# hidasib/GRU4Rec

Measured on NVIDIA H100. Metric: mini-batches/sec, higher is better.
Workload: dtype f32

## Files before the change

### gru4rec_b200/_lib.py

```python
import ctypes as C
import os
import numpy as np

_HERE = os.path.dirname(os.path.abspath(__file__))
LIB_PATH = os.path.join(_HERE, 'libg4r.so')
G4R_MAX_LAYERS = 8
G4R_TOPK_MAX = 1024
SCHED_POSITIONS = 2

G4R_OK, G4R_ERR_INVALID, G4R_ERR_INDEX, G4R_ERR_CUDA, G4R_ERR_NAN, G4R_ERR_STATE = 0, -1, -2, -3, -4, -5
LOSS = {'cross-entropy': 0, 'bpr-max': 1, 'top1-max': 2, 'bpr': 3, 'top1': 4, 'xe_logit': 5}
ACT = {'linear': 0, 'relu': 1, 'tanh': 2, 'leaky': 3, 'elu': 4, 'selu': 5, 'softmax': 6, 'softmax_logit': 7}
ADAPT = {None: 0, 'adagrad': 1, 'rmsprop': 2, 'adadelta': 3, 'adam': 4}


class G4RConfig(C.Structure):
    _fields_ = [
        ('n_items', C.c_int32), ('n_layers', C.c_int32), ('layers', C.c_int32 * G4R_MAX_LAYERS), ('batch_size', C.c_int32),
        ('embedding', C.c_int32), ('constrained_embedding', C.c_int32), ('loss', C.c_int32),
        ('final_act', C.c_int32), ('final_act_p1', C.c_float), ('final_act_p2', C.c_float),
        ('hidden_act', C.c_int32), ('hidden_act_p1', C.c_float), ('hidden_act_p2', C.c_float),
        ('dropout_p_hidden', C.c_float), ('dropout_p_embed', C.c_float),
        ('learning_rate', C.c_float), ('momentum', C.c_float), ('lmbd', C.c_float),
        ('n_sample', C.c_int32), ('sample_alpha', C.c_float),
        ('smoothing', C.c_float), ('bpreg', C.c_float), ('logq', C.c_float),
        ('adapt', C.c_int32), ('sample_store', C.c_int32), ('dropout_seed', C.c_uint32), ('mrg_seed', C.c_uint32),
        ('max_resident_steps', C.c_int32), ('device', C.c_int32), ('world_size', C.c_int32), ('rank', C.c_int32),
        ('eval_batch_size', C.c_int32), ('step_mode', C.c_int32), ('mg_replicated', C.c_int32), ('eval_tc', C.c_int32),
        ('adapt_p1', C.c_float), ('adapt_p1c', C.c_float), ('adapt_p2', C.c_float), ('adapt_p2c', C.c_float), ('grad_cap', C.c_float),
    ]


EXPORTS = [
    'g4r_version', 'g4r_workspace_bytes', 'g4r_create', 'g4r_destroy', 'g4r_last_error', 'g4r_stream',
    'g4r_tensor_shape', 'g4r_set_tensor', 'g4r_get_tensor', 'g4r_reset_hidden',
    'g4r_set_sampling_cdf', 'g4r_set_logq_support', 'g4r_generate_samples', 'g4r_generate_samples_from_uniform',
    'g4r_set_sample_store', 'g4r_get_sample_store', 'g4r_sample_store_rows', 'g4r_set_sample_pointer', 'g4r_get_sample_pointer',
    'g4r_mrg_uniform', 'g4r_searchsorted', 'g4r_gather_rows',
    'g4r_schedule_build', 'g4r_schedule_build_history', 'g4r_schedule_free', 'g4r_schedule_steps', 'g4r_schedule_events', 'g4r_schedule_export', 'g4r_schedule_positions',
    'g4r_train_step', 'g4r_train_steps', 'g4r_upload_steps', 'g4r_run_uploaded', 'g4r_kernel_launches',
    'g4r_profile_uploaded', 'g4r_phase_name', 'g4r_phase_count', 'g4r_persistent_stamps', 'g4r_fast_windows', 'g4r_uses_tensor_cores', 'g4r_mg_unique_id', 'g4r_mg_init',
    'g4r_mg_sharded', 'g4r_mg_ipc_handle', 'g4r_mg_ipc_open', 'g4r_mg_owner', 'g4r_mg_local_row', 'g4r_mg_shard_rows', 'g4r_mg_segment_bytes',
    'g4r_eval_schedule', 'g4r_eval_events', 'g4r_eval_counts', 'g4r_set_eval_items', 'g4r_set_eval_exclude_seen', 'g4r_predict', 'g4r_reset_eval_hidden',
    'g4r_predict_topk', 'g4r_predict_topk_filtered',
    'g4r_sessions_open', 'g4r_sessions_count', 'g4r_sessions_feed', 'g4r_sessions_topk', 'g4r_sessions_end',
    'g4r_sessions_export', 'g4r_sessions_import',
]

_lib = None


def load():
    global _lib
    if _lib is not None:
        return _lib
    if not os.path.exists(LIB_PATH):
        raise RuntimeError('libg4r.so not found at %s: build it with gru4rec_b200/csrc/build.sh '
                           '(there is no CPU fallback)' % LIB_PATH)
    lib = C.CDLL(LIB_PATH)
    vp, i32, i64, f32p = C.c_void_p, C.c_int32, C.c_int64, C.POINTER(C.c_float)
    lib.g4r_version.restype = C.c_int
    lib.g4r_workspace_bytes.argtypes = [C.POINTER(G4RConfig), C.POINTER(C.c_size_t)]
    lib.g4r_create.argtypes = [C.POINTER(G4RConfig), vp, C.c_size_t, C.POINTER(vp)]
    lib.g4r_destroy.argtypes = [vp]
    lib.g4r_last_error.argtypes = [vp]; lib.g4r_last_error.restype = C.c_char_p
    lib.g4r_stream.argtypes = [vp]; lib.g4r_stream.restype = vp
    lib.g4r_tensor_shape.argtypes = [vp, C.c_char_p, C.POINTER(i64), C.POINTER(i64)]
    lib.g4r_set_tensor.argtypes = [vp, C.c_char_p, vp, i64, i64]
    lib.g4r_get_tensor.argtypes = [vp, C.c_char_p, vp, i64, i64]
    lib.g4r_reset_hidden.argtypes = [vp]
    lib.g4r_set_sampling_cdf.argtypes = [vp, vp, i64]
    lib.g4r_set_logq_support.argtypes = [vp, vp, i64]
    lib.g4r_generate_samples.argtypes = [vp]
    lib.g4r_generate_samples_from_uniform.argtypes = [vp, vp, i64]
    lib.g4r_set_sample_store.argtypes = [vp, vp, i64]
    lib.g4r_get_sample_store.argtypes = [vp, vp, i64]
    lib.g4r_sample_store_rows.argtypes = [vp]
    lib.g4r_set_sample_pointer.argtypes = [vp, i64]
    lib.g4r_get_sample_pointer.argtypes = [vp]; lib.g4r_get_sample_pointer.restype = i64
    lib.g4r_mrg_uniform.argtypes = [vp, vp, i64]
    lib.g4r_searchsorted.argtypes = [vp, vp, i64, vp, i64, vp]
    lib.g4r_gather_rows.argtypes = [vp, vp, i64, i64, vp, i64, vp]
    lib.g4r_schedule_build.argtypes = [vp, i64, vp, i64, vp, i32, i32, i32, C.POINTER(vp)]
    lib.g4r_schedule_build_history.argtypes = [vp, i64, vp, i64, vp, vp, i32, i32, C.POINTER(vp)]
    lib.g4r_schedule_free.argtypes = [vp]
    lib.g4r_schedule_steps.argtypes = [vp]; lib.g4r_schedule_steps.restype = i64
    lib.g4r_schedule_events.argtypes = [vp]; lib.g4r_schedule_events.restype = i64
    lib.g4r_schedule_export.argtypes = [vp, vp, vp, vp, vp, vp]
    lib.g4r_schedule_positions.argtypes = [vp, vp]
    lib.g4r_train_step.argtypes = [vp, vp, vp, i32, vp, C.POINTER(C.c_float)]
    lib.g4r_train_steps.argtypes = [vp, vp, i64, i64, vp, C.POINTER(i64)]
    lib.g4r_upload_steps.argtypes = [vp, vp, i64, i64]
    lib.g4r_run_uploaded.argtypes = [vp, vp, C.POINTER(C.c_float)]
    lib.g4r_kernel_launches.argtypes = [vp]; lib.g4r_kernel_launches.restype = i64
    lib.g4r_profile_uploaded.argtypes = [vp, vp, vp, i32]
    lib.g4r_phase_name.argtypes = [i32]; lib.g4r_phase_name.restype = C.c_char_p
    lib.g4r_phase_count.restype = C.c_int
    lib.g4r_persistent_stamps.argtypes = [vp, i32, vp, i64]
    lib.g4r_fast_windows.argtypes = [vp, C.POINTER(i64)]; lib.g4r_fast_windows.restype = i64
    lib.g4r_uses_tensor_cores.argtypes = [vp]
    lib.g4r_mg_unique_id.argtypes = [vp]
    lib.g4r_mg_init.argtypes = [vp, vp]
    lib.g4r_mg_sharded.argtypes = [vp]
    lib.g4r_mg_ipc_handle.argtypes = [vp, vp]
    lib.g4r_mg_ipc_open.argtypes = [vp, vp, i32]
    lib.g4r_mg_owner.argtypes = [i64, i32]
    lib.g4r_mg_local_row.argtypes = [i64, i32]; lib.g4r_mg_local_row.restype = i64
    lib.g4r_mg_shard_rows.argtypes = [i64, i32, i32]; lib.g4r_mg_shard_rows.restype = i64
    lib.g4r_mg_segment_bytes.argtypes = [C.POINTER(G4RConfig), C.POINTER(C.c_size_t), C.POINTER(C.c_size_t), C.POINTER(C.c_size_t), C.POINTER(C.c_size_t)]
    lib.g4r_eval_schedule.argtypes = [vp, vp, vp, i32, i32, vp, vp, C.POINTER(i64)]
    lib.g4r_eval_events.argtypes = [vp, vp, vp, i32, i32, i32, vp, vp, C.POINTER(i64), vp, vp, vp]
    lib.g4r_eval_counts.argtypes = [vp, vp, i64]
    lib.g4r_set_eval_items.argtypes = [vp, vp, i64]
    lib.g4r_set_eval_exclude_seen.argtypes = [vp, i32]
    lib.g4r_predict.argtypes = [vp, vp, i32, vp, vp]
    lib.g4r_reset_eval_hidden.argtypes = [vp]
    lib.g4r_predict_topk.argtypes = [vp, vp, i32, vp, i32, vp, vp]
    lib.g4r_predict_topk_filtered.argtypes = [vp, vp, i32, vp, i32, vp, i64, vp, vp, vp, vp]
    lib.g4r_sessions_open.argtypes = [vp, i64]
    lib.g4r_sessions_count.argtypes = [vp, C.POINTER(i64)]; lib.g4r_sessions_count.restype = i64
    lib.g4r_sessions_feed.argtypes = [vp, vp, vp, i64]
    lib.g4r_sessions_topk.argtypes = [vp, vp, vp, i64, i32, vp, i64, vp, vp, i32, vp, vp]
    lib.g4r_sessions_end.argtypes = [vp, vp, i64]
    lib.g4r_sessions_export.argtypes = [vp, vp, vp, vp, vp]
    lib.g4r_sessions_import.argtypes = [vp, vp, vp, vp, vp, i64]
    _lib = lib
    return lib


class NaNError(ArithmeticError):
    def __init__(self, msg, step):
        ArithmeticError.__init__(self, msg)
        self.step = step


def _ptr(a):
    return a.ctypes.data_as(C.c_void_p) if a is not None else None


def parse_act(name):
    if name in ('linear', 'relu', 'tanh', 'softmax', 'softmax_logit'):
        return ACT[name], 0.0, 0.0
    if name.startswith('leaky-'):
        return ACT['leaky'], float(name.split('-')[1]), 0.0
    if name.startswith('elu-'):
        return ACT['elu'], float(name.split('-')[1]), 0.0
    if name.startswith('selu-'):
        p = [float(x) for x in name.split('-')[1:]]
        return ACT['selu'], p[0], p[1]
    raise NotImplementedError


SEEN_BUDGET = 256 << 20


def seen_budget():
    env = os.environ.get('G4R_SEEN_BUDGET')
    return SEEN_BUDGET if env is None else min(SEEN_BUDGET, max(0, int(env)))


def check_topk(k, n_items):
    if not isinstance(k, (int, np.integer)) or isinstance(k, bool) or not 1 <= k <= min(n_items, G4R_TOPK_MAX):
        raise ValueError('k must be an integer in 1 .. min(n_items, %d) = %d, got %r' % (G4R_TOPK_MAX, min(n_items, G4R_TOPK_MAX), k))
    return int(k)


def set_adapt_params(cfg, adapt, adapt_params, grad_cap):
    ap = [float(x) for x in (adapt_params or [])]
    if adapt in ('rmsprop', 'adadelta') and len(ap) < 1 or adapt == 'adam' and len(ap) < 2:
        raise IndexError('list index out of range')
    cfg.adapt_p1 = ap[0] if len(ap) > 0 else 0.0
    cfg.adapt_p1c = (1.0 - ap[0]) if len(ap) > 0 else 0.0
    cfg.adapt_p2 = ap[1] if len(ap) > 1 else 0.0
    cfg.adapt_p2c = (1.0 - ap[1]) if len(ap) > 1 else 0.0
    cfg.grad_cap = float(grad_cap or 0.0)


def make_config(n_items, mk, sample_store=0, eval_lanes=0, max_resident_steps=0, step_mode=0, world_size=1, rank=0, replicated=False, eval_tc=None):
    cfg = G4RConfig()
    layers = mk.get('layers', [100])
    cfg.n_items = n_items
    cfg.n_layers = len(layers)
# ... 224 lines not shown
        self._check(self.lib.g4r_train_step(self.h, _ptr(X), _ptr(Y), len(X), _ptr(Rp), C.byref(cost)))
        return np.float32(cost.value)

    def train_steps(self, sched, first=0, n=None):
        n = sched.n_steps - first if n is None else n
        if self.cfg.world_size > 1:
            import torch
            import torch.distributed as dist
            if dist.is_available() and dist.is_initialized():
                dev = 'cuda' if dist.get_backend() == 'nccl' else 'cpu'
                t = torch.tensor([n, -n], dtype=torch.int64, device=dev)
                dist.all_reduce(t, op=dist.ReduceOp.MIN)
                if int(t[0]) != n or int(-t[1]) != n:
                    raise ValueError('train_steps: every rank must run the same number of steps (got %d, range %d..%d)' % (n, int(t[0]), int(-t[1])))
        costs = np.empty(n, dtype=np.float32)
        nan_step = C.c_int64(-1)
        rc = self.lib.g4r_train_steps(self.h, sched.h, first, n, _ptr(costs), C.byref(nan_step))
        self._check(rc, nan_step.value)
        return costs

    def upload_steps(self, sched, first, n):
        self._check(self.lib.g4r_upload_steps(self.h, sched.h, first, n))

    def run_uploaded(self, n, want_cost=True):
        costs = np.empty(n, dtype=np.float32) if want_cost else None
        ms = C.c_float()
        self._check(self.lib.g4r_run_uploaded(self.h, _ptr(costs), C.byref(ms)))
        return costs, ms.value

    def profile_uploaded(self):
        n = self.lib.g4r_phase_count()
        ms = np.zeros(n, dtype=np.float32); cnt = np.zeros(n, dtype=np.int32)
        self._check(self.lib.g4r_profile_uploaded(self.h, _ptr(ms), _ptr(cnt), n))
        return {self.lib.g4r_phase_name(i).decode(): (float(ms[i]), int(cnt[i])) for i in range(n) if cnt[i] > 0}

    def persistent_stamps(self, enable=True, n_steps=0):
        out = np.zeros((n_steps, 16), dtype=np.uint64) if n_steps > 0 else None
        self._check(self.lib.g4r_persistent_stamps(self.h, 1 if enable else 0, _ptr(out), n_steps))
        return out

    def init_multi_gpu(self, dist):
        import torch
        buf = (C.c_char * 128)()
        if dist.get_rank() == 0:
            rc = self.lib.g4r_mg_unique_id(buf)
            if rc != 0:
                raise RuntimeError('ncclGetUniqueId failed')
        t = torch.tensor(list(bytes(buf)), dtype=torch.uint8, device='cuda' if dist.get_backend() == 'nccl' else 'cpu')
        dist.broadcast(t, 0)
        raw = bytes(t.cpu().tolist())
        idbuf = (C.c_char * 128).from_buffer_copy(raw)
        self._check(self.lib.g4r_mg_init(self.h, idbuf))
        self._dist = dist
        if self.sharded():
            mh = (C.c_char * 64)()
            self._check(self.lib.g4r_mg_ipc_handle(self.h, mh))
            dev = 'cuda' if dist.get_backend() == 'nccl' else 'cpu'
            mine = torch.tensor(list(bytes(mh)), dtype=torch.uint8, device=dev)
            allh = [torch.empty_like(mine) for _ in range(dist.get_world_size())]
            dist.all_gather(allh, mine)
            raw = b''.join(bytes(t.cpu().tolist()) for t in allh)
            buf2 = (C.c_char * len(raw)).from_buffer_copy(raw)
            self._check(self.lib.g4r_mg_ipc_open(self.h, buf2, dist.get_world_size()))
            dist.barrier()

    def sharded(self):
        return bool(self.lib.g4r_mg_sharded(self.h))

    def _quiesce(self):
        d = getattr(self, '_dist', None)
        if d is not None and self.sharded():
            import torch
            torch.cuda.synchronize()
            d.barrier()

    def uses_tensor_cores(self):
        return bool(self.lib.g4r_uses_tensor_cores(self.h))

    def fast_windows(self):
        fb = C.c_int64()
        n = self.lib.g4r_fast_windows(self.h, C.byref(fb))
        return n, fb.value

    def kernel_launches(self):
        return self.lib.g4r_kernel_launches(self.h)

    def stream(self):
        return self.lib.g4r_stream(self.h)

    def eval_schedule(self, sched, cut_off, mode=0):
        cut = np.ascontiguousarray(cut_off, dtype=np.int32)
        rec = np.zeros(len(cut), dtype=np.float64); mrr = np.zeros(len(cut), dtype=np.float64)
        n = C.c_int64()
        self._check(self.lib.g4r_eval_schedule(self.h, sched.h, _ptr(cut), len(cut), mode, _ptr(rec), _ptr(mrr), C.byref(n)))
        return rec, mrr, n.value

    def eval_events(self, sched, cut_off, mode=0, k=0):
        cut = np.ascontiguousarray(cut_off, dtype=np.int32)
        rec = np.zeros(len(cut), dtype=np.float64); mrr = np.zeros(len(cut), dtype=np.float64)
        n = C.c_int64()
        counts = np.empty((sched.n_events, 2), dtype=np.int32)
        items = scores = None
        if k:
            items = np.empty((sched.n_events, k), dtype=np.int32); scores = np.empty((sched.n_events, k), dtype=np.float32)
        self._check(self.lib.g4r_eval_events(self.h, sched.h, _ptr(cut), len(cut), mode, int(k), _ptr(rec), _ptr(mrr), C.byref(n),
                                             _ptr(counts), _ptr(items), _ptr(scores)))
        return rec, mrr, n.value, counts, items, scores

    def eval_counts(self, n_lanes):
        out = np.zeros((n_lanes, 2), dtype=np.int32)
        self._check(self.lib.g4r_eval_counts(self.h, _ptr(out), n_lanes))
        return out

    def set_eval_items(self, items=None):
        if items is None or len(items) == 0:
            self._check(self.lib.g4r_set_eval_items(self.h, None, 0))
            return
        it = np.ascontiguousarray(items, dtype=np.int64)
        self._check(self.lib.g4r_set_eval_items(self.h, _ptr(it), it.size))

    def set_eval_exclude_seen(self, on):
        self._check(self.lib.g4r_set_eval_exclude_seen(self.h, 1 if on else 0))

    def predict(self, X, reset_mask=None):
        X = np.ascontiguousarray(X, dtype=np.int32)
        rm = None if reset_mask is None else np.ascontiguousarray(reset_mask, dtype=np.uint8)
        out = np.empty((len(X), self.cfg.n_items), dtype=np.float32)
        self._check(self.lib.g4r_predict(self.h, _ptr(X), len(X), _ptr(rm), _ptr(out)))
        return out

    def predict_topk(self, X, k, reset_mask=None, items=None, exclude=None):
        X = np.ascontiguousarray(X, dtype=np.int32)
        rm = None if reset_mask is None else np.ascontiguousarray(reset_mask, dtype=np.uint8)
        if items is None and exclude is None:
            k = check_topk(k, self.cfg.n_items)
            out_i = np.empty((len(X), k), dtype=np.int32)
            out_s = np.empty((len(X), k), dtype=np.float32)
            self._check(self.lib.g4r_predict_topk(self.h, _ptr(X), len(X), _ptr(rm), k, _ptr(out_i), _ptr(out_s)))
            return out_i, out_s
        k, cand, off, ex = self._topk_filters(len(X), k, items, exclude)
        out_i = np.empty((len(X), k), dtype=np.int32)
        out_s = np.empty((len(X), k), dtype=np.float32)
        self._check(self.lib.g4r_predict_topk_filtered(self.h, _ptr(X), len(X), _ptr(rm), k, _ptr(cand), 0 if cand is None else cand.size,
                                                       _ptr(off), _ptr(ex), _ptr(out_i), _ptr(out_s)))
        return out_i, out_s

    def _topk_filters(self, n, k, items, exclude):
        cand = None
        n_distinct = self.cfg.n_items
        if items is not None:
            cand = np.asarray(items, dtype=np.int64).reshape(-1)
            if cand.size and (cand.min() < 0 or cand.max() >= self.cfg.n_items):
                raise IndexError('candidate item index out of range')
            cand = np.ascontiguousarray(cand, dtype=np.int32)
            n_distinct = int(np.count_nonzero(np.bincount(cand, minlength=self.cfg.n_items)))
        k = check_topk(k, n_distinct)
        off = ex = None
        if exclude is not None:
            if len(exclude) != n:
                raise ValueError('exclude must hold one entry per lane (%d), got %d' % (n, len(exclude)))
            parts = [np.asarray(e if e is not None else [], dtype=np.int64).reshape(-1) for e in exclude]
            off = np.zeros(n + 1, dtype=np.int64)
            off[1:] = np.cumsum([len(p) for p in parts])
            ex = np.concatenate(parts) if parts else np.zeros(0, np.int64)
            if ex.size and (ex.min() < 0 or ex.max() >= self.cfg.n_items):
                raise IndexError('excluded item index out of range')
# ... 60 lines not shown
```

### gru4rec_b200/csrc/g4r_fast.cuh

```cuda
#pragma once

constexpr int FK_THREADS = 512;
constexpr int FK_NW = FK_THREADS / 32;
constexpr int FK_G = 48;
constexpr int FK_CT = 32;
constexpr int FK_Q = FK_CT / FK_NW;
constexpr int FK_B = 32;
static_assert(FK_THREADS / 16 == FK_B, "statistics mapping: 16 threads per lane");
constexpr int FK_LDS = 132;


__device__ __forceinline__ void red_release_add(unsigned int* p, unsigned int v) {
  asm volatile("red.release.gpu.global.add.u32 [%0], %1;" :: "l"(p), "r"(v) : "memory");
}
__device__ __forceinline__ unsigned int atom_acqrel_add(unsigned int* p, unsigned int v) {
  unsigned int old;
  asm volatile("atom.acq_rel.gpu.global.add.u32 %0, [%1], %2;" : "=r"(old) : "l"(p), "r"(v) : "memory");
  return old;
}
__device__ __forceinline__ void wait_ge(const unsigned int* p, unsigned int target) {
  while (ld_acquire_u32(p) < target) { }
}
__device__ __forceinline__ uint32_t smem_u32(const void* p) { return (uint32_t)__cvta_generic_to_shared(p); }
__device__ __forceinline__ void mbar_init(uint64_t* bar, unsigned int count) {
  asm volatile("mbarrier.init.shared::cta.b64 [%0], %1;" :: "r"(smem_u32(bar)), "r"(count) : "memory");
}
__device__ __forceinline__ void mbar_expect_tx(uint64_t* bar, unsigned int bytes) {
  asm volatile("mbarrier.arrive.expect_tx.shared::cta.b64 _, [%0], %1;" :: "r"(smem_u32(bar)), "r"(bytes) : "memory");
}
__device__ __forceinline__ void mbar_wait(uint64_t* bar, unsigned int parity) {
  asm volatile(
      "{\n\t.reg .pred p;\n\t"
      "WAIT_LOOP:\n\t"
      "mbarrier.try_wait.parity.shared::cta.b64 p, [%0], %1;\n\t"
      "@p bra.uni WAIT_DONE;\n\t"
      "bra.uni WAIT_LOOP;\n\t"
      "WAIT_DONE:\n\t}\n" :: "r"(smem_u32(bar)), "r"(parity) : "memory");
}
__device__ __forceinline__ void tma_row(void* sdst, const void* gsrc, unsigned int bytes, uint64_t* bar) {
  asm volatile("cp.async.bulk.shared::cluster.global.mbarrier::complete_tx::bytes [%0], [%1], %2, [%3];"
               :: "r"(smem_u32(sdst)), "l"(gsrc), "r"(bytes), "r"(smem_u32(bar)) : "memory");
}

struct FastSmem {
  alignas(128) float sY[FK_B * FK_LDS];
  float sS[FK_CT * FK_LDS];
  float sAcc[FK_CT * FK_LDS];
  float sVel[FK_CT * FK_LDS];
  float sTW[FK_B * FK_LDS];
  float sD[FK_CT * FK_LDS];
  float sG[FK_CT * FK_B];
  float sO[FK_CT * FK_B];
  float sRS[FK_B * 8];
  float sPart[FK_NW * FK_B * 8];
  float sT[FK_B];
  float sBias[FK_CT], sByP[FK_CT], sByA[FK_CT], sByV[FK_CT], sDby[FK_CT], sTB[FK_B];
  int sIt[2][FK_CT], sPos[2][FK_CT], sTc[2][FK_B], sYit[2][FK_B], sCb[2][2];
  int sFlag[4];
  alignas(8) unsigned long long mbar;
  alignas(16) float gA[FK_B * 388];
  alignas(16) float gW[8 * FK_LDS + FK_NW * FK_B * 5 + 16 * FK_B];
  int gIdx[3 * FK_B];
};

template <class SM>
__device__ __forceinline__ void fk_load_idx(const ModelDev& md, SM& sm, int s, int n_steps, int chunk, int buf) {
  const int tid = threadIdx.x;
  if (s >= n_steps) return;
  const int M = md.wM[s];
  const int* cbeg = md.pCbeg + (size_t)s * (md.NCH + 1);
  const bool hc = chunk < md.NCH;
  const int cb = hc ? cbeg[chunk] : 0, ce = hc ? cbeg[chunk + 1] : 0;
  if (tid < FK_CT) {
    int it = 0, pos = 0;
    if (cb + tid < ce) { it = md.pItem[(size_t)s * md.NP + cb + tid]; pos = md.pPos[(size_t)s * md.NP + cb + tid]; }
    sm.sIt[buf][tid] = it; sm.sPos[buf][tid] = pos;
  }
  if (tid >= 32 && tid < 32 + FK_B) {
    const int b = tid - 32;
    sm.sTc[buf][b] = b < M ? md.pTcol[(size_t)s * md.B + b] : -1;
    sm.sYit[buf][b] = b < M ? md.wY[(size_t)s * md.B + b] : 0;
  }
  if (tid == 64) { sm.sCb[buf][0] = cb; sm.sCb[buf][1] = ce; }
}

template <class SM>
__device__ __forceinline__ void fk_prefetch_rows(const ModelDev& md, SM& sm, int s, int n_steps, int buf, bool pw) {
  if (s >= n_steps) return;
  const int tid = threadIdx.x;
  const int M = md.wM[s];
  const int cb = sm.sCb[buf][0], ce = sm.sCb[buf][1];
  const int nj = ce - cb;
  const bool ada = md.adapt == G4R_ADAPT_ADAGRAD, mom = md.mom > 0.f;
  const unsigned int rowb = (unsigned int)md.ldL * 4u;
  uint64_t* bar = reinterpret_cast<uint64_t*>(&sm.mbar);
  const int ntab = 1 + (ada ? 1 : 0) + (mom ? 1 : 0);
  const int ncopy = nj * ntab + (pw ? M : 0);
  if (tid == 0) {
    const unsigned int total = rowb * (unsigned int)ncopy;
    if (total > 0) mbar_expect_tx(bar, total);
    else asm volatile("mbarrier.arrive.shared::cta.b64 _, [%0];" :: "r"(smem_u32(bar)) : "memory");
  }
  if ((tid & 31) == 0) {
    asm volatile("fence.proxy.async.global;" ::: "memory");
    for (int i = tid >> 5; i < ncopy; i += FK_NW) {
      if (i < nj * ntab) {
        const int j = i / ntab, t = i % ntab;
        const size_t off = (size_t)sm.sIt[buf][j] * md.ldL;
        if (t == 0) tma_row(sm.sS + j * FK_LDS, md.Wy + off, rowb, bar);
        else if (t == 1 && ada) tma_row(sm.sAcc + j * FK_LDS, md.Wy_acc + off, rowb, bar);
        else tma_row(sm.sVel + j * FK_LDS, md.Wy_vel + off, rowb, bar);
      } else {
        const int b = i - nj * ntab;
        tma_row(sm.sTW + b * FK_LDS, md.Wy + (size_t)sm.sYit[buf][b] * md.ldL, rowb, bar);
      }
    }
  }
  if (false) {
  } else if (tid >= 64 && tid < 64 + FK_CT) {
    const int j = tid - 64;
    if (j < nj) {
      const int it = sm.sIt[buf][j];
      float bz = md.By[it];
      sm.sByP[j] = bz;
      if (md.logq > 0.f) bz -= (sm.sPos[buf][j] < M) ? md.logP0t[it] : md.logP0s[it];
      sm.sBias[j] = bz;
      sm.sByA[j] = ada ? md.By_acc[it] : 0.f;
      sm.sByV[j] = mom ? md.By_vel[it] : 0.f;
    }
  } else if (tid >= 96 && tid < 96 + FK_B) {
    const int b = tid - 96;
    if (pw && b < M) {
      const int it = sm.sYit[buf][b];
      float bz = md.By[it];
      if (md.logq > 0.f) bz -= md.logP0t[it];
      sm.sTB[b] = bz;
    }
  }
}

__device__ __forceinline__ void fk_group_barrier(FastSync* fs, unsigned int& gepoch, unsigned int G = FK_G) {
  __syncthreads();
  gepoch += 1;
  if (threadIdx.x == 0) { red_release_add(&fs->grp, 1u); wait_ge(&fs->grp, gepoch * G); }
  __syncthreads();
}

template <class SM>
__device__ __forceinline__ void fk_stage_lanes(const ModelDev& md, SM& sm, int s, int M) {
  if (threadIdx.x < FK_B) {
    const int b = threadIdx.x;
    sm.gIdx[b] = b < M ? md.wSlot[(size_t)s * md.B + b] : -1;
    sm.gIdx[FK_B + b] = b < M ? md.wX[(size_t)s * md.B + b] : 0;
    sm.gIdx[2 * FK_B + b] = b < M ? md.wF[(size_t)s * md.B + b] : 0;
  }
  __syncthreads();
}
template <int W>
__device__ __forceinline__ void fk_slab_dot(float (&acc)[W], const float* sAop, int lda, const float* sWt, int K) {
  const int b = threadIdx.x & 31, ks = threadIdx.x >> 5;
  const int kq = (K + 3) / 4;
  const int per = (kq + FK_NW - 1) / FK_NW;
  const int q0 = ks * per, q1 = min(kq, q0 + per);
#pragma unroll
  for (int j = 0; j < W; j++) acc[j] = 0.f;
  for (int q = q0; q < q1; q++) {
    const float4 a = ld4(sAop + b * lda + q * 4);
#pragma unroll
    for (int j = 0; j < W; j++) {
      const float4 w = ld4(sWt + j * FK_LDS + q * 4);
      acc[j] = fmaf(a.x, w.x, acc[j]); acc[j] = fmaf(a.y, w.y, acc[j]); acc[j] = fmaf(a.z, w.z, acc[j]); acc[j] = fmaf(a.w, w.w, acc[j]);
    }
  }
}
template <int W>
__device__ __forceinline__ float fk_slab_reduce(const float (&acc)[W], float* red, int jsel) {
  const int b = threadIdx.x & 31, ks = threadIdx.x >> 5;
#pragma unroll
  for (int j = 0; j < W; j++) red[(ks * FK_B + b) * W + j] = acc[j];
  __syncthreads();
  float v = 0.f;
  if (jsel < W) {
#pragma unroll
    for (int k = 0; k < FK_NW; k++) v += red[(k * FK_B + b) * W + jsel];
  }
  return v;
}
constexpr int FK_W1 = 5;
constexpr int FK_W2 = 3;

__device__ void fk_f1(const ModelDev& md, FastSmem& sm, int s, int cta, const unsigned int* wait_ctr, unsigned int wait_target, const float* inrows = nullptr) {
  const LayerDev& ly = md.layer[0];
  const int M = md.wM[s], L = ly.L, ldL = ly.ldL, tid = threadIdx.x;
  const int c0 = cta * FK_W1;
  if (c0 >= 2 * L) return;
  const int W = min(FK_W1, 2 * L - c0);
  fk_stage_lanes(md, sm, s, M);
  if (tid == 0) sm.sFlag[3] = (!wait_ctr || ld_acquire_u32(wait_ctr) >= wait_target) ? 1 : 0;
  const int kw = ldL / 4;
  stage_rows4(sm.gA, FK_LDS, FK_B, kw, [&](int rr) -> const float* { const int sl = sm.gIdx[rr]; return sl >= 0 ? ly.H + (size_t)sl * ldL : nullptr; });
  for (int i = tid; i < FK_W1 * FK_LDS; i += FK_THREADS) {
    const int j = i / FK_LDS, k = i % FK_LDS;
    sm.gW[i] = (j < W && k < L) ? ly.Wrz[(size_t)k * ly.ld2 + c0 + j] : 0.f;
  }
  const int b = tid & 31, jsel = tid >> 5;
  __syncthreads();
  const bool early = sm.sFlag[3] != 0;
  float pre = 0.f;
  if (early && jsel < W && b < M) pre = (inrows ? inrows[(size_t)b * ly.ld3 + L + c0 + jsel] : ly.Wx[(size_t)sm.gIdx[FK_B + b] * ly.ld3 + L + c0 + jsel]) + ly.Bh[L + c0 + jsel];
  float acc[FK_W1];
  fk_slab_dot<FK_W1>(acc, sm.gA, FK_LDS, sm.gW, L);
  const float v = fk_slab_reduce<FK_W1>(acc, sm.gW + 8 * FK_LDS, jsel);
  if (!early) {
    if (tid == 0) wait_ge(wait_ctr, wait_target);
    __syncthreads();
    if (jsel < W && b < M) pre = (inrows ? inrows[(size_t)b * ly.ld3 + L + c0 + jsel] : ly.Wx[(size_t)sm.gIdx[FK_B + b] * ly.ld3 + L + c0 + jsel]) + ly.Bh[L + c0 + jsel];
  }
  if (jsel < W && b < M) {
    const int c = c0 + jsel;
    const float g = sigmoidf_(v + pre);
    if (c < L) ly.r[(size_t)b * ldL + c] = g; else ly.z[(size_t)b * ldL + (c - L)] = g;
  }
  if (cta == 0) {
    for (int i = tid; i < FK_B * kw; i += FK_THREADS) {
      const int rr = i / kw, c4 = i % kw;
      if (rr < M) st4(ly.Hold + (size_t)rr * ldL + c4 * 4, ld4(sm.gA + rr * FK_LDS + c4 * 4));
    }
// ... 18 lines not shown
        if (rr < M) { hv[u] = ld4(ly.Hold + (size_t)rr * ldL + c4 * 4); rv[u] = ld4(ly.r + (size_t)rr * ldL + c4 * 4); }
      }
    }
#pragma unroll
    for (int u = 0; u < 2; u++) {
      const int i = i0 + u * FK_THREADS + tid;
      if (i < FK_B * kw) st4(sm.gA + (i / kw) * FK_LDS + (i % kw) * 4, make_float4(hv[u].x * rv[u].x, hv[u].y * rv[u].y, hv[u].z * rv[u].z, hv[u].w * rv[u].w));
    }
  }
  for (int i = tid; i < FK_W2 * FK_LDS; i += FK_THREADS) {
    const int j = i / FK_LDS, k = i % FK_LDS;
    sm.gW[i] = (j < W && k < L) ? ly.Wh[(size_t)k * ldL + c0 + j] : 0.f;
  }
  const int b = tid & 31, jsel = tid >> 5;
  float pre = 0.f, z = 0.f, ho = 0.f;
  if (jsel < W && b < M) {
    const int c = c0 + jsel;
    pre = (inrows ? inrows[(size_t)b * ly.ld3 + c] : ly.Wx[(size_t)sm.gIdx[FK_B + b] * ly.ld3 + c]) + ly.Bh[c];
    z = ly.z[(size_t)b * ldL + c];
    ho = ly.Hold[(size_t)b * ldL + c];
  }
  __syncthreads();
  float acc[FK_W2];
  fk_slab_dot<FK_W2>(acc, sm.gA, FK_LDS, sm.gW, L);
  const float v0 = fk_slab_reduce<FK_W2>(acc, sm.gW + 8 * FK_LDS, jsel);
  if (jsel < W && b < M) {
    const int c = c0 + jsel;
    const float v = v0 + pre;
    const float ht = act_fwd(md.hact, v);
    float h = (1.0f - z) * ho + z * ht;
    if (md.p_drop_h > 0.f) h *= drop_scale(md.drop_seed, md.wG[s], 0u, (uint32_t)(b * L + c), 1.0f - md.p_drop_h);
    ly.ah[(size_t)b * ldL + c] = v;
    ly.ht[(size_t)b * ldL + c] = ht;
    ly.y[(size_t)b * ldL + c] = h;
    ly.H[(size_t)sm.gIdx[b] * ldL + c] = (sm.gIdx[2 * FK_B + b] & 1) ? 0.f : h;
  }
}
__device__ void fk_b2(const ModelDev& md, FastSmem& sm, int s, int cta) {
  const LayerDev& ly = md.layer[0];
  const int M = md.wM[s], L = ly.L, ldL = ly.ldL, tid = threadIdx.x;
  const int c0 = cta * FK_W2;
  if (c0 >= L) return;
  const int W = min(FK_W2, L - c0);
  const int kw = ldL / 4;
  __syncthreads();
  stage_rows4(sm.gA, FK_LDS, FK_B, kw, [&](int rr) -> const float* { return rr < M ? ly.dvec + (size_t)rr * ly.ld3 : nullptr; });
  stage_rows4(sm.gW, FK_LDS, W, kw, [&](int rr) -> const float* { return ly.Wh + (size_t)(c0 + rr) * ldL; });
  const int b = tid & 31, jsel = tid >> 5;
  float ho = 0.f, r = 0.f;
  if (jsel < W && b < M) { ho = ly.Hold[(size_t)b * ldL + c0 + jsel]; r = ly.r[(size_t)b * ldL + c0 + jsel]; }
  __syncthreads();
  float acc[FK_W2];
  fk_slab_dot<FK_W2>(acc, sm.gA, FK_LDS, sm.gW, L);
  const float v = fk_slab_reduce<FK_W2>(acc, sm.gW + 8 * FK_LDS, jsel);
  if (jsel < W && b < M) ly.dvec[(size_t)b * ly.ld3 + L + c0 + jsel] = v * ho * r * (1.f - r);
}
template <class SM>
__device__ void fk_sparse_in(const ModelDev& md, SM& sm, int s, int b) {
  const LayerDev& ly = md.layer[0];
  const int M = md.wM[s];
  if (b >= M) return;
  const uint8_t xf = md.wXflag[(size_t)s * md.B + b];
  if (!(xf & 1)) return;
  const int ld3 = ly.ld3, tid = threadIdx.x;
  const int item = md.wX[(size_t)s * md.B + b];
  const int* xnext = md.wXnext + (size_t)s * md.B;
  if (tid == 0) { int n = 0; for (int bb = b; bb >= 0 && n < FK_B; bb = xnext[bb]) sm.gIdx[n++] = bb; sm.gIdx[FK_B] = n; }
  __syncthreads();
  const int nmem = sm.gIdx[FK_B];
  const bool ada = md.adapt == G4R_ADAPT_ADAGRAD, mom = md.mom > 0.f;
  float* prow = ly.Wx + (size_t)item * ld3;
  for (int c4 = tid; c4 < ld3 / 4; c4 += FK_THREADS) {
    const float4 p0 = ld4(prow + c4 * 4), z = make_float4(0.f, 0.f, 0.f, 0.f);
    RowChain<float4> u;
    u.begin(p0, p0, ada ? ld4(ly.Wx_acc + (size_t)item * ld3 + c4 * 4) : z, mom ? ld4(ly.Wx_vel + (size_t)item * ld3 + c4 * 4) : z);
    for (int k = 0; k < nmem; k++) u.add(md, ld4(ly.dvec + (size_t)sm.gIdx[k] * ld3 + c4 * 4), ada, mom);
    st4(prow + c4 * 4, u.ps);
    if (ada) st4(ly.Wx_acc + (size_t)item * ld3 + c4 * 4, u.al);
    if (mom) st4(ly.Wx_vel + (size_t)item * ld3 + c4 * 4, u.vl);
  }
}

template <class SM>
__device__ void fk_sparse_in_one(const ModelDev& md, SM& sm, int s, int b, const unsigned int* ctr, unsigned int target) {
  const LayerDev& ly = md.layer[0];
  const int M = md.wM[s], ld3 = ly.ld3, tid = threadIdx.x;
  const bool act = b < M && (md.wXflag[(size_t)s * md.B + b] & 1);
  const int item = act ? md.wX[(size_t)s * md.B + b] : 0;
  const bool ada = md.adapt == G4R_ADAPT_ADAGRAD, mom = md.mom > 0.f;
  if (act && tid == 0) {
    const int* xnext = md.wXnext + (size_t)s * md.B;
    int n = 0; for (int bb = b; bb >= 0 && n < FK_B; bb = xnext[bb]) sm.gIdx[n++] = bb; sm.gIdx[FK_B] = n;
  }
  float* prow = ly.Wx + (size_t)item * ld3;
  const int c4 = tid;
  const bool mine = act && c4 < ld3 / 4;
  float4 p0 = make_float4(0.f, 0.f, 0.f, 0.f), a0 = p0, v0 = p0;
  if (mine) {
    p0 = ld4(prow + c4 * 4);
    if (ada) a0 = ld4(ly.Wx_acc + (size_t)item * ld3 + c4 * 4);
    if (mom) v0 = ld4(ly.Wx_vel + (size_t)item * ld3 + c4 * 4);
  }
  if (tid == 0) wait_ge(ctr, target);
  __syncthreads();
  if (mine) {
    const int nmem = sm.gIdx[FK_B];
    RowChain<float4> u;
    u.begin(p0, p0, a0, v0);
    for (int k = 0; k < nmem; k++) u.add(md, ld4(ly.dvec + (size_t)sm.gIdx[k] * ld3 + c4 * 4), ada, mom);
    st4(prow + c4 * 4, u.ps);
    if (ada) st4(ly.Wx_acc + (size_t)item * ld3 + c4 * 4, u.al);
    if (mom) st4(ly.Wx_vel + (size_t)item * ld3 + c4 * 4, u.vl);
  }
}

template <bool CL, class SM>
__device__ void fk_b1(const ModelDev& md, SM& sm, int s, int cta, int ncta) {
  const LayerDev& ly = md.layer[0];
  const int M = md.wM[s], L = ly.L, ldL = ly.ldL;
  const int tid = threadIdx.x, lane = tid & 31, warp = tid >> 5;
  const int E = M * ldL;
  const int per = ((E + ncta - 1) / ncta + 31) / 32 * 32;
  const int e0 = cta * per;
  float* red = sm.sPart;
  const size_t cs = (size_t)md.B * ldL;
  float pht = 0.f, pho = 0.f, pz = 0.f, pah = 0.f;
  if (!CL && tid < per && e0 + tid < E && (e0 + tid) % ldL < L) {
    const size_t o = (size_t)((e0 + tid) / ldL) * ldL + (e0 + tid) % ldL;
    pht = ly.ht[o]; pho = ly.Hold[o]; pz = ly.z[o]; pah = ly.ah[o];
  }
  for (int eb = 0; eb < per; eb += 32) {
    const int e = e0 + eb + lane;
    float d = 0.f;
    if (e < E) {
      float v[10];
#pragma unroll
      for (int u = 0; u < 10; u++) { const int ch = warp + FK_NW * u; v[u] = ch < md.NCH ? md.part[(size_t)ch * cs + e] : 0.f; }
      d = (((v[0] + v[1]) + (v[2] + v[3])) + ((v[4] + v[5]) + (v[6] + v[7]))) + (v[8] + v[9]);
    }
    red[warp * per + eb + lane] = d;
  }
  __syncthreads();
  for (int i = tid; i < per; i += FK_THREADS) {
    const int e = e0 + i;
    if (e >= E) continue;
    const int b = e / ldL, c = e % ldL;
    if (c >= L) continue;
    float dy = 0.f;
#pragma unroll
    for (int w = 0; w < FK_NW; w++) dy += red[w * per + i];
    const size_t o = (size_t)b * ldL + c;
    if (CL) { ly.dy[o] = dy; continue; }
    const float ht = pht, ho = pho, z = pz, ah = pah;
    float dh = dy;
    if (md.p_drop_h > 0.f) dh *= drop_scale(md.drop_seed, md.wG[s], 0u, (uint32_t)(b * L + c), 1.0f - md.p_drop_h);
    const float dz = dh * (ht - ho);
    const float dah = dh * z * act_der(md.hact, ah, ht);
    ly.dvec[(size_t)b * ly.ld3 + c] = dah;
    ly.dvec[(size_t)b * ly.ld3 + 2 * L + c] = dz * z * (1.f - z);
  }
}

constexpr int FR_U = 4;

struct FastSmemR {
  alignas(128) float sY[FK_B * FK_LDS];
  float sS[FK_CT * FK_LDS];
  float sAcc[FK_CT * FK_LDS];
  float sVel[FK_CT * FK_LDS];
  float sTW[FK_B * FK_LDS];
  float sD[FK_CT * FK_LDS];
  float sG[FK_CT * FK_B];
  float sO[FK_CT * FK_B];
  float sRS[FK_B * 8];
  float sPart[FK_NW * FK_B * 8];
  float sT[FK_B];
  float sBias[FK_CT], sByP[FK_CT], sByA[FK_CT], sByV[FK_CT], sDby[FK_CT], sTB[FK_B];
  int sIt[2][FK_CT], sPos[2][FK_CT], sTc[2][FK_B], sYit[2][FK_B], sCb[2][2];
  int sFlag[4];
  alignas(8) unsigned long long mbar;
  int gIdx[3 * FK_B];
  alignas(16) float gH[2][FK_B * FK_LDS];
  float gHr[FK_B * FK_LDS];
  float rC[3][3 * FR_U * FK_LDS];
  float rR[3][FR_U * FK_LDS];
  float rB[3][3 * FR_U];
  float gR[FK_B * FR_U], gZ[FK_B * FR_U], gDr[FK_B * FR_U], gDz[FK_B * FR_U];
};
static_assert(sizeof(FastSmemR) <= 232448, "FastSmemR exceeds the 227 KB shared memory of one CTA");
static_assert(FK_NW * FK_B * 8 >= FK_NW * FK_B * 2 * FR_U, "sPart too small for the F1 reduction");

__device__ void fr_load_resident(const ModelDev& md, FastSmemR& sm, int k0) {
  const LayerDev& ly = md.layer[0];
  const int L = ly.L, tid = threadIdx.x;
  for (int i = tid; i < 3 * FR_U * FK_LDS; i += FK_THREADS) {
    const int q = i / FK_LDS, k = i % FK_LDS, t = q / FR_U, c = k0 + q % FR_U;
    float p = 0.f, a = 0.f, v = 0.f;
    if (c < L && k < L) {
      const size_t o = t == 0 ? (size_t)k * ly.ldL + c : (size_t)k * ly.ld2 + (t == 2 ? L : 0) + c;
      const float* P = t == 0 ? ly.Wh : ly.Wrz;
      const float* A = t == 0 ? ly.Wh_acc : ly.Wrz_acc;
      const float* V = t == 0 ? ly.Wh_vel : ly.Wrz_vel;
      p = P[o]; if (A) a = A[o]; if (V) v = V[o];
    }
    sm.rC[0][i] = p; sm.rC[1][i] = a; sm.rC[2][i] = v;
  }
  for (int i = tid; i < FR_U * FK_LDS; i += FK_THREADS) {
    const int k = k0 + i / FK_LDS, c = i % FK_LDS;
    float p = 0.f, a = 0.f, v = 0.f;
    if (k < L && c < L) {
      const size_t o = (size_t)k * ly.ldL + c;
      p = ly.Wh[o]; if (ly.Wh_acc) a = ly.Wh_acc[o]; if (ly.Wh_vel) v = ly.Wh_vel[o];
    }
    sm.rR[0][i] = p; sm.rR[1][i] = a; sm.rR[2][i] = v;
  }
  if (tid < 3 * FR_U) {
    const int c = k0 + tid % FR_U;
    float p = 0.f, a = 0.f, v = 0.f;
    if (c < L) { const int o = (tid / FR_U) * L + c; p = ly.Bh[o]; if (ly.Bh_acc) a = ly.Bh_acc[o]; if (ly.Bh_vel) v = ly.Bh_vel[o]; }
    sm.rB[0][tid] = p; sm.rB[1][tid] = a; sm.rB[2][tid] = v;
  }
  __syncthreads();
}
__device__ void fr_store_resident(const ModelDev& md, FastSmemR& sm, int k0) {
  const LayerDev& ly = md.layer[0];
  const int L = ly.L, tid = threadIdx.x;
  __syncthreads();
  for (int i = tid; i < 3 * FR_U * FK_LDS; i += FK_THREADS) {
    const int q = i / FK_LDS, k = i % FK_LDS, t = q / FR_U, c = k0 + q % FR_U;
    if (c < L && k < L) {
      const size_t o = t == 0 ? (size_t)k * ly.ldL + c : (size_t)k * ly.ld2 + (t == 2 ? L : 0) + c;
      float* P = t == 0 ? ly.Wh : ly.Wrz;
      float* A = t == 0 ? ly.Wh_acc : ly.Wrz_acc;
      float* V = t == 0 ? ly.Wh_vel : ly.Wrz_vel;
      P[o] = sm.rC[0][i]; if (A) A[o] = sm.rC[1][i]; if (V) V[o] = sm.rC[2][i];
    }
  }
  if (tid < 3 * FR_U) {
    const int c = k0 + tid % FR_U;
    if (c < L) { const int o = (tid / FR_U) * L + c; ly.Bh[o] = sm.rB[0][tid]; if (ly.Bh_acc) ly.Bh_acc[o] = sm.rB[1][tid]; if (ly.Bh_vel) ly.Bh_vel[o] = sm.rB[2][tid]; }
  }
}

__device__ void fr_f1(const ModelDev& md, FastSmemR& sm, int s, int k0, const float* sH, const unsigned int* wait_ctr, unsigned int wait_target) {
  const LayerDev& ly = md.layer[0];
  const int M = md.wM[s], L = ly.L, ldL = ly.ldL, tid = threadIdx.x;
  if (tid == 0) sm.sFlag[3] = (!wait_ctr || ld_acquire_u32(wait_ctr) >= wait_target) ? 1 : 0;
  __syncthreads();
  const bool early = sm.sFlag[3] != 0;
  const int b = tid & 31, jsel = tid >> 5, j = jsel % FR_U, c = k0 + j;
  const bool isr = jsel < FR_U;
  const bool on = jsel < 2 * FR_U && b < M && c < L;
  const int col = (isr ? L : 2 * L) + c;
  const float bias = sm.rB[0][(isr ? 1 : 2) * FR_U + j];
  float pre = 0.f;
  if (early && on) pre = ly.Wx[(size_t)sm.gIdx[FK_B + b] * ly.ld3 + col] + bias;
  float acc[2 * FR_U];
  fk_slab_dot<2 * FR_U>(acc, sH, FK_LDS, sm.rC[0] + FR_U * FK_LDS, L);
  const float v = fk_slab_reduce<2 * FR_U>(acc, sm.sPart, jsel);
  if (!early) {
    if (tid == 0) wait_ge(wait_ctr, wait_target);
    __syncthreads();
    if (on) pre = ly.Wx[(size_t)sm.gIdx[FK_B + b] * ly.ld3 + col] + bias;
  }
  if (jsel < 2 * FR_U) {
    const float g = on ? sigmoidf_(v + pre) : 0.f;
    if (isr) {
      sm.gR[b * FR_U + j] = g;
      if (on) {
        const float ho = sH[b * FK_LDS + c];
        ly.r[(size_t)b * ldL + c] = g;
        ly.Hold[(size_t)b * ldL + c] = ho;
        ly.Hr[(size_t)b * ldL + c] = ho * g;
      }
    } else {
      sm.gZ[b * FR_U + j] = g;
      if (on) ly.z[(size_t)b * ldL + c] = g;
    }
  }
}
__device__ void fr_f2(const ModelDev& md, FastSmemR& sm, int s, int k0, const float* sHo) {
  const LayerDev& ly = md.layer[0];
  const int M = md.wM[s], L = ly.L, ldL = ly.ldL, tid = threadIdx.x;
  const int b = tid & 31, jsel = tid >> 5, c = k0 + jsel;
  const bool on = jsel < FR_U && b < M && c < L;
  float pre = 0.f;
  if (on) pre = ly.Wx[(size_t)sm.gIdx[FK_B + b] * ly.ld3 + c] + sm.rB[0][jsel];
  stage_rows4(sm.gHr, FK_LDS, FK_B, ldL / 4, [&](int rr) -> const float* { return rr < M ? ly.Hr + (size_t)rr * ldL : nullptr; });
  __syncthreads();
  float acc[FR_U];
  fk_slab_dot<FR_U>(acc, sm.gHr, FK_LDS, sm.rC[0], L);
  const float v0 = fk_slab_reduce<FR_U>(acc, sm.sPart, jsel);
  if (on) {
    const float v = v0 + pre;
    const float ht = act_fwd(md.hact, v);
    const float z = sm.gZ[b * FR_U + jsel], ho = sHo[b * FK_LDS + c];
    float h = (1.0f - z) * ho + z * ht;
    if (md.p_drop_h > 0.f) h *= drop_scale(md.drop_seed, md.wG[s], 0u, (uint32_t)(b * L + c), 1.0f - md.p_drop_h);
    ly.ah[(size_t)b * ldL + c] = v;
    ly.ht[(size_t)b * ldL + c] = ht;
    ly.y[(size_t)b * ldL + c] = h;
    ly.H[(size_t)sm.gIdx[b] * ldL + c] = (sm.gIdx[2 * FK_B + b] & 1) ? 0.f : h;
  }
}
__device__ void fr_b2(const ModelDev& md, FastSmemR& sm, int s, int k0, const float* sHo) {
  const LayerDev& ly = md.layer[0];
  const int M = md.wM[s], L = ly.L, ld3 = ly.ld3, tid = threadIdx.x;
  float dz = 0.f;
  if (tid < FK_B * FR_U && tid / FR_U < M && k0 + tid % FR_U < L) dz = ly.dvec[(size_t)(tid / FR_U) * ld3 + 2 * L + k0 + tid % FR_U];
  stage_rows4(sm.sD, FK_LDS, FK_B, ly.ldL / 4, [&](int rr) -> const float* { return rr < M ? ly.dvec + (size_t)rr * ld3 : nullptr; });
  if (tid < FK_B * FR_U) sm.gDz[tid] = dz;
  __syncthreads();
  const int b = tid & 31, jsel = tid >> 5, c = k0 + jsel;
  float acc[FR_U];
  fk_slab_dot<FR_U>(acc, sm.sD, FK_LDS, sm.rR[0], L);
  const float v = fk_slab_reduce<FR_U>(acc, sm.sPart, jsel);
  if (jsel < FR_U) {
    float dar = 0.f;
    if (b < M && c < L) {
      const float ho = sHo[b * FK_LDS + c], r = sm.gR[b * FR_U + jsel];
      dar = v * ho * r * (1.f - r);
      ly.dvec[(size_t)b * ld3 + L + c] = dar;
    }
    sm.gDr[b * FR_U + jsel] = dar;
  }
}
__device__ void fr_dense(const ModelDev& md, FastSmemR& sm, int s, int k0, const float* sHo) {
  const LayerDev& ly = md.layer[0];
  const int M = md.wM[s], L = ly.L, kw = ly.ldL / 4;
  const bool ada = md.adapt == G4R_ADAPT_ADAGRAD, mom = md.mom > 0.f;
  const int ncol = 3 * FR_U * kw, nrow = FR_U * kw;
  for (int t = threadIdx.x; t < ncol + nrow + 3 * FR_U; t += FK_THREADS) {
    if (t < ncol + nrow) {
      const bool colt = t < ncol;
      const int u = colt ? t : t - ncol, q = u % kw, jm = u / kw, j = jm % FR_U;
      const float* vec; const float* sc; int ss, o;
      if (colt) {
        const int m = jm / FR_U;
        vec = (m == 0 ? sm.gHr : sHo) + q * 4;
        if (m == 0) { sc = sm.sD + k0 + j; ss = FK_LDS; } else { sc = (m == 1 ? sm.gDr : sm.gDz) + j; ss = FR_U; }
        o = jm * FK_LDS + q * 4;
      } else {
        vec = sm.sD + q * 4; sc = sm.gHr + k0 + j; ss = FK_LDS;
        o = j * FK_LDS + q * 4;
      }
      float4 g = make_float4(0.f, 0.f, 0.f, 0.f);
#pragma unroll 4
      for (int b = 0; b < M; b++) {
        const float4 a = ld4(vec + b * FK_LDS);
        const float d = sc[b * ss];
        g.x = fmaf(a.x, d, g.x); g.y = fmaf(a.y, d, g.y); g.z = fmaf(a.z, d, g.z); g.w = fmaf(a.w, d, g.w);
      }
      if (k0 + j < L) {
        float* P = colt ? sm.rC[0] : sm.rR[0];
        float* A = colt ? sm.rC[1] : sm.rR[1];
        float* V = colt ? sm.rC[2] : sm.rR[2];
        if (q * 4 + 0 < L) dense_elem(md, ada, mom, g.x, P + o + 0, A + o + 0, V + o + 0);
        if (q * 4 + 1 < L) dense_elem(md, ada, mom, g.y, P + o + 1, A + o + 1, V + o + 1);
        if (q * 4 + 2 < L) dense_elem(md, ada, mom, g.z, P + o + 2, A + o + 2, V + o + 2);
        if (q * 4 + 3 < L) dense_elem(md, ada, mom, g.w, P + o + 3, A + o + 3, V + o + 3);
      }
    } else {
      const int i = t - ncol - nrow, m = i / FR_U, j = i % FR_U;
      if (k0 + j < L) {
        float g = 0.f;
        for (int b = 0; b < M; b++) g = g + (m == 0 ? sm.sD[b * FK_LDS + k0 + j] : (m == 1 ? sm.gDr : sm.gDz)[b * FR_U + j]);
        dense_elem(md, ada, mom, g, sm.rB[0] + i, sm.rB[1] + i, sm.rB[2] + i);
      }
    }
  }
}
template <class SM>
__device__ __forceinline__ void fk_part(SM& sm, float* part, int M, int nj, int ldL) {
  const int kw = ldL / 4;
  for (int t = threadIdx.x; t < M * kw; t += FK_THREADS) {
    const int bb = t / kw, q4 = t % kw;
    float4 a = make_float4(0.f, 0.f, 0.f, 0.f);
    for (int jj = 0; jj < nj; jj++) {
      const float g = sm.sG[jj * FK_B + bb];
      const float4 w = ld4(sm.sS + jj * FK_LDS + q4 * 4);
      a.x = fmaf(g, w.x, a.x); a.y = fmaf(g, w.y, a.y); a.z = fmaf(g, w.z, a.z); a.w = fmaf(g, w.w, a.w);
    }
    st4(part + (size_t)bb * ldL + q4 * 4, a);
  }
}
template <class SM>
__device__ __forceinline__ void fk_dsy(SM& sm, int M, int nj, int kw) {
  for (int t = threadIdx.x; t < nj * kw; t += FK_THREADS) {
    const int jj = t / kw, q4 = t % kw;
    float4 d = make_float4(0.f, 0.f, 0.f, 0.f);
    for (int bb = 0; bb < M; bb++) {
      const float4 y = ld4(sm.sY + bb * FK_LDS + q4 * 4);
      const float g = sm.sG[jj * FK_B + bb];
      d.x = fmaf(g, y.x, d.x); d.y = fmaf(g, y.y, d.y); d.z = fmaf(g, y.z, d.z); d.w = fmaf(g, y.w, d.w);
    }
    st4(sm.sD + jj * FK_LDS + q4 * 4, d);
  }
}
template <class SM>
__device__ __forceinline__ void fk_update_rows(const ModelDev& md, SM& sm, int buf, int nj, int kw) {
  const int lane = threadIdx.x & 31, warp = threadIdx.x >> 5, ldL = md.ldL;
  const bool ada = md.adapt == G4R_ADAPT_ADAGRAD, mom = md.mom > 0.f;
  for (int j = warp; j < nj; j += FK_NW) {
    const int item = sm.sIt[buf][j];
    if (j > 0 && sm.sIt[buf][j - 1] == item) continue;
    int je = j + 1;
    while (je < nj && sm.sIt[buf][je] == item) je++;
    if (lane < kw) {
      const float4 p0 = ld4(sm.sS + j * FK_LDS + lane * 4), z = make_float4(0.f, 0.f, 0.f, 0.f);
      RowChain<float4> u;
      u.begin(p0, p0, ada ? ld4(sm.sAcc + j * FK_LDS + lane * 4) : z, mom ? ld4(sm.sVel + j * FK_LDS + lane * 4) : z);
      for (int k = j; k < je; k++) u.add(md, ld4(sm.sD + k * FK_LDS + lane * 4), ada, mom);
      const size_t off = (size_t)item * ldL + lane * 4;
      st4(md.Wy + off, u.ps);
      if (ada) st4(md.Wy_acc + off, u.al);
      if (mom) st4(md.Wy_vel + off, u.vl);
    }
    if (lane == 0) {
      RowChain<float> u;
      u.begin(sm.sByP[j], sm.sByP[j], sm.sByA[j], sm.sByV[j]);
      for (int k = j; k < je; k++) u.add(md, sm.sDby[k], ada, mom);
      md.By[item] = u.ps;
      if (ada) md.By_acc[item] = u.al;
      if (mom) md.By_vel[item] = u.vl;
    }
  }
}
template <class SM>
__device__ __forceinline__ void fk_dby(SM& sm, int M, int nj) {
  const int lane = threadIdx.x & 31, warp = threadIdx.x >> 5;
  for (int jj = warp; jj < nj; jj += FK_NW) {
    float a = (lane < M) ? sm.sG[jj * FK_B + lane] : 0.f;
    a = warp_sum(a);
    if (lane == 0) sm.sDby[jj] = a;
  }
}
#include "g4r_fastc.cuh"

template <bool CL>
__global__ void __launch_bounds__(FK_THREADS, 1) k_fast_t(int slot, int n_steps, FastSync* fs, unsigned long long* tstamp) {
  using SM = typename std::conditional<CL, FastSmemC, FastSmemR>::type;
  extern __shared__ __align__(128) unsigned char fk_raw[];
  SM& sm = *reinterpret_cast<SM*>(fk_raw);
  const ModelDev& md = MD;
  const LayerDev& ly = md.layer[0];
  const int cta = blockIdx.x, ncta = gridDim.x;
  const int tid = threadIdx.x, lane = tid & 31, warp = tid >> 5;
  const int G = CL ? (int)cl_size() : md.ldL / 4;
  const bool gru = cta < G;
  const bool col = CL || !gru;
  const int chunk = CL ? cta : cta - G;
  const int ncol = CL ? ncta : ncta - G;
  const bool has_chunk = col && chunk < md.NCH;
  const bool pw = loss_pairwise(md.loss);
  const int ldL = md.ldL, B = md.B;
  const int kw = ldL / 4;
  uint64_t* bar = reinterpret_cast<uint64_t*>(&sm.mbar);
  unsigned int bar_epoch = 0, gepoch = 0, stats_target = 0;
  const int in_ctas = min(B, ncta - G);
#ifdef G4R_CF_FINE
#define FK_FTS(s_) ((tstamp && cta == 0 && (s_) < 500 && n_steps >= 1000) ? tstamp + (size_t)((s_) + 500) * 16 : nullptr)
#define FK_STAMP_OK(s_) ((s_) < 500)
#else
#define FK_FTS(s_) ((unsigned long long*)nullptr)
#define FK_STAMP_OK(s_) true
#endif
#define FK_STAMP(k) do { if (tstamp && cta == ((CL || ((k) >= 4 && (k) <= 8)) ? 0 : G) && tid == 0 && FK_STAMP_OK(s)) { unsigned long long t_; asm volatile("mov.u64 %0, %%globaltimer;" : "=l"(t_)); tstamp[(size_t)s * 16 + (k)] = t_; } } while (0)
  if (tid == 0) { mbar_init(bar, 1); asm volatile("fence.mbarrier_init.release.cluster;" ::: "memory"); }
  if (col) fk_load_idx(md, sm, 0, n_steps, chunk, 0);
  __syncthreads();
  if (col) fk_prefetch_rows(md, sm, 0, n_steps, 0, pw);
  ClusterCtx cc = {0, 1, 0, 0};
  if constexpr (CL) {
    if (gru) {
      cc = cf_init(md, sm);
      cf_load_resident(md, sm, cc);
      if (n_steps > 0) {
        fk_stage_lanes(md, sm, 0, md.wM[0]);
        cf_f1(md, sm, cc, 0, false, nullptr, 0u, nullptr);
        cf_f2(md, sm, cc, 0, nullptr);
        __syncthreads();
        if (tid == 0) red_release_add(&fs->h_ready, 1u);
      }
    }
  } else {
    if (gru) {
      fr_load_resident(md, sm, 4 * cta);
      if (n_steps > 0) {
        fk_stage_lanes(md, sm, 0, md.wM[0]);
        stage_rows4(sm.gH[0], FK_LDS, FK_B, kw, [&](int rr) -> const float* { const int sl = sm.gIdx[rr]; return sl >= 0 ? ly.H + (size_t)sl * ldL : nullptr; });
        fr_f1(md, sm, 0, 4 * cta, sm.gH[0], nullptr, 0u);
        fk_group_barrier(fs, gepoch, G);
        fr_f2(md, sm, 0, 4 * cta, sm.gH[0]);
        __syncthreads();
        if (tid == 0) red_release_add(&fs->h_ready, 1u);
      }
    }
  }
  for (int s = 0; s < n_steps; s++) {
    const int buf = s & 1;
    const int M = md.wM[s];
    const int sti = md.wSti[s];
    const int N = M + (sti >= 0 ? md.S : 0);
    FK_STAMP(0);
    if (col) fk_load_idx(md, sm, s + 1, n_steps, chunk, buf ^ 1);
    const bool gru_next = !CL && gru && s + 1 < n_steps;
    if (gru_next && tid < FK_B) {
      const int M1 = md.wM[s + 1];
      sm.gIdx[tid] = tid < M1 ? md.wSlot[(size_t)(s + 1) * B + tid] : -1;
      sm.gIdx[FK_B + tid] = tid < M1 ? md.wX[(size_t)(s + 1) * B + tid] : 0;
      sm.gIdx[2 * FK_B + tid] = tid < M1 ? md.wF[(size_t)(s + 1) * B + tid] : 0;
    }
    if (tid == 0) wait_ge(&fs->h_ready, (unsigned int)(s + 1) * (unsigned int)G);
    __syncthreads();
    if constexpr (!CL) {
      if (!col) {
        const bool nxt = s + 1 < n_steps;
        const int k0 = 4 * cta;
        const float* sHo = sm.gH[s & 1];
        float* hnext = sm.gH[(s + 1) & 1];
        if (nxt) stage_rows4(hnext, FK_LDS, FK_B, kw, [&](int rr) -> const float* { const int sl = sm.gIdx[rr]; return sl >= 0 ? ly.H + (size_t)sl * ldL : nullptr; });
        __syncthreads();
        if (tid == 0) wait_ge(&fs->b1_done, (unsigned int)(s + 1) * (unsigned int)ncol);
        __syncthreads();
        FK_STAMP(4);
        fr_b2(md, sm, s, k0, sHo);
        __syncthreads();
        if (tid == 0) red_release_add(&fs->dvec_done, 1u);
        FK_STAMP(5);
        fr_dense(md, sm, s, k0, sHo);
        FK_STAMP(6);
        if (nxt) {
          fr_f1(md, sm, s + 1, k0, hnext, &fs->in_done, (unsigned int)(s + 1) * (unsigned int)in_ctas);
          fk_group_barrier(fs, gepoch, G);
          FK_STAMP(7);
          fr_f2(md, sm, s + 1, k0, hnext);
          __syncthreads();
          if (tid == 0) red_release_add(&fs->h_ready, 1u);
        }
        FK_STAMP(8);
        continue;
      }
    }
    stage_rows4(sm.sY, FK_LDS, FK_B, kw, [&](int rr) -> const float* { return rr < M ? ly.y + (size_t)rr * ldL : nullptr; });
    mbar_wait(bar, (unsigned int)(s & 1));
    __syncthreads();
    FK_STAMP(1);
    const int cb = sm.sCb[buf][0], ce = sm.sCb[buf][1];
    const int nj = ce - cb;
    if (pw) {
      for (int b = warp; b < FK_B; b += FK_NW) {
        if (b < M) {
          float a = 0.f;
          if (lane < kw) {
            const float4 y = ld4(sm.sY + b * FK_LDS + lane * 4), w = ld4(sm.sTW + b * FK_LDS + lane * 4);
            a = fmaf(w.x, y.x, a); a = fmaf(w.y, y.y, a); a = fmaf(w.z, y.z, a); a = fmaf(w.w, y.w, a);
          }
          a = warp_sum(a);
          if (lane == 0) sm.sT[b] = act_fwd(md.fact, a + sm.sTB[b]);
        }
      }
    }
    {
      float accq[FK_Q];
#pragma unroll
      for (int q = 0; q < FK_Q; q++) accq[q] = 0.f;
      const float* yr = sm.sY + lane * FK_LDS;
      for (int c4 = 0; c4 < kw; c4++) {
        const float4 y = ld4(yr + c4 * 4);
#pragma unroll
        for (int q = 0; q < FK_Q; q++) {
          if (warp + FK_NW * q < nj) {
            const float4 w = ld4(sm.sS + (warp + FK_NW * q) * FK_LDS + c4 * 4);
            accq[q] = fmaf(y.x, w.x, accq[q]); accq[q] = fmaf(y.y, w.y, accq[q]); accq[q] = fmaf(y.z, w.z, accq[q]); accq[q] = fmaf(y.w, w.w, accq[q]);
          }
        }
      }
      FK_STAMP(9);
#pragma unroll
      for (int q = 0; q < FK_Q; q++) {
        const int jj = warp + q * FK_NW;
        if (jj < nj && lane < M) sm.sO[jj * FK_B + lane] = accq[q] + sm.sBias[jj];
      }
      __syncthreads();
      {
        const int b = tid >> 4, sub = tid & 15;
        const bool okb = b < M;
        const int tc = okb ? sm.sTc[buf][b] : -1;
        const float t = (pw && okb) ? sm.sT[b] : 0.f;
        float yv[2]; bool use[2], ist[2];
        float mloc = -INFINITY;
        const bool smx = loss_softmaxneg(md.loss), xe = (md.loss == G4R_LOSS_XE || md.loss == G4R_LOSS_XE_LOGIT);
#pragma unroll
        for (int q = 0; q < 2; q++) {
          const int jj = sub + 16 * q;
          use[q] = okb && jj < nj;
          ist[q] = use[q] && (tc == cb + jj);
          const float o = use[q] ? sm.sO[jj * FK_B + b] : 0.f;
          yv[q] = xe ? o : act_fwd(md.fact, o);
          if (use[q] && (xe || (smx && !ist[q]))) mloc = fmaxf(mloc, yv[q]);
        }
#pragma unroll
        for (int o = 1; o < 16; o <<= 1) mloc = fmaxf(mloc, __shfl_xor_sync(0xffffffffu, mloc, o));
        float Z = 0.f, A = 0.f, Q = 0.f, D = 0.f, T = 0.f, has = 0.f;
#pragma unroll
        for (int q = 0; q < 2; q++) {
          if (!use[q]) continue;
          const float y = yv[q];
          if (ist[q]) has = 1.f;
          if (xe) { Z += expf(y - mloc); if (ist[q]) T = y; }
          else if (md.loss == G4R_LOSS_BPR_MAX) { if (!ist[q]) { const float e = expf(y - mloc), sg = sigmoidf_(t - y); Z += e; A += sg * e; Q += y * y * e; D += sg * (1.f - sg) * e; } }
          else if (md.loss == G4R_LOSS_TOP1_MAX) { if (!ist[q]) { const float e = expf(y - mloc), a1 = sigmoidf_(y - t), b1 = sigmoidf_(y * y); Z += e; A += (a1 + b1) * e; D += a1 * (1.f - a1) * e; } }
          else if (md.loss == G4R_LOSS_BPR) { const float sg = sigmoidf_(t - y); A += -logf(sg); if (!ist[q]) D += 1.f - sg; }
          else { const float a1 = sigmoidf_(y - t), b1 = sigmoidf_(y * y); A += a1 + b1; if (!ist[q]) D += a1 * (1.f - a1); }
        }
#pragma unroll
        for (int o = 1; o < 16; o <<= 1) {
          Z += __shfl_xor_sync(0xffffffffu, Z, o); A += __shfl_xor_sync(0xffffffffu, A, o); Q += __shfl_xor_sync(0xffffffffu, Q, o);
          D += __shfl_xor_sync(0xffffffffu, D, o); T += __shfl_xor_sync(0xffffffffu, T, o); has += __shfl_xor_sync(0xffffffffu, has, o);
        }
        if (has_chunk && okb && sub == 0) {
          float* st = md.stat + ((size_t)chunk * md.B + b) * G4R_NSTAT;
          st4(st, make_float4(mloc, Z, A, Q));
          st4(st + 4, make_float4(D, T, has > 0.f ? 1.f : 0.f, pw ? t : 0.f));
        }
      }
    }
    __syncthreads();
    FK_STAMP(10);
    bar_epoch += 1;
    if (tid == 0) { red_release_add(&fs->bar, 1u); wait_ge(&fs->bar, bar_epoch * (unsigned int)ncol); }
    __syncthreads();
    if (chunk < M) {
      const int b = chunk;
      const bool maxed = !(md.loss == G4R_LOSS_BPR || md.loss == G4R_LOSS_TOP1);
      float mc = -INFINITY, Z = 0.f, A = 0.f, Q = 0.f, D = 0.f, T = 0.f, has = 0.f, tt = 0.f;
      if (tid < md.NCH) {
        const float* st = md.stat + ((size_t)tid * md.B + b) * G4R_NSTAT;
        const float4 u = ld4(st), v = ld4(st + 4);
        mc = u.x; Z = u.y; A = u.z; Q = u.w; D = v.x; T = v.y; has = v.z;
        if (tid == 0) tt = v.w;
      }
      float mg = mc;
#pragma unroll
      for (int o = 1; o < 32; o <<= 1) mg = fmaxf(mg, __shfl_xor_sync(0xffffffffu, mg, o));
      if (lane == 0) sm.sPart[warp] = mg;
      __syncthreads();
      mg = sm.sPart[0];
      for (int w = 1; w < FK_NW; w++) mg = fmaxf(mg, sm.sPart[w]);
      if (loss_softmaxneg(md.loss)) mg = fmaxf(mg, 0.f);
      if (maxed) {
        const float sc = (mc == -INFINITY) ? 0.f : expf(mc - mg);
        Z *= sc; A *= sc; Q *= sc; D *= sc;
      }
#pragma unroll
      for (int o = 1; o < 32; o <<= 1) {
        Z += __shfl_xor_sync(0xffffffffu, Z, o); A += __shfl_xor_sync(0xffffffffu, A, o); Q += __shfl_xor_sync(0xffffffffu, Q, o);
        D += __shfl_xor_sync(0xffffffffu, D, o); T += __shfl_xor_sync(0xffffffffu, T, o); has += __shfl_xor_sync(0xffffffffu, has, o);
      }
      __syncthreads();
      if (lane == 0) { float* w = sm.sPart + 32 + warp * 8; w[0] = Z; w[1] = A; w[2] = Q; w[3] = D; w[4] = T; w[5] = has; w[6] = tt; }
      __syncthreads();
      if (tid == 0) {
        tt = sm.sPart[32 + 6];
        for (int w = 1; w < FK_NW; w++) { const float* q = sm.sPart + 32 + w * 8; Z += q[0]; A += q[1]; Q += q[2]; D += q[3]; T += q[4]; }
        const float m = mg;
        float* rs = md.RS + (size_t)b * G4R_NSTAT;
        float loss = 0.f, r0 = m, r1 = Z, r2 = 0.f, r3 = 0.f, r4 = 0.f, r5 = tt;
        if (md.loss == G4R_LOSS_XE) { const float pt = __fdiv_rn(expf(T - m), Z); loss = -logf(pt + G4R_EPS_LOG); r2 = pt; r5 = T; }
        else if (md.loss == G4R_LOSS_XE_LOGIT) { loss = logf(Z) - (T - m); r5 = T; }
        else if (md.loss == G4R_LOSS_BPR_MAX) { r2 = __fdiv_rn(A, Z); r3 = __fdiv_rn(Q, Z); r4 = __fdiv_rn(D, Z); loss = -logf(r2 + G4R_EPS_LOG) + md.bpreg * r3; }
        else if (md.loss == G4R_LOSS_TOP1_MAX) { r2 = __fdiv_rn(A, Z); r4 = __fdiv_rn(D, Z); loss = r2; }
        else if (md.loss == G4R_LOSS_BPR) { loss = A; r4 = D; }
        else { const float c = sigmoidf_(tt * tt); loss = (float)M * (__fdiv_rn(A, (float)N) - __fdiv_rn(c, (float)(M + md.S_cfg))); r4 = D; }
        st4(rs, make_float4(r0, r1, r2, r3));
        st4(rs + 4, make_float4(r4, r5, loss, 0.f));
        red_release_add(&fs->stats, 1u);
      }
    }
    stats_target += (unsigned int)M;
    if (tid == 0) wait_ge(&fs->stats, stats_target);
    __syncthreads();
    FK_STAMP(2);
    if (tid < M * 2) st4(sm.sRS + tid * 4, ld4(md.RS + tid * 4));
    __syncthreads();
    if (chunk == 0 && tid == 0) {
      float c = 0.f;
      for (int b = 0; b < M; b++) c += sm.sRS[b * 8 + 6];
      c = __fdiv_rn(c, (float)md.B);
      md.cost[s] = c;
      if (c != c) atomicExch(md.nanflag, 1);
    }
    FK_STAMP(11);
    for (int i = tid; i < FK_CT * FK_B; i += FK_THREADS) {
      const int jj = i / FK_B, b = i % FK_B;
      sm.sG[i] = (jj < nj && b < M) ? loss_grad_elem(md, sm.sRS + (size_t)b * 8, sm.sO[i], sm.sTc[buf][b] == cb + jj, M, N) : 0.f;
    }
    __syncthreads();
    fk_dby(sm, M, nj);
    FK_STAMP(12);
    float* part = md.part + (size_t)(has_chunk ? chunk : 0) * md.B * ldL;
    if constexpr (CL) {
      if (has_chunk) { fk_dsy(sm, M, nj, kw); fk_part(sm, part, M, nj, ldL); }
      __syncthreads();
      FK_STAMP(13);
      fk_update_rows(md, sm, buf, nj, kw);
      if (has_chunk && nj == 0) for (int i = tid; i < M * ldL; i += FK_THREADS) part[i] = 0.f;
      __syncthreads();
      FK_STAMP(14);
      bar_epoch += 1;
      if (tid == 0) { red_release_add(&fs->bar, 1u); wait_ge(&fs->bar, bar_epoch * (unsigned int)ncta); }
      __syncthreads();
      FK_STAMP(3);
      fk_b1<CL>(md, sm, s, cta, ncta);
      __syncthreads();
      if (tid == 0) red_release_add(&fs->b1_done, 1u);
      FK_STAMP(15);
      fk_prefetch_rows(md, sm, s + 1, n_steps, buf ^ 1, pw);
      FK_STAMP(4);
      if (gru) {
        if (s + 1 < n_steps) fk_stage_lanes(md, sm, s + 1, md.wM[s + 1]);
        cf_backward(md, sm, cc, fs, s, ncta, s + 1 < n_steps, (tstamp && cta == 0 && FK_STAMP_OK(s)) ? tstamp + (size_t)s * 16 : nullptr, FK_FTS(s));
        FK_STAMP(6);
        if (s + 1 < n_steps) {
          cf_f1(md, sm, cc, s + 1, true, &fs->in_done, (unsigned int)(s + 1) * (unsigned int)in_ctas, FK_FTS(s));
          FK_STAMP(7);
          cf_f2(md, sm, cc, s + 1, FK_FTS(s));
          __syncthreads();
          if (tid == 0) red_release_add(&fs->h_ready, 1u);
        } else {
          cl_wait();
        }
        FK_STAMP(8);
      }
      if (!gru && cta < G + in_ctas) {
        const unsigned int tgt = (unsigned int)(s + 1) * (unsigned int)G;
        if (in_ctas == B && ly.ld3 / 4 <= FK_THREADS) fk_sparse_in_one(md, sm, s, cta - G, &fs->grp, tgt);
        else {
          if (tid == 0) wait_ge(&fs->grp, tgt);
          __syncthreads();
          for (int b = cta - G; b < B; b += in_ctas) { fk_sparse_in(md, sm, s, b); __syncthreads(); }
        }
        __syncthreads();
        if (tid == 0) red_release_add(&fs->in_done, 1u);
      }
    } else {
      if (has_chunk) fk_part(sm, part, M, nj, ldL);
      if (has_chunk && nj == 0) for (int i = tid; i < M * ldL; i += FK_THREADS) part[i] = 0.f;
      __syncthreads();
      FK_STAMP(13);
      bar_epoch += 1;
      if (tid == 0) { red_release_add(&fs->bar, 1u); wait_ge(&fs->bar, bar_epoch * (unsigned int)ncol); }
      __syncthreads();
      FK_STAMP(3);
      fk_b1<CL>(md, sm, s, chunk, ncol);
      __syncthreads();
      if (tid == 0) red_release_add(&fs->b1_done, 1u);
      FK_STAMP(15);
      fk_dsy(sm, M, nj, kw);
      __syncthreads();
      if (chunk < in_ctas) {
        const unsigned int tgt = (unsigned int)(s + 1) * (unsigned int)G;
        if (in_ctas == B && ly.ld3 / 4 <= FK_THREADS) fk_sparse_in_one(md, sm, s, chunk, &fs->dvec_done, tgt);
        else {
          if (tid == 0) wait_ge(&fs->dvec_done, tgt);
          __syncthreads();
          for (int b = chunk; b < B; b += in_ctas) { fk_sparse_in(md, sm, s, b); __syncthreads(); }
        }
        __syncthreads();
        if (tid == 0) red_release_add(&fs->in_done, 1u);
      }
      fk_update_rows(md, sm, buf, nj, kw);
      __syncthreads();
      FK_STAMP(14);
      if (tid == 0) red_release_add(&fs->rows_done, 1u);
      if (s + 1 < n_steps) {
        if (tid == 0) wait_ge(&fs->rows_done, (unsigned int)(s + 1) * (unsigned int)ncol);
        __syncthreads();
        fk_prefetch_rows(md, sm, s + 1, n_steps, buf ^ 1, pw);
      }
    }
  }
  if constexpr (CL) { if (gru) cf_store_resident(md, sm, cc); }
  else { if (gru) fr_store_resident(md, sm, 4 * cta); }
#undef FK_STAMP
}
```

### gru4rec_b200/csrc/g4r_kernels.cuh

```cuda
#pragma once
#include <cuda_runtime.h>
#include <stdint.h>
#include "../../include/g4r.h"

#define G4R_EPS_LOG 1e-24f
#define G4R_NSTAT 8

struct ActSpec { int kind; float p1, p2; };
constexpr int MG_CAP = 256;
struct MgDev {
  int R, rank;
  int *gItem, *gPos, *gM, *gX;
  int *mEnt, *mItem, *mCbeg;
  int *mTot;
  int *xEnt, *xItem, *xTot;
  float *DSYall, *DBYall, *INall;
  float* gradFlat; size_t gradCount;
};

struct MgTensor { float *p, *acc, *vel; size_t goff; int count; };
struct TsBuf {
  unsigned char *A1, *A2, *A3, *A4, *A5, *A6, *A7, *A8;
  unsigned char *W1, *W2, *W3, *W4, *B3, *B4, *B5, *B8a, *B8b;
  float *P, *P1, *Pa, *Pb;
  float *O, *bias;
  int ldO;
  int Mpad, Lk2, Lk1, Lk3, Nk, Bk;
  int Lp;
};
struct TsShape { int NT, m_tiles, n_tiles, ksplit, ldP; size_t p_floats; };
static inline TsShape ts_shape(int rows, int cols, int chunks, int n_sm, int cluster_cap) {
  TsShape t;
  t.NT = cols > 128 ? 256 : 128;
  t.m_tiles = (rows + 127) / 128; t.n_tiles = (cols + t.NT - 1) / t.NT;
  const int tiles = t.m_tiles * t.n_tiles;
  int ks = (n_sm - 8) / tiles;
  if (ks > chunks) ks = chunks;
  if (ks < 1) ks = 1;
  if (cluster_cap > 0) {
    int p2 = 1;
    while (p2 * 2 <= ks && p2 * 2 <= cluster_cap) p2 *= 2;
    t.ksplit = p2;
  } else {
    const int cps = (chunks + ks - 1) / ks;
    t.ksplit = (chunks + cps - 1) / cps;
  }
  t.ldP = t.n_tiles * t.NT;
  t.p_floats = (size_t)t.ksplit * t.m_tiles * 128 * t.ldP;
  return t;
}

constexpr int MGS_MAXR = 8;
constexpr int MGS_FLAG_STRIDE = 32;
constexpr int MGS_GRU_CTAS = 48;
enum { MGF_ROWS = 0, MGF_APPLIED = MGS_MAXR, MGF_IN = 2 * MGS_MAXR, MGF_INAPPLIED = 3 * MGS_MAXR, MGF_DENSE = 4 * MGS_MAXR,
       MGF_COUNT = 4 * MGS_MAXR + MGS_MAXR * MGS_GRU_CTAS };
struct ShardDev {
  int R, rank, rows_local, ldW;
  int NA, DSL;
  float* W[MGS_MAXR];
  float* Wx[MGS_MAXR];
  float* inbox[MGS_MAXR];
  float* inboxIn[MGS_MAXR];
  float* denseIn[MGS_MAXR];
  float* mgInLL[MGS_MAXR];
  unsigned int* flags[MGS_MAXR];
  float *W_acc, *W_vel, *Wx_acc, *Wx_vel;
  float* mgIn;
  const int *aEnt, *aItem, *aCbeg;
  const int *xEnt, *xItem, *xTot;
  const int *gX, *gM;
  int* abort;
};
struct FastSync {
  unsigned int bar;      unsigned int p0[31];
  unsigned int stats;    unsigned int p1[31];
  unsigned int h_ready;  unsigned int p2[31];
  unsigned int b1_done;  unsigned int p3[31];
  unsigned int grp;      unsigned int p4[31];
  unsigned int in_done;  unsigned int p5[31];
  unsigned int dvec_done; unsigned int p6[31];
  unsigned int rows_done; unsigned int p7[31];
};
struct GridBar { unsigned int count; unsigned int gen; unsigned int pad[30]; };

struct LayerDev {
  int L, ldL, ld2, ld3;
  int in_dim, ld_in;
  float *Wx, *Wx_acc, *Wx_vel;
  float *Wh, *Wh_acc, *Wh_vel;
  float *Wrz, *Wrz_acc, *Wrz_vel;
  float *Bh, *Bh_acc, *Bh_vel;
  float *Wx_g, *Wh_g, *Wrz_g, *Bh_g;
  float *H;
  float *Hold, *r, *z, *ah, *ht, *y;
  float *dvec;
  float *dy;
  float *Hr;
  const float* in;
};

struct ModelDev {
  int n_items, n_layers, B, Bld, S, mode;
  int L, ldL;
  int in0_dim, ld_in0;
  int NP;
  int NCH;
  int loss; ActSpec fact, hact;
  float p_drop_h, p_drop_e, lr, mom, lmbd, bpreg, logq, alpha;
  int adapt; int nn_top1;
  float ap1, ap1c, ap2, ap2c;
  float grad_cap, smoothing;
  const float* gscale;
  float* gnorm2;
  float* stat2;
  int S_cfg;
  int export_only;
  uint32_t drop_seed;
  LayerDev layer[G4R_MAX_LAYERS];
  float *Wy, *Wy_acc, *Wy_vel; float *By, *By_acc, *By_vel;
  float *E, *E_acc, *E_vel;
  float *Sx, *in0, *dSx;
  float *snapAcc, *snapVel;
  const float *logP0t, *logP0s;
  float *O;
  float *DSY; float *DBY;
  float *part;
  float *stat;
  float *RS;
  float *cost;
  int   *nanflag;
  int CAP;
  const int *wX, *wY, *wSlot, *wM, *wSti, *wXnext; const uint8_t *wF, *wXflag; const uint32_t* wG;
  int *pItem, *pPos, *pTcol, *pCbeg;
  int* pKey;
  int shardR;
  const int* ST;
};

__device__ __forceinline__ float sigmoidf_(float x) { return 1.0f / (1.0f + expf(-x)); }

__device__ __forceinline__ float act_fwd(const ActSpec a, float x) {
  switch (a.kind) {
    case G4R_ACT_LINEAR: return x;
    case G4R_ACT_RELU: return fmaxf(x, 0.f);
    case G4R_ACT_TANH: return tanhf(x);
    case G4R_ACT_LEAKY: return x >= 0.f ? x : a.p1 * x;
    case G4R_ACT_ELU: return x >= 0.f ? x : a.p1 * (expf(x) - 1.0f);
    case G4R_ACT_SELU: return a.p1 * (x >= 0.f ? x : a.p2 * (expf(x) - 1.0f));
    default: return x;
  }
}
__device__ __forceinline__ float act_der(const ActSpec a, float x, float y) {
  switch (a.kind) {
    case G4R_ACT_LINEAR: return 1.f;
    case G4R_ACT_RELU: return x > 0.f ? 1.f : 0.f;
    case G4R_ACT_TANH: return 1.f - y * y;
    case G4R_ACT_LEAKY: return x >= 0.f ? 1.f : a.p1;
    case G4R_ACT_ELU: return x >= 0.f ? 1.f : a.p1 * expf(x);
    case G4R_ACT_SELU: return a.p1 * (x >= 0.f ? 1.f : a.p2 * expf(x));
    default: return 1.f;
  }
}

__host__ __device__ __forceinline__ uint32_t mix32(uint32_t x) {
  x ^= x >> 16; x *= 0x7feb352dU; x ^= x >> 15; x *= 0x846ca68bU; x ^= x >> 16; return x;
}
__device__ __forceinline__ float drop_scale(uint32_t seed, uint32_t gstep, uint32_t stream, uint32_t idx, float retain) {
  uint32_t k = mix32(seed ^ (0x9E3779B9U * (stream + 1U)));
  k = mix32(k + gstep);
  uint32_t r = mix32(k + idx);
  float u = (float)(r >> 8) * (1.0f / 16777216.0f);
  return u < retain ? __fdiv_rn(1.0f, retain) : 0.f;
}
#define G4R_STREAM_EMBED 100u

__device__ __forceinline__ float warp_sum(float v) {
#pragma unroll
  for (int o = 16; o > 0; o >>= 1) v += __shfl_xor_sync(0xffffffffu, v, o);
  return v;
}
// ... 1060 lines not shown
```

### gru4rec_b200/csrc/g4r_lib.cu

```cuda
#include <cuda_runtime.h>
#include <algorithm>
#include <cmath>
#include <cstdio>
#include <cstring>
#include <map>
#include <mutex>
#include <string>
#include <vector>
#include "g4r_kernels.cuh"
#include "g4r_misc.cuh"

#define G4R_VERSION 100

static thread_local std::string g_create_error;
struct g4r_handle;
static void eval_release(g4r_handle* h);
static void sessions_release(g4r_handle* h);
static void mg_release(g4r_handle* h);
static void shard_release(g4r_handle* h);
static bool shard_eligible(const g4r_config& c, int n_sm);
static int shard_create(g4r_handle* h);
static bool tc_eligible(const g4r_config& c);
struct TensorInfo;
static int shard_set_tensor(g4r_handle* h, const TensorInfo& t, const float* host);
static int shard_get_tensor(g4r_handle* h, const TensorInfo& t, float* host);
static int mgs_run_window(g4r_handle* h, int64_t n);
static int mgs_plan_window(g4r_handle* h, int64_t n);

struct TensorInfo { float* ptr; int64_t rows, cols, ld; bool sharded = false; size_t seg_off = 0; };

struct g4r_schedule {
  int B = 0, mode = 0;
  int64_t n_steps = 0, n_events = 0;
  std::vector<int32_t> X, Y, slots, M;
  std::vector<uint8_t> F;
  std::vector<int64_t> P;
  bool has_pos = false;
  int64_t max_len = 1;
  bool hist = false;
};

struct g4r_handle {
  g4r_config cfg;
  ModelDev md;
  std::string err;
  cudaStream_t stream = nullptr;
  cudaEvent_t ev0 = nullptr, ev1 = nullptr;
  char* ws = nullptr; size_t ws_bytes = 0; bool own_ws = false;
  size_t ws_off = 0;
  std::map<std::string, TensorInfo> tensors;
  int Bmax = 0, n_sm = 132;
  int CAP = 0;
  int *hX = nullptr, *hY = nullptr, *hSlot = nullptr, *hM = nullptr, *hSti = nullptr; uint8_t* hF = nullptr; uint32_t* hG = nullptr;
  float* hCost = nullptr;
  int *dX = nullptr, *dY = nullptr, *dSlot = nullptr, *dM = nullptr, *dSti = nullptr, *dXnext = nullptr; uint8_t *dF = nullptr, *dXflag = nullptr; uint32_t* dG = nullptr;
  int* dStepBase = nullptr;
  float *dP = nullptr, *dLogP0t = nullptr, *dLogP0s = nullptr, *dU = nullptr;
  int* dST = nullptr; int gen_len = 0; int64_t sample_ptr = 0; bool have_store = false; bool have_cdf = false;
  int32_t* dMrgState = nullptr; int n_streams = 0; bool mrg_init = false; int64_t mrg_rstate[6];
  float* He[G4R_MAX_LAYERS] = {};
  int* dRankCnt = nullptr; float* dTgt = nullptr;
  uint32_t global_step = 0;
  int win_steps = 0;
  int64_t launches = 0;
  int npow2 = 0;
  int slot = -1;
  cudaGraphExec_t graphU = nullptr, graph1 = nullptr; int graph_unroll = 16;
  bool use_graph = true;
  GridBar* dGridBar = nullptr; unsigned long long* dStamp = nullptr; int pk_blocks = 0; size_t pk_smem = 0;
  bool mg_alloc = false; MgDev mgdev; std::vector<MgTensor> mg_tensors;
  void* eval_ctx = nullptr;
  void* sessions = nullptr;
  uint64_t wy_version = 0;
  void* mg_host = nullptr;
  void* shard = nullptr;
  char* shard_ws = nullptr;
  size_t shard_ws_bytes = 0;
  FastSync* dFastSync = nullptr; bool fast_ok = false; bool fastc_ok = false; int fastc_grid = 0; int* hFlags = nullptr; int64_t fast_windows = 0, slow_windows = 0;
  bool prof = false; bool stamp_on = false;
  bool two_pass = false;
  bool phase_only = false;
  float* dGscale = nullptr;
  bool tc_ok = false; void* ts_buf = nullptr; unsigned long long* ts_dbg = nullptr; cudaStream_t side = nullptr, side2 = nullptr; cudaEvent_t ts_ev[12] = {};
  std::vector<cudaEvent_t> prof_ev; std::vector<int> prof_phase;
};

enum { PH_GATHER = 0, PH_F1, PH_F2, PH_SCORE, PH_STATS, PH_LOSSGRAD, PH_B1, PH_B2, PH_B3, PH_DENSE, PH_SPARSE_IN, PH_STATS2, PH_GRADCAP, PH_COUNT };
static const char* kPhaseNames[PH_COUNT] = {"gather_in", "gru_rz", "gru_h", "score", "stats", "lossgrad_update", "gru_bwd_elem", "gru_bwd_dHr", "gru_bwd_din", "dense_update", "sparse_in_update",
                                            "smoothing_stats", "grad_cap_norm_apply"};

#define LAUNCH_ON(strm, ph, ...) do { \
    cudaEvent_t e0_ = nullptr, e1_ = nullptr; \
    if (h->prof) { cudaEventCreate(&e0_); cudaEventCreate(&e1_); cudaEventRecord(e0_, (strm)); } \
    __VA_ARGS__; \
    h->launches++; \
    if (h->prof) { cudaEventRecord(e1_, (strm)); h->prof_ev.push_back(e0_); h->prof_ev.push_back(e1_); h->prof_phase.push_back(ph); } \
  } while (0)
#define LAUNCH(ph, ...) LAUNCH_ON(h->stream, ph, __VA_ARGS__)

#define CK(call) do { cudaError_t e_ = (call); if (e_ != cudaSuccess) { h->err = std::string(#call) + ": " + cudaGetErrorString(e_); return G4R_ERR_CUDA; } } while (0)
#define FAIL(code, msg) do { h->err = (msg); return (code); } while (0)

static inline int round4(int x) { return (x + 3) & ~3; }
static inline size_t align_up(size_t x, size_t a) { return (x + a - 1) / a * a; }

struct Carver {
  char* base; size_t off; bool dry;
  template <class T> T* take(size_t n) {
    off = align_up(off, 256);
    T* p = dry ? nullptr : reinterpret_cast<T*>(base + off);
    off += n * sizeof(T);
    return p;
  }
};

static int validate_config(const g4r_config& c, std::string& err) {
  if (c.n_items <= 0 || c.n_layers <= 0 || c.n_layers > G4R_MAX_LAYERS || c.batch_size <= 0) { err = "invalid sizes"; return G4R_ERR_INVALID; }
  for (int i = 0; i < c.n_layers; i++) if (c.layers[i] <= 0) { err = "invalid layer width"; return G4R_ERR_INVALID; }
  if (c.adapt < G4R_ADAPT_NONE || c.adapt > G4R_ADAPT_ADAM) { err = "adapt: unknown optimizer"; return G4R_ERR_INVALID; }
  if (c.adapt > G4R_ADAPT_ADAGRAD && c.constrained_embedding) {
    err = "adapt = rmsprop / adadelta / adam with constrained_embedding is not implemented on the device path"; return G4R_ERR_INVALID;
  }
  if (c.grad_cap < 0.f) { err = "grad_cap < 0"; return G4R_ERR_INVALID; }
  if ((c.adapt > G4R_ADAPT_ADAGRAD || c.grad_cap > 0.f || c.smoothing != 0.f) && c.world_size > 1) {
    err = "adapt other than adagrad, grad_cap and smoothing are single-GPU options"; return G4R_ERR_INVALID;
  }
  if (c.hidden_act < G4R_ACT_LINEAR || c.hidden_act > G4R_ACT_SELU) { err = "hidden_act unsupported"; return G4R_ERR_INVALID; }
  const bool elem = c.final_act >= G4R_ACT_LINEAR && c.final_act <= G4R_ACT_SELU;
  bool ok = false;
  if (c.loss == G4R_LOSS_XE && c.final_act == G4R_ACT_SOFTMAX) ok = true;
  if (c.loss == G4R_LOSS_XE_LOGIT && c.final_act == G4R_ACT_SOFTMAX_LOGIT) ok = true;
  if ((c.loss == G4R_LOSS_BPR_MAX || c.loss == G4R_LOSS_TOP1_MAX || c.loss == G4R_LOSS_BPR || c.loss == G4R_LOSS_TOP1) && elem) ok = true;
  if (!ok) { err = "loss / final_act combination not implemented on the device path"; return G4R_ERR_INVALID; }
  if (c.smoothing < 0.f) { err = "smoothing < 0"; return G4R_ERR_INVALID; }
  if (c.constrained_embedding && c.embedding) {  }
  if (c.n_sample < 0) { err = "n_sample < 0"; return G4R_ERR_INVALID; }
  return G4R_OK;
}

static int model_mode(const g4r_config& c) { return c.constrained_embedding ? 2 : (c.embedding > 0 ? 1 : 0); }

static int next_pow2(int x) { int p = 1; while (p < x) p <<= 1; return p; }

static void layout(const g4r_config& c, Carver& cv, g4r_handle* h, int n_sm) {
  const bool shard = shard_eligible(c, n_sm);
  const int mode = model_mode(c);
  const int nl = c.n_layers;
  const int B = c.batch_size;
  const int Be = c.eval_batch_size > 0 ? c.eval_batch_size : B;
  const int Bmax = std::max(B, Be);
  const int Llast = c.layers[nl - 1], ldL = round4(Llast);
  const bool mom = c.momentum > 0.f;
  const bool ada = c.adapt != G4R_ADAPT_NONE;
  const int nacc = opt_states(c.adapt);
  const int gen_len = (c.n_sample > 0 && c.sample_store > 0) ? c.sample_store / c.n_sample : 0;
  const bool store = gen_len > 1;
  const int S = store ? c.n_sample : 0;
  const int NP = round4(B + S);
  const int NCH = std::max(1, std::min(shard ? n_sm - MGS_GRU_CTAS : n_sm, (NP + 3) / 4));
  const int R = c.world_size > 1 ? c.world_size : 1;
  const int CAP = std::max(c.max_resident_steps > 0 ? c.max_resident_steps : 2048, R > 1 ? MG_CAP : 1);
  ModelDev md; memset(&md, 0, sizeof(md));
  md.n_items = c.n_items; md.n_layers = nl; md.B = B; md.Bld = round4(Bmax); md.S = S; md.mode = mode; md.L = Llast; md.ldL = ldL;
  md.NP = NP; md.NCH = NCH; md.CAP = CAP; md.S_cfg = c.n_sample; md.shardR = shard ? R : 0;
  md.loss = c.loss; md.fact = {c.final_act, c.final_act_p1, c.final_act_p2}; md.hact = {c.hidden_act, c.hidden_act_p1, c.hidden_act_p2};
  md.p_drop_h = c.dropout_p_hidden; md.p_drop_e = c.dropout_p_embed; md.lr = c.learning_rate; md.mom = c.momentum; md.lmbd = c.lmbd;
  md.bpreg = c.bpreg; md.logq = c.logq; md.alpha = c.sample_alpha; md.adapt = c.adapt;
  md.ap1 = c.adapt_p1; md.ap1c = c.adapt_p1c; md.ap2 = c.adapt_p2; md.ap2c = c.adapt_p2c; md.grad_cap = c.grad_cap;
  md.smoothing = (c.loss == G4R_LOSS_XE || c.loss == G4R_LOSS_XE_LOGIT) ? c.smoothing : 0.f;
  md.drop_seed = c.dropout_seed + (c.world_size > 1 ? (uint32_t)c.rank * 0x9E3779B1u : 0u);
  md.in0_dim = mode == 2 ? Llast : (mode == 1 ? c.embedding : 0);
  md.ld_in0 = round4(md.in0_dim);
  auto reg = [&](const std::string& name, float* p, int64_t rows, int64_t cols, int64_t ld) { if (!cv.dry) h->tensors[name] = TensorInfo{p, rows, cols, ld}; };
  auto table3 = [&](const std::string& name, int64_t rows, int64_t cols, float** p, float** a, float** v, int64_t ld_override = 0) {
    const int64_t ld = ld_override > 0 ? ld_override : round4((int)cols);
    *p = cv.take<float>((size_t)rows * ld); reg(name, *p, rows, cols, ld);
    *a = ada ? cv.take<float>((size_t)rows * ld * nacc) : nullptr; if (ada) reg(name + ".acc", *a, rows, cols, ld);
    if (nacc > 1) reg(name + (c.adapt == G4R_ADAPT_ADAM ? ".meang" : ".upd"), *a + (size_t)rows * ld, rows, cols, ld);
    if (nacc > 2) reg(name + ".countt", *a + 2 * (size_t)rows * ld, rows, cols, ld);
    *v = mom ? cv.take<float>((size_t)rows * ld) : nullptr; if (mom) reg(name + ".vel", *v, rows, cols, ld);
  };
  if (!shard) {
    table3("Wy", c.n_items, Llast, &md.Wy, &md.Wy_acc, &md.Wy_vel);
    table3("By", c.n_items, 1, &md.By, &md.By_acc, &md.By_vel, 1);
  }
  if (mode == 1) table3("E", c.n_items, c.embedding, &md.E, &md.E_acc, &md.E_vel);
  for (int i = 0; i < nl; i++) {
    LayerDev& ly = md.layer[i];
    const int L = c.layers[i];
    ly.L = L; ly.ldL = round4(L); ly.ld2 = round4(2 * L); ly.ld3 = round4(3 * L);
    int in_rows;
    if (i == 0) { in_rows = mode == 0 ? c.n_items : md.in0_dim; ly.in_dim = mode == 0 ? 0 : md.in0_dim; ly.ld_in = md.ld_in0; }
    else { in_rows = c.layers[i - 1]; ly.in_dim = c.layers[i - 1]; ly.ld_in = round4(c.layers[i - 1]); }
    const std::string si = std::to_string(i);
    if (!(shard && i == 0)) table3("Wx" + si, in_rows, 3 * L, &ly.Wx, &ly.Wx_acc, &ly.Wx_vel);
    table3("Wh" + si, L, L, &ly.Wh, &ly.Wh_acc, &ly.Wh_vel);
    table3("Wrz" + si, L, 2 * L, &ly.Wrz, &ly.Wrz_acc, &ly.Wrz_vel);
    table3("Bh" + si, 1, 3 * L, &ly.Bh, &ly.Bh_acc, &ly.Bh_vel);
    ly.H = cv.take<float>((size_t)B * ly.ldL); reg("H" + si, ly.H, B, L, ly.ldL);
    float* he = cv.take<float>((size_t)Be * ly.ldL); if (!cv.dry) h->He[i] = he;
    reg("He" + si, he, Be, L, ly.ldL);
    ly.Hold = cv.take<float>((size_t)Bmax * ly.ldL); ly.r = cv.take<float>((size_t)Bmax * ly.ldL); ly.z = cv.take<float>((size_t)Bmax * ly.ldL);
    ly.ah = cv.take<float>((size_t)Bmax * ly.ldL); ly.ht = cv.take<float>((size_t)Bmax * ly.ldL); ly.y = cv.take<float>((size_t)Bmax * ly.ldL);
    ly.dvec = cv.take<float>((size_t)Bmax * ly.ld3); ly.dy = cv.take<float>((size_t)Bmax * ly.ldL); ly.Hr = cv.take<float>((size_t)Bmax * ly.ldL);
    reg("y" + si, ly.y, Bmax, L, ly.ldL); reg("dvec" + si, ly.dvec, Bmax, 3 * L, ly.ld3);
  }
  if (mode != 0) {
    md.Sx = cv.take<float>((size_t)Bmax * md.ld_in0); md.in0 = cv.take<float>((size_t)Bmax * md.ld_in0); md.dSx = cv.take<float>((size_t)Bmax * md.ld_in0);
    if (mode == 2) { md.snapAcc = cv.take<float>((size_t)Bmax * md.ld_in0); md.snapVel = cv.take<float>((size_t)Bmax * md.ld_in0); }
    reg("dSx", md.dSx, Bmax, md.in0_dim, md.ld_in0);
  }
  for (int i = 0; i < nl; i++) md.layer[i].in = (i == 0) ? md.in0 : md.layer[i - 1].y;
  md.O = cv.take<float>((size_t)NP * md.Bld);
  md.DSY = cv.take<float>((size_t)NP * ldL); md.DBY = cv.take<float>((size_t)NP);
  md.part = cv.take<float>((size_t)NCH * B * ldL);
  md.stat = cv.take<float>((size_t)NCH * B * G4R_NSTAT);
  md.RS = cv.take<float>((size_t)Bmax * G4R_NSTAT);
  md.stat2 = md.smoothing > 0.f ? cv.take<float>((size_t)NCH * B * 2) : nullptr;
  float* gsc = c.grad_cap > 0.f ? cv.take<float>(8) : nullptr;
  md.gscale = gsc;
  md.cost = cv.take<float>((size_t)CAP);
  md.nanflag = cv.take<int>(4);
  reg("O", md.O, NP, Bmax, md.Bld); reg("DSY", md.DSY, NP, Llast, ldL);
  int* dX = cv.take<int>((size_t)CAP * B); int* dY = cv.take<int>((size_t)CAP * B); int* dSlot = cv.take<int>((size_t)CAP * B);
  int* dXnext = cv.take<int>((size_t)CAP * B);
  uint8_t* dF = cv.take<uint8_t>((size_t)CAP * B); uint8_t* dXflag = cv.take<uint8_t>((size_t)CAP * B);
  int* dM = cv.take<int>(CAP); int* dSti = cv.take<int>(CAP); uint32_t* dG = cv.take<uint32_t>(CAP);
  md.pItem = cv.take<int>((size_t)CAP * NP); md.pPos = cv.take<int>((size_t)CAP * NP);
  md.pTcol = cv.take<int>((size_t)CAP * B); md.pCbeg = cv.take<int>((size_t)CAP * (NCH + 1));
  md.pKey = shard ? cv.take<int>((size_t)CAP * NP) : nullptr;
  int* dStepBase = cv.take<int>(4);
  GridBar* dGridBar = cv.take<GridBar>(1);
  FastSync* dFastSync = cv.take<FastSync>(1);
  unsigned long long* dStamp = cv.take<unsigned long long>((size_t)CAP * 16);
  float* dP = cv.take<float>(c.n_items); float* dL0t = cv.take<float>(c.n_items); float* dL0s = cv.take<float>(c.n_items);
  int* dST = store ? cv.take<int>((size_t)gen_len * c.n_sample) : nullptr;
  float* dU = store ? cv.take<float>((size_t)gen_len * c.n_sample) : nullptr;
  int32_t* dMrg = cv.take<int32_t>((size_t)15360 * 6);
  MgDev mgd; memset(&mgd, 0, sizeof(mgd));
  std::vector<MgTensor> mgt;
  const bool twins = R > 1 || c.grad_cap > 0.f;
  if (twins) {
    size_t cnt = 0;
    for (int i = 0; i < nl; i++) {
      const LayerDev& ly = md.layer[i];
      if (ly.in_dim > 0) cnt += (size_t)ly.in_dim * ly.ld3;
      cnt += (size_t)ly.L * ly.ldL + (size_t)ly.L * ly.ld2 + ly.ld3;
    }
    float* gf = cv.take<float>(cnt);
    size_t off = 0;
    for (int i = 0; i < nl; i++) {
      LayerDev& ly = md.layer[i];
      if (ly.in_dim > 0) { ly.Wx_g = gf ? gf + off : nullptr; mgt.push_back(MgTensor{ly.Wx, ly.Wx_acc, ly.Wx_vel, off, ly.in_dim * ly.ld3}); off += (size_t)ly.in_dim * ly.ld3; }
      ly.Wh_g = gf ? gf + off : nullptr; mgt.push_back(MgTensor{ly.Wh, ly.Wh_acc, ly.Wh_vel, off, ly.L * ly.ldL}); off += (size_t)ly.L * ly.ldL;
      ly.Wrz_g = gf ? gf + off : nullptr; mgt.push_back(MgTensor{ly.Wrz, ly.Wrz_acc, ly.Wrz_vel, off, ly.L * ly.ld2}); off += (size_t)ly.L * ly.ld2;
      ly.Bh_g = gf ? gf + off : nullptr; mgt.push_back(MgTensor{ly.Bh, ly.Bh_acc, ly.Bh_vel, off, ly.ld3}); off += ly.ld3;
    }
    mgd.R = R; mgd.rank = c.rank; mgd.gradFlat = gf; mgd.gradCount = cnt;
  }
  if (R > 1) {
    mgd.gItem = cv.take<int>((size_t)R * MG_CAP * NP); mgd.gPos = nullptr;
    mgd.gM = cv.take<int>((size_t)R * MG_CAP); mgd.gX = cv.take<int>((size_t)R * MG_CAP * B);
    mgd.mEnt = cv.take<int>((size_t)MG_CAP * R * NP); mgd.mItem = cv.take<int>((size_t)MG_CAP * R * NP);
    mgd.mCbeg = cv.take<int>((size_t)MG_CAP * (n_sm + 1)); mgd.mTot = cv.take<int>(MG_CAP);
    mgd.xEnt = cv.take<int>((size_t)MG_CAP * R * B); mgd.xItem = cv.take<int>((size_t)MG_CAP * R * B); mgd.xTot = cv.take<int>(MG_CAP);
    if (!shard) {
      const int in_ld = mode == 0 ? md.layer[0].ld3 : md.ld_in0;
      mgd.DSYall = cv.take<float>((size_t)R * NP * ldL); mgd.DBYall = cv.take<float>((size_t)R * NP); mgd.INall = cv.take<float>((size_t)R * B * in_ld);
    }
  }
  char* shard_ws = nullptr; size_t shard_ws_bytes = 0;
  if (shard) {
    shard_ws_bytes = (size_t)2 * MG_CAP * R * sizeof(int) + 4096 + (size_t)B * md.layer[0].ld3 * sizeof(float) + 1024;
    shard_ws = cv.take<char>(shard_ws_bytes);
  }
  TsBuf tsb; memset(&tsb, 0, sizeof(tsb));
  const bool tc = tc_eligible(c);
  if (tc) {
    auto r32 = [](int x) { return (x + 31) / 32 * 32; };
    auto r128 = [](int x) { return (x + 127) / 128 * 128; };
    const int L = Llast;
    tsb.Mpad = r128(B); tsb.Lk1 = r32(L); tsb.Lk2 = r32(2 * L); tsb.Lk3 = r32(3 * L); tsb.Nk = r128(NP); tsb.Bk = r32(B);
    tsb.ldO = tsb.Nk;
    auto op = [&](int rows, int K) { return cv.take<unsigned char>((size_t)((rows + 255) / 256 * 256) * K * 8); };
    tsb.Lp = (L + 255) / 256 * 256;
    tsb.A1 = op(B, tsb.Lk2); tsb.A2 = op(B, tsb.Lk2); tsb.A3 = op(B, tsb.Lk1); tsb.A4 = op(NP, tsb.Bk); tsb.A5 = op(B, tsb.Nk);
    tsb.A6 = op(B, tsb.Lk1); tsb.A7 = op(B, tsb.Lk3); tsb.A8 = op(3 * L, tsb.Bk);
    tsb.W1 = op(2 * L, tsb.Lk2); tsb.W2 = op(L, tsb.Lk2); tsb.W3 = op(L, tsb.Lk1); tsb.W4 = op(L, tsb.Lk3);
    tsb.B3 = op(NP, tsb.Lk1); tsb.B4 = op(L, tsb.Bk); tsb.B5 = op(L, tsb.Nk); tsb.B8a = op(2 * tsb.Lp, tsb.Bk); tsb.B8b = op(L, tsb.Bk);
    size_t pf = 0;
    for (const TsShape& t : {ts_shape(B, 2 * L, tsb.Lk2 / 32, n_sm, 16), ts_shape(B, L, tsb.Lk2 / 32, n_sm, 16), ts_shape(B, NP, tsb.Lk1 / 32, n_sm, 16),
                             ts_shape(B, L, tsb.Nk / 32, n_sm, 16), ts_shape(B, L, tsb.Lk1 / 32, n_sm, 16), ts_shape(B, L, tsb.Lk3 / 32, n_sm, 16)}) pf = std::max(pf, t.p_floats);
    tsb.P = cv.take<float>(pf);
    tsb.P1 = cv.take<float>(ts_shape(tsb.Nk, L, tsb.Bk / 32, n_sm, 16).p_floats);
    tsb.Pa = cv.take<float>(ts_shape(3 * L, 2 * tsb.Lp, tsb.Bk / 32, n_sm, 0).p_floats);
    tsb.Pb = cv.take<float>(ts_shape(3 * L, L, tsb.Bk / 32, n_sm, 0).p_floats);
    tsb.O = cv.take<float>((size_t)tsb.Mpad * tsb.ldO); tsb.bias = cv.take<float>(tsb.Nk);
  }
  int* dRank = cv.take<int>((size_t)Be * 4); float* dTgt = cv.take<float>((size_t)Be * 3);
  if (!cv.dry) {
    md.wX = dX; md.wY = dY; md.wSlot = dSlot; md.wM = dM; md.wSti = dSti; md.wXnext = dXnext; md.wF = dF; md.wXflag = dXflag; md.wG = dG;
    md.ST = dST; md.logP0t = dL0t; md.logP0s = dL0s;
    h->md = md; h->Bmax = Bmax; h->CAP = CAP; h->mg_alloc = R > 1; h->mgdev = mgd; h->mg_tensors = mgt; h->gen_len = store ? gen_len : 0;
    h->dX = dX; h->dY = dY; h->dSlot = dSlot; h->dM = dM; h->dSti = dSti; h->dXnext = dXnext; h->dF = dF; h->dXflag = dXflag; h->dG = dG;
    h->dGridBar = dGridBar; h->dStamp = dStamp; h->dFastSync = dFastSync;
    h->dStepBase = dStepBase; h->dP = dP; h->dLogP0t = dL0t; h->dLogP0s = dL0s; h->dST = dST; h->dU = dU; h->dMrgState = dMrg;
    h->dRankCnt = dRank; h->dTgt = dTgt;
    h->npow2 = next_pow2(B + S);
    h->shard_ws = shard_ws; h->shard_ws_bytes = shard_ws_bytes;
    h->tc_ok = tc;
    if (tc) { if (!h->ts_buf) h->ts_buf = new TsBuf(); *static_cast<TsBuf*>(h->ts_buf) = tsb; }
    h->dGscale = gsc; h->two_pass = c.grad_cap > 0.f; h->phase_only = c.grad_cap > 0.f || md.smoothing > 0.f;
  }
}

#define G4R_MAX_SLOTS 24
__constant__ ModelDev c_models[G4R_MAX_SLOTS];
static bool g_slot_used[G4R_MAX_SLOTS] = {};
static std::mutex g_slot_mutex;
static int slot_alloc() { std::lock_guard<std::mutex> lk(g_slot_mutex); for (int i = 0; i < G4R_MAX_SLOTS; i++) if (!g_slot_used[i]) { g_slot_used[i] = true; return i; } return -1; }
static void slot_free(int i) { std::lock_guard<std::mutex> lk(g_slot_mutex); if (i >= 0 && i < G4R_MAX_SLOTS) g_slot_used[i] = false; }
static cudaError_t slot_upload(int slot, const ModelDev& md, cudaStream_t st) {
  return cudaMemcpyToSymbolAsync(c_models, &md, sizeof(ModelDev), (size_t)slot * sizeof(ModelDev), cudaMemcpyHostToDevice, st);
}
#define MD (c_models[slot])
#define STEP_IDX (base ? (*base + off) : off)
__global__ void __launch_bounds__(256) k_gather_in(int slot, const int* base, int off, int train) { phase_gather_in(MD, STEP_IDX, train != 0, blockIdx.x, gridDim.x); }
__global__ void __launch_bounds__(GEMM_THREADS) k_f1(int slot, const int* base, int off, int li, float* Hsrc) {
  __shared__ float sA[GK * (GB + 1)], sB[GK * (GB + 1)];
  phase_f1(MD, li, STEP_IDX, Hsrc, blockIdx.x, sA, sB);
}
__global__ void __launch_bounds__(GEMM_THREADS) k_f2(int slot, const int* base, int off, int li, float* Hsrc, int train) {
  __shared__ float sA[GK * (GB + 1)], sB[GK * (GB + 1)];
  phase_f2(MD, li, STEP_IDX, Hsrc, train != 0, blockIdx.x, sA, sB);
}
__global__ void __launch_bounds__(SC_THREADS) k_score(int slot, const int* base, int off) {
  extern __shared__ __align__(16) float smem[];
  phase_score(MD, STEP_IDX, blockIdx.x, smem);
}
__global__ void __launch_bounds__(256) k_stats(int slot, const int* base, int off) {
  extern __shared__ __align__(16) float smem[];
  phase_stats(MD, STEP_IDX, blockIdx.x, gridDim.x, smem);
}
__global__ void __launch_bounds__(SC_THREADS) k_lossgrad(int slot, const int* base, int off) {
  extern __shared__ __align__(16) float smem[];
  phase_lossgrad(MD, STEP_IDX, blockIdx.x, smem);
}
__global__ void __launch_bounds__(256) k_b1(int slot, const int* base, int off, int li, int nch) { phase_b1(MD, li, STEP_IDX, blockIdx.x, gridDim.x, nch); }
__global__ void __launch_bounds__(GEMM_THREADS) k_b2(int slot, const int* base, int off, int li) {
  __shared__ float sA[GK * (GB + 1)], sB[GK * (GB + 1)];
  phase_b2(MD, li, STEP_IDX, blockIdx.x, sA, sB);
}
__global__ void __launch_bounds__(GEMM_THREADS) k_b3(int slot, const int* base, int off, int li) {
  __shared__ float sA[GK * (GB + 1)], sB[GK * (GB + 1)];
  phase_b3(MD, li, STEP_IDX, blockIdx.x, sA, sB);
}
__global__ void __launch_bounds__(GEMM_THREADS) k_dense(int slot, const int* base, int off, int li) {
  __shared__ float sA[GK * (GB + 1)], sB[GK * (GB + 1)];
  phase_dense(MD, li, STEP_IDX, blockIdx.x, sA, sB);
}
__global__ void __launch_bounds__(128) k_sparse_in(int slot, const int* base, int off, int apply_pass) { phase_sparse_in(MD, STEP_IDX, blockIdx.x, apply_pass != 0); }
__global__ void __launch_bounds__(256) k_stats2a(int slot, const int* base, int off) { phase_stats2a(MD, STEP_IDX, blockIdx.x); }
__global__ void __launch_bounds__(256) k_stats2b(int slot, const int* base, int off) {
  __shared__ float smem[64];
  phase_stats2b(MD, STEP_IDX, blockIdx.x, gridDim.x, smem);
}
__global__ void __launch_bounds__(1024) k_gradnorm(int slot, const int* base, int off, const float* dense_flat, size_t dense_count, float* gscale) {
  __shared__ float smem[32];
  phase_gradnorm(MD, STEP_IDX, dense_flat, dense_count, gscale, smem);
}
__global__ void __launch_bounds__(SC_THREADS) k_apply_rows(int slot, const int* base, int off) { phase_apply_rows(MD, STEP_IDX, blockIdx.x); }
__global__ void __launch_bounds__(256) k_apply_dense(int slot, float* p, float* acc, float* vel, const float* g, int n) {
  const int i = blockIdx.x * blockDim.x + threadIdx.x;
  if (i < n) dense_update(MD, p + i, acc ? acc + i : nullptr, vel ? vel + i : nullptr, g[i], (size_t)n);
}
__global__ void k_advance(int* base, int n) { if (threadIdx.x == 0 && blockIdx.x == 0) *base += n; }

#include "g4r_persistent.cuh"
#include "g4r_fast.cuh"

static bool fast_shape(const g4r_config& c, int n_sm) {
  const int L = c.layers[0], ldL = round4(L);
  const bool smoothing = (c.loss == G4R_LOSS_XE || c.loss == G4R_LOSS_XE_LOGIT) && c.smoothing > 0.f;
  return c.step_mode == 2 && c.adapt <= G4R_ADAPT_ADAGRAD && !(c.grad_cap > 0.f) && !smoothing && model_mode(c) == 0 && c.n_layers == 1 &&
         ldL <= 128 && c.batch_size <= FK_B && 2 * L <= FK_W1 * FK_G && L <= FK_W2 * FK_G && n_sm >= FK_G + 1 &&
         n_sm - ldL / 4 >= c.batch_size && !tc_eligible(c) && !shard_eligible(c, n_sm);
}

// ... 713 lines not shown
extern "C" int g4r_schedule_positions(const g4r_schedule* s, int64_t* pos) {
  if (!s || !pos) return G4R_ERR_INVALID;
  if (!s->has_pos) { g_create_error = "g4r_schedule_positions: the schedule was not built with mode 1 | G4R_SCHED_POSITIONS"; return G4R_ERR_STATE; }
  memcpy(pos, s->P.data(), s->P.size() * sizeof(int64_t));
  return G4R_OK;
}

static int64_t stage_window(g4r_handle* h, const g4r_schedule* s, int64_t first, int64_t n) {
  const int B = h->md.B;
  n = std::min<int64_t>(n, h->CAP);
  const bool store = h->gen_len > 0;
  if (store && h->sample_ptr >= h->gen_len) return 0;
  if (store) n = std::min<int64_t>(n, h->gen_len - h->sample_ptr);
  memcpy(h->hX, s->X.data() + first * B, (size_t)n * B * sizeof(int));
  memcpy(h->hY, s->Y.data() + first * B, (size_t)n * B * sizeof(int));
  memcpy(h->hSlot, s->slots.data() + first * B, (size_t)n * B * sizeof(int));
  memcpy(h->hF, s->F.data() + first * B, (size_t)n * B);
  memcpy(h->hM, s->M.data() + first, (size_t)n * sizeof(int));
  for (int64_t i = 0; i < n; i++) {
    h->hSti[i] = store ? (int)(h->sample_ptr + i) : -1;
    h->hG[i] = h->global_step + (uint32_t)i;
  }
  return n;
}

static int validate_window(g4r_handle* h, int64_t n) {
  const int B = h->md.B, I = h->md.n_items;
  for (int64_t i = 0; i < n; i++) {
    const int M = h->hM[i];
    if (M <= 0 || M > B) FAIL(G4R_ERR_INVALID, "batch size out of range");
    for (int b = 0; b < M; b++) {
      const int x = h->hX[i * B + b], y = h->hY[i * B + b], sl = h->hSlot[i * B + b];
      if (x < 0 || x >= I || y < 0 || y >= I) FAIL(G4R_ERR_INDEX, "Index out of bounds");
      if (sl < 0 || sl >= B) FAIL(G4R_ERR_INDEX, "lane slot out of bounds");
    }
  }
  return G4R_OK;
}

static int upload_window(g4r_handle* h, int64_t n) {
  const int B = h->md.B;
  int rc = validate_window(h, n);
  if (rc) return rc;
  if (h->gen_len > 0 && !h->have_store) FAIL(G4R_ERR_STATE, "sample store not generated");
  cudaStream_t st = h->stream;
  CK(cudaMemcpyAsync(h->dX, h->hX, (size_t)n * B * sizeof(int), cudaMemcpyHostToDevice, st));
  CK(cudaMemcpyAsync(h->dY, h->hY, (size_t)n * B * sizeof(int), cudaMemcpyHostToDevice, st));
  CK(cudaMemcpyAsync(h->dSlot, h->hSlot, (size_t)n * B * sizeof(int), cudaMemcpyHostToDevice, st));
  CK(cudaMemcpyAsync(h->dF, h->hF, (size_t)n * B, cudaMemcpyHostToDevice, st));
  CK(cudaMemcpyAsync(h->dM, h->hM, (size_t)n * sizeof(int), cudaMemcpyHostToDevice, st));
  CK(cudaMemcpyAsync(h->dSti, h->hSti, (size_t)n * sizeof(int), cudaMemcpyHostToDevice, st));
  CK(cudaMemcpyAsync(h->dG, h->hG, (size_t)n * sizeof(uint32_t), cudaMemcpyHostToDevice, st));
  CK(cudaMemsetAsync(h->md.nanflag + 2, 0, sizeof(int), st));
  k_plan<<<(unsigned)n, 256, (size_t)h->npow2 * 8 + 1024, st>>>(h->md, h->dXnext, h->dXflag, h->npow2);
  h->launches++;
  CK(cudaGetLastError());
  h->win_steps = (int)n;
  if (h->shard) return mgs_plan_window(h, n);
  return G4R_OK;
}

static int build_graph(g4r_handle* h, int unroll, cudaGraphExec_t* out) {
  cudaGraph_t g = nullptr;
  CK(cudaStreamBeginCapture(h->stream, cudaStreamCaptureModeThreadLocal));
  const int64_t l0 = h->launches;
  for (int i = 0; i < unroll; i++) enqueue_train_step(h, h->dStepBase, i);
  k_advance<<<1, 32, 0, h->stream>>>(h->dStepBase, unroll);
  h->launches = l0;
  CK(cudaStreamEndCapture(h->stream, &g));
  CK(cudaGraphInstantiate(out, g, 0));
  cudaGraphDestroy(g);
  return G4R_OK;
}
static int64_t launches_per_step(const g4r_handle* h) {
  const ModelDev& md = h->md;
  if (h->tc_ok) return 25;
  int64_t n = (md.mode != 0 ? 1 : 0) + 4;
  for (int li = 0; li < md.n_layers; li++) n += 2 + 2 + (md.layer[li].in_dim > 0 ? 1 : 0) + 1;
  if (md.smoothing > 0.f) n += 2;
  if (h->two_pass) n += 3 + (int64_t)h->mg_tensors.size();
  return n;
}

static int run_window(g4r_handle* h, int64_t n) {
  bool fast = false, fastc = false;
  if ((h->cfg.step_mode == 3 && h->fastc_ok) || (h->cfg.step_mode == 2 && h->fast_ok)) {
    if (!h->prof) {
      CK(cudaMemcpyAsync(h->hFlags, h->md.nanflag, 4 * sizeof(int), cudaMemcpyDeviceToHost, h->stream));
      CK(cudaStreamSynchronize(h->stream));
      const bool fits = h->hFlags[2] <= FK_CT;
      fastc = fits && h->cfg.step_mode == 3;
      fast = fits && h->cfg.step_mode == 2;
    }
  }
  if (fastc) {
    int slot = h->slot, nst = (int)n; FastSync* fsp = h->dFastSync; unsigned long long* ts = h->stamp_on ? h->dStamp : nullptr;
    void* args[] = {&slot, &nst, &fsp, &ts};
    CK(cudaMemsetAsync(h->dFastSync, 0, sizeof(FastSync), h->stream));
    CK(fastc_launch(h->fastc_grid, h->stream, args));
    h->launches += 1; h->fast_windows++;
  } else if (fast) {
    int slot = h->slot, nst = (int)n; FastSync* fsp = h->dFastSync; unsigned long long* ts = h->stamp_on ? h->dStamp : nullptr;
    void* args[] = {&slot, &nst, &fsp, &ts};
    CK(cudaMemsetAsync(h->dFastSync, 0, sizeof(FastSync), h->stream));
    CK(cudaLaunchCooperativeKernel((void*)k_fast_t<false>, dim3(h->pk_blocks), dim3(FK_THREADS), args, sizeof(FastSmemR), h->stream));
    h->launches += 1; h->fast_windows++;
  } else if (h->cfg.step_mode >= 1 && !h->prof && h->pk_blocks > 0 && !h->phase_only && !h->tc_ok) {
    if (h->cfg.step_mode >= 2) h->slow_windows++;
    int slot = h->slot, nst = (int)n; GridBar* gb = h->dGridBar; unsigned long long* ts = h->stamp_on ? h->dStamp : nullptr;
    void* args[] = {&slot, &nst, &gb, &ts};
    CK(cudaMemsetAsync(h->dGridBar, 0, sizeof(GridBar), h->stream));
    CK(cudaLaunchCooperativeKernel((void*)k_persistent, dim3(h->pk_blocks), dim3(PK_THREADS), args, h->pk_smem, h->stream));
    h->launches += 1;
  } else if (h->prof || !h->use_graph) {
    for (int64_t i = 0; i < n; i++) enqueue_train_step(h, nullptr, (int)i);
  } else {
    if (!h->graphU) { int rc = build_graph(h, h->graph_unroll, &h->graphU); if (rc) return rc; rc = build_graph(h, 1, &h->graph1); if (rc) return rc; }
    CK(cudaMemsetAsync(h->dStepBase, 0, sizeof(int), h->stream));
    int64_t i = 0;
    for (; i + h->graph_unroll <= n; i += h->graph_unroll) CK(cudaGraphLaunch(h->graphU, h->stream));
    for (; i < n; i++) CK(cudaGraphLaunch(h->graph1, h->stream));
    h->launches += n * launches_per_step(h) + (n / h->graph_unroll) + (n % h->graph_unroll);
  }
  CK(cudaGetLastError());
  if (h->gen_len > 0) h->sample_ptr += n;
  h->global_step += (uint32_t)n;
  return G4R_OK;
}

#include "g4r_multi.cuh"
#include "g4r_shard.cuh"
static bool mg_is_ready(g4r_handle* h) { return h->mg_host && static_cast<MgHost*>(h->mg_host)->ready; }

extern "C" int g4r_upload_steps(g4r_handle* h, const g4r_schedule* s, int64_t first, int64_t n) {
  if (!h || !s) return G4R_ERR_INVALID;
  if (h->shard && n > MG_CAP) FAIL(G4R_ERR_INVALID, "row-sharded handle: at most MG_CAP steps per uploaded window");
  if (s->B != h->md.B) FAIL(G4R_ERR_INVALID, "schedule batch size != model batch size");
  if (first < 0 || n <= 0 || first + n > s->n_steps) FAIL(G4R_ERR_INVALID, "step range out of schedule");
  if (n > h->CAP) FAIL(G4R_ERR_INVALID, "n exceeds the resident window capacity");
  cudaSetDevice(h->cfg.device);
  if (h->gen_len > 0 && h->sample_ptr + n > h->gen_len) FAIL(G4R_ERR_STATE, "window would wrap the sample store; regenerate or shorten");
  const int64_t got = stage_window(h, s, first, n);
  if (got != n) FAIL(G4R_ERR_STATE, "could not stage the window");
  return upload_window(h, n);
}

extern "C" int g4r_run_uploaded(g4r_handle* h, float* cost_out, float* device_ms) {
  if (!h) return G4R_ERR_INVALID;
  if (h->win_steps <= 0) FAIL(G4R_ERR_STATE, "no uploaded window");
  cudaSetDevice(h->cfg.device);
  h->wy_version++;
  const int n = h->win_steps;
  if (h->cfg.world_size > 1 && !mg_is_ready(h)) FAIL(G4R_ERR_STATE, "multi-GPU handle: call g4r_mg_init first");
  if (h->cfg.world_size > 1 && !h->shard) FAIL(G4R_ERR_STATE, "g4r_run_uploaded on a multi-GPU handle needs the row-sharded path");
  CK(cudaEventRecord(h->ev0, h->stream));
  int rc = h->shard ? mgs_run_window(h, n) : run_window(h, n);
  if (rc) return rc;
  CK(cudaEventRecord(h->ev1, h->stream));
  if (cost_out) CK(cudaMemcpyAsync(h->hCost, h->md.cost, (size_t)n * sizeof(float), cudaMemcpyDeviceToHost, h->stream));
  if (h->shard) CK(cudaMemcpyAsync(h->hFlags, h->md.nanflag, 4 * sizeof(int), cudaMemcpyDeviceToHost, h->stream));
  CK(cudaStreamSynchronize(h->stream));
  if (h->shard && h->hFlags[3]) FAIL(G4R_ERR_STATE, "multi-GPU: a cross-GPU wait timed out (a peer rank stopped or never started its window)");
  if (cost_out) memcpy(cost_out, h->hCost, (size_t)n * sizeof(float));
  if (device_ms) CK(cudaEventElapsedTime(device_ms, h->ev0, h->ev1));
  return G4R_OK;
}

extern "C" int g4r_profile_uploaded(g4r_handle* h, float* phase_ms, int32_t* phase_launches, int32_t n_phases) {
  if (!h || !phase_ms || !phase_launches || n_phases < PH_COUNT) return G4R_ERR_INVALID;
  if (h->shard) FAIL(G4R_ERR_STATE, "per-phase profiling is a single-GPU measurement (row-sharded handle)");
  if (h->win_steps <= 0) FAIL(G4R_ERR_STATE, "no uploaded window");
  cudaSetDevice(h->cfg.device);
  h->wy_version++;
  h->prof = true; h->prof_ev.clear(); h->prof_phase.clear();
  int rc = run_window(h, h->win_steps);
  h->prof = false;
  if (rc) return rc;
  CK(cudaStreamSynchronize(h->stream));
  for (int i = 0; i < n_phases; i++) { phase_ms[i] = 0.f; phase_launches[i] = 0; }
  for (size_t k = 0; k < h->prof_phase.size(); k++) {
    float ms = 0.f;
    cudaEventElapsedTime(&ms, h->prof_ev[2 * k], h->prof_ev[2 * k + 1]);
    phase_ms[h->prof_phase[k]] += ms; phase_launches[h->prof_phase[k]]++;
    cudaEventDestroy(h->prof_ev[2 * k]); cudaEventDestroy(h->prof_ev[2 * k + 1]);
  }
  h->prof_ev.clear(); h->prof_phase.clear();
  return G4R_OK;
}
extern "C" int g4r_persistent_stamps(g4r_handle* h, int32_t enable, unsigned long long* out, int64_t n_steps) {
  if (!h) return G4R_ERR_INVALID;
  h->stamp_on = enable != 0;
  if (out && n_steps > 0) {
    if (n_steps > h->CAP) FAIL(G4R_ERR_INVALID, "n_steps exceeds window capacity");
    cudaSetDevice(h->cfg.device);
    CK(cudaMemcpyAsync(out, h->dStamp, (size_t)n_steps * 16 * sizeof(unsigned long long), cudaMemcpyDeviceToHost, h->stream));
    CK(cudaStreamSynchronize(h->stream));
  }
  return G4R_OK;
}
extern "C" int g4r_uses_tensor_cores(const g4r_handle* h) { return (h && h->tc_ok) ? 1 : 0; }
extern "C" int64_t g4r_fast_windows(const g4r_handle* h, int64_t* fallback_windows) {
  if (!h) return 0;
  if (fallback_windows) *fallback_windows = h->slow_windows;
  return h->fast_windows;
}
extern "C" const char* g4r_phase_name(int32_t i) { return (i >= 0 && i < PH_COUNT) ? kPhaseNames[i] : ""; }
extern "C" int g4r_phase_count(void) { return PH_COUNT; }

extern "C" int g4r_train_steps(g4r_handle* h, const g4r_schedule* s, int64_t first, int64_t n, float* cost_out, int64_t* nan_step) {
  if (!h || !s) return G4R_ERR_INVALID;
  if (s->B != h->md.B) FAIL(G4R_ERR_INVALID, "schedule batch size != model batch size");
  if (first < 0 || n < 0 || first + n > s->n_steps) FAIL(G4R_ERR_INVALID, "step range out of schedule");
  cudaSetDevice(h->cfg.device);
  h->wy_version++;
  if (nan_step) *nan_step = -1;
  int64_t done = 0;
  while (done < n) {
    if (h->gen_len > 0 && (!h->have_store || h->sample_ptr >= h->gen_len)) {
      int rc = g4r_generate_samples(h);
      if (rc) return rc;
    }
    const bool multi = h->cfg.world_size > 1;
    const int64_t w = stage_window(h, s, first + done, multi ? std::min<int64_t>(n - done, MG_CAP) : n - done);
    if (w <= 0) FAIL(G4R_ERR_STATE, "empty window");
    int rc = upload_window(h, w);
    if (rc) return rc;
    if (multi) {
      if (!mg_is_ready(h)) FAIL(G4R_ERR_STATE, "multi-GPU handle: call g4r_mg_init first");
      rc = h->shard ? mgs_run_window(h, w) : mg_run_window(h, w);
    } else rc = run_window(h, w);
    if (rc) return rc;
    CK(cudaMemcpyAsync(h->hCost, h->md.cost, (size_t)w * sizeof(float), cudaMemcpyDeviceToHost, h->stream));
    if (h->shard) CK(cudaMemcpyAsync(h->hFlags, h->md.nanflag, 4 * sizeof(int), cudaMemcpyDeviceToHost, h->stream));
    CK(cudaStreamSynchronize(h->stream));
    if (h->shard && h->hFlags[3]) FAIL(G4R_ERR_STATE, "multi-GPU: a cross-GPU wait timed out (a peer rank stopped or never started its window)");
    for (int64_t i = 0; i < w; i++) {
      if (cost_out) cost_out[done + i] = h->hCost[i];
      if (h->hCost[i] != h->hCost[i]) {
        if (nan_step) *nan_step = first + done + i;
        FAIL(G4R_ERR_NAN, "NaN error!");
      }
    }
    done += w;
  }
  return G4R_OK;
}

extern "C" int g4r_train_step(g4r_handle* h, const int32_t* X, const int32_t* Y, int32_t M, const int8_t* R, float* cost) {
  if (!h || !X || !Y) return G4R_ERR_INVALID;
  const int B = h->md.B;
  if (M <= 0 || M > B) FAIL(G4R_ERR_INVALID, "M out of range");
  if (h->shard) FAIL(G4R_ERR_STATE, "g4r_train_step: not available on a row-sharded multi-GPU handle (use g4r_train_steps)");
  cudaSetDevice(h->cfg.device);
  h->wy_version++;
  if (h->gen_len > 0 && (!h->have_store || h->sample_ptr >= h->gen_len)) {
    int rc = g4r_generate_samples(h);
    if (rc) return rc;
  }
  for (int b = 0; b < B; b++) {
    h->hX[b] = b < M ? X[b] : -1; h->hY[b] = b < M ? Y[b] : -1; h->hSlot[b] = b;
    h->hF[b] = (b < M && R && R[b]) ? 1 : 0;
  }
  h->hM[0] = M; h->hSti[0] = h->gen_len > 0 ? (int)h->sample_ptr : -1; h->hG[0] = h->global_step;
  int rc = upload_window(h, 1);
  if (rc) return rc;
  rc = run_window(h, 1);
  if (rc) return rc;
  CK(cudaMemcpyAsync(h->hCost, h->md.cost, sizeof(float), cudaMemcpyDeviceToHost, h->stream));
  CK(cudaStreamSynchronize(h->stream));
  if (cost) *cost = h->hCost[0];
  if (h->hCost[0] != h->hCost[0]) FAIL(G4R_ERR_NAN, "NaN error!");
  return G4R_OK;
}

#include "g4r_eval.cuh"
```

### gru4rec_b200/csrc/g4r_shard.cuh

```cuda
#pragma once

constexpr unsigned long long MGS_TIMEOUT_NS = 4000000000ull;

__device__ __forceinline__ unsigned int ld_acquire_sys_u32(const unsigned int* p) {
  unsigned int v;
  asm volatile("ld.acquire.sys.global.u32 %0, [%1];" : "=r"(v) : "l"(p) : "memory");
  return v;
}
__device__ __forceinline__ void st_release_sys_u32(unsigned int* p, unsigned int v) {
  asm volatile("st.release.sys.global.u32 [%0], %1;" :: "l"(p), "r"(v) : "memory");
}
__device__ __forceinline__ float4 ld_volatile4(const float* p) {
  float4 v;
  asm volatile("ld.volatile.global.v4.f32 {%0, %1, %2, %3}, [%4];" : "=f"(v.x), "=f"(v.y), "=f"(v.z), "=f"(v.w) : "l"(p) : "memory");
  return v;
}
__device__ __forceinline__ unsigned long long mgs_timer() {
  unsigned long long t;
  asm volatile("mov.u64 %0, %%globaltimer;" : "=l"(t));
  return t;
}
__device__ __forceinline__ void wait_sys_ge(const unsigned int* p, unsigned int target, int* abort) {
  if ((int)(ld_acquire_sys_u32(p) - target) >= 0) return;
  const unsigned long long t0 = mgs_timer();
  unsigned int spins = 0;
  while ((int)(ld_acquire_sys_u32(p) - target) < 0) {
    if ((++spins & 127u) == 0) {
      if (*(volatile int*)abort) return;
      if (mgs_timer() - t0 > MGS_TIMEOUT_NS) { atomicExch(abort, 1); return; }
    }
  }
}
__device__ __forceinline__ void mgs_wait_flags(const ShardDev& sh, int first, int skip, unsigned int target) {
  if (threadIdx.x < 32) {
    const int q = threadIdx.x;
    if (q < sh.R && q != skip) wait_sys_ge(sh.flags[sh.rank] + (size_t)(first + q) * MGS_FLAG_STRIDE, target, sh.abort);
    __syncwarp();
  }
}
__device__ __forceinline__ void ll_store4(float* dst_pairs, float4 v, unsigned int seq) {
  asm volatile("st.volatile.global.v4.u32 [%0], {%1, %2, %3, %4};" :: "l"(dst_pairs), "r"(__float_as_uint(v.x)), "r"(seq), "r"(__float_as_uint(v.y)), "r"(seq) : "memory");
  asm volatile("st.volatile.global.v4.u32 [%0], {%1, %2, %3, %4};" :: "l"(dst_pairs + 4), "r"(__float_as_uint(v.z)), "r"(seq), "r"(__float_as_uint(v.w)), "r"(seq) : "memory");
}
__device__ __forceinline__ float4 ll_load4(const float* src_pairs, unsigned int seq, int* abort) {
  uint4 a, b;
  unsigned int spins = 0; unsigned long long t0 = 0;
  while (true) {
    asm volatile("ld.volatile.global.v4.u32 {%0, %1, %2, %3}, [%4];" : "=r"(a.x), "=r"(a.y), "=r"(a.z), "=r"(a.w) : "l"(src_pairs) : "memory");
    asm volatile("ld.volatile.global.v4.u32 {%0, %1, %2, %3}, [%4];" : "=r"(b.x), "=r"(b.y), "=r"(b.z), "=r"(b.w) : "l"(src_pairs + 4) : "memory");
    if (a.y == seq && a.w == seq && b.y == seq && b.w == seq) break;
    if ((++spins & 127u) == 0) {
      if (*(volatile int*)abort) break;
      const unsigned long long t = mgs_timer();
      if (t0 == 0) t0 = t;
      if (t - t0 > MGS_TIMEOUT_NS) { atomicExch(abort, 1); break; }
    }
  }
  return make_float4(__uint_as_float(a.x), __uint_as_float(a.z), __uint_as_float(b.x), __uint_as_float(b.z));
}
__device__ __forceinline__ float ll_load1(const float* src_pair, unsigned int seq, int* abort) {
  uint2 a;
  unsigned int spins = 0; unsigned long long t0 = 0;
  while (true) {
    asm volatile("ld.volatile.global.v2.u32 {%0, %1}, [%2];" : "=r"(a.x), "=r"(a.y) : "l"(src_pair) : "memory");
    if (a.y == seq) break;
    if ((++spins & 127u) == 0) {
      if (*(volatile int*)abort) break;
      const unsigned long long t = mgs_timer();
      if (t0 == 0) t0 = t;
      if (t - t0 > MGS_TIMEOUT_NS) { atomicExch(abort, 1); break; }
    }
  }
  return __uint_as_float(a.x);
}
__device__ __forceinline__ void wait_ge_abortable(const unsigned int* p, unsigned int target, int* abort) {
  unsigned int spins = 0;
  while (ld_acquire_u32(p) < target) { if ((++spins & 1023u) == 0 && *(volatile int*)abort) return; }
}

struct FastSmemMG : FastSmem {
  ShardDev sh;
  int sOw[2][FK_CT], sLoc[2][FK_CT], sYow[2][FK_B], sYloc[2][FK_B];
};
struct FastSyncMG {
  unsigned int exp_done;   unsigned int p0[31];
  unsigned int apply_done; unsigned int p1[31];
  unsigned int h1;         unsigned int p2[31];
  unsigned int h2;         unsigned int p3[31];
};

__device__ __forceinline__ void fk_load_idx_mg(const ModelDev& md, FastSmemMG& sm, int s, int n_steps, int chunk, int buf) {
  const int tid = threadIdx.x;
  if (s >= n_steps) return;
  const int M = md.wM[s], R = sm.sh.R;
  const int* cbeg = md.pCbeg + (size_t)s * (md.NCH + 1);
  const bool hc = chunk < md.NCH;
  const int cb = hc ? cbeg[chunk] : 0, ce = hc ? cbeg[chunk + 1] : 0;
  if (tid < FK_CT) {
    int it = 0, pos = 0;
    if (cb + tid < ce) { it = md.pItem[(size_t)s * md.NP + cb + tid]; pos = md.pPos[(size_t)s * md.NP + cb + tid]; }
    sm.sIt[buf][tid] = it; sm.sPos[buf][tid] = pos;
    sm.sOw[buf][tid] = it % R; sm.sLoc[buf][tid] = it / R;
  }
  if (tid >= 32 && tid < 32 + FK_B) {
    const int b = tid - 32;
    const int y = b < M ? md.wY[(size_t)s * md.B + b] : 0;
    sm.sTc[buf][b] = b < M ? md.pTcol[(size_t)s * md.B + b] : -1;
    sm.sYit[buf][b] = y; sm.sYow[buf][b] = y % R; sm.sYloc[buf][b] = y / R;
  }
  if (tid == 64) { sm.sCb[buf][0] = cb; sm.sCb[buf][1] = ce; }
}

__device__ __forceinline__ void fk_prefetch_mg(const ModelDev& md, FastSmemMG& sm, int s, int n_steps, int buf, bool pw) {
  if (s >= n_steps) return;
  const int tid = threadIdx.x;
  const int M = md.wM[s];
  const int nj = sm.sCb[buf][1] - sm.sCb[buf][0];
  const int ldW = sm.sh.ldW;
  const unsigned int rowb = (unsigned int)ldW * 4u;
  uint64_t* bar = reinterpret_cast<uint64_t*>(&sm.mbar);
  const int ncopy = nj + (pw ? M : 0);
  if (tid == 0) {
    const unsigned int total = rowb * (unsigned int)ncopy;
    if (total > 0) mbar_expect_tx(bar, total);
    else asm volatile("mbarrier.arrive.shared::cta.b64 _, [%0];" :: "r"(smem_u32(bar)) : "memory");
  }
  if ((tid & 31) == 0) {
    asm volatile("fence.proxy.async.global;" ::: "memory");
    for (int i = tid >> 5; i < ncopy; i += FK_NW) {
      if (i < nj) tma_row(sm.sS + i * FK_LDS, sm.sh.W[sm.sOw[buf][i]] + (size_t)sm.sLoc[buf][i] * ldW, rowb, bar);
      else { const int b = i - nj; tma_row(sm.sTW + b * FK_LDS, sm.sh.W[sm.sYow[buf][b]] + (size_t)sm.sYloc[buf][b] * ldW, rowb, bar); }
    }
  }
}

__device__ void mgs_apply_rows(const ModelDev& md, FastSmemMG& sm, int s, int a, int par, unsigned int T) {
  const ShardDev& sh = sm.sh;
  const int R = sh.R, ldW = sh.ldW, nq = ldW / 4;
  const int lane = threadIdx.x & 31, warp = threadIdx.x >> 5;
  const int* cbeg = sh.aCbeg + (size_t)s * (sh.NA + 1);
  const int cb = cbeg[a], ce = cbeg[a + 1];
  const int* ent = sh.aEnt + (size_t)s * R * md.NP;
  const int* it = sh.aItem + (size_t)s * R * md.NP;
  const bool ada = md.adapt == G4R_ADAPT_ADAGRAD, mom = md.mom > 0.f;
  const float* inb = sh.inbox[sh.rank] + (size_t)par * R * md.NP * ldW * 2;
  float* W = sh.W[sh.rank];
  for (int j = cb + warp; j < ce; j += FK_NW) {
    const int item = it[j];
    if (j > cb && it[j - 1] == item) continue;
    int je = j + 1;
    while (je < ce && it[je] == item) je++;
    const size_t ro = (size_t)(item / R) * ldW;
    for (int q4 = lane; q4 < nq; q4 += 32) {
      const float4 z = make_float4(0.f, 0.f, 0.f, 0.f), p0 = ld4(W + ro + q4 * 4);
      RowChain<float4> u;
      u.begin(p0, p0, ada ? ld4(sh.W_acc + ro + q4 * 4) : z, mom ? ld4(sh.W_vel + ro + q4 * 4) : z);
      for (int k = j; k < je; k++) {
        const int e = ent[k];
        u.add(md, ll_load4(inb + (((size_t)(e >> 20) * md.NP + (size_t)(e & 0xfffff)) * ldW + q4 * 4) * 2, T, sh.abort), ada, mom);
      }
// ... 802 lines not shown
```

### include/g4r.h

```cpp
#ifndef G4R_H
#define G4R_H
#include <stddef.h>
#include <stdint.h>

#ifdef __cplusplus
extern "C" {
#endif

#define G4R_MAX_LAYERS 8

typedef enum {
  G4R_OK = 0,
  G4R_ERR_INVALID = -1,
  G4R_ERR_INDEX = -2,
  G4R_ERR_CUDA = -3,
  G4R_ERR_NAN = -4,
  G4R_ERR_STATE = -5
} g4r_status;

typedef enum { G4R_LOSS_XE = 0, G4R_LOSS_BPR_MAX = 1, G4R_LOSS_TOP1_MAX = 2, G4R_LOSS_BPR = 3, G4R_LOSS_TOP1 = 4,
               G4R_LOSS_XE_LOGIT = 5 } g4r_loss;
typedef enum { G4R_ACT_LINEAR = 0, G4R_ACT_RELU = 1, G4R_ACT_TANH = 2, G4R_ACT_LEAKY = 3, G4R_ACT_ELU = 4,
               G4R_ACT_SELU = 5, G4R_ACT_SOFTMAX = 6, G4R_ACT_SOFTMAX_LOGIT = 7 } g4r_act;
typedef enum { G4R_ADAPT_NONE = 0, G4R_ADAPT_ADAGRAD = 1, G4R_ADAPT_RMSPROP = 2, G4R_ADAPT_ADADELTA = 3, G4R_ADAPT_ADAM = 4 } g4r_adapt;

typedef struct g4r_config {
  int32_t n_items;
  int32_t n_layers;
  int32_t layers[G4R_MAX_LAYERS];
  int32_t batch_size;
  int32_t embedding;
  int32_t constrained_embedding;
  int32_t loss;
  int32_t final_act;
  float final_act_p1, final_act_p2;
  int32_t hidden_act;
  float hidden_act_p1, hidden_act_p2;
  float dropout_p_hidden, dropout_p_embed;
  float learning_rate, momentum, lmbd;
  int32_t n_sample;
  float sample_alpha;
  float smoothing, bpreg, logq;
  int32_t adapt;
  int32_t sample_store;
  uint32_t dropout_seed;
  uint32_t mrg_seed;
  int32_t max_resident_steps;
  int32_t device;
  int32_t world_size, rank;
  int32_t eval_batch_size;
  int32_t step_mode;
  int32_t mg_replicated;
  int32_t eval_tc;
  float adapt_p1, adapt_p1c;
  float adapt_p2, adapt_p2c;
  float grad_cap;
} g4r_config;

typedef struct g4r_handle g4r_handle;
typedef struct g4r_schedule g4r_schedule;

int g4r_version(void);
int g4r_workspace_bytes(const g4r_config* cfg, size_t* bytes);
int g4r_create(const g4r_config* cfg, void* device_workspace, size_t workspace_bytes, g4r_handle** out);
int g4r_destroy(g4r_handle* h);
const char* g4r_last_error(const g4r_handle* h);
void* g4r_stream(g4r_handle* h);

int g4r_tensor_shape(g4r_handle* h, const char* name, int64_t* rows, int64_t* cols);
int g4r_set_tensor(g4r_handle* h, const char* name, const float* host, int64_t rows, int64_t cols);
int g4r_get_tensor(g4r_handle* h, const char* name, float* host, int64_t rows, int64_t cols);
int g4r_reset_hidden(g4r_handle* h);

int g4r_set_sampling_cdf(g4r_handle* h, const float* P, int64_t n);
int g4r_set_logq_support(g4r_handle* h, const float* P0, int64_t n);
int g4r_generate_samples(g4r_handle* h);
int g4r_generate_samples_from_uniform(g4r_handle* h, const float* u, int64_t n);
int g4r_set_sample_store(g4r_handle* h, const int64_t* st, int64_t rows);
int g4r_get_sample_store(g4r_handle* h, int64_t* st, int64_t rows);
int g4r_sample_store_rows(g4r_handle* h);
int g4r_set_sample_pointer(g4r_handle* h, int64_t p);
int64_t g4r_get_sample_pointer(g4r_handle* h);
int g4r_mrg_uniform(g4r_handle* h, float* out, int64_t n);

int g4r_searchsorted(g4r_handle* h, const float* d, int64_t n_d, const float* x, int64_t n_x, int64_t* y);
int g4r_gather_rows(g4r_handle* h, const float* table, int64_t rows, int64_t cols, const int64_t* idx, int64_t n_idx, float* out);

int g4r_schedule_build(const int64_t* data_items, int64_t n_events, const int32_t* offset_sessions, int64_t n_sessions,
                       const int64_t* session_order, int32_t batch_size, int32_t n_sample, int32_t mode, g4r_schedule** out);
int g4r_schedule_free(g4r_schedule* s);
int64_t g4r_schedule_steps(const g4r_schedule* s);
int64_t g4r_schedule_events(const g4r_schedule* s);
int g4r_schedule_export(const g4r_schedule* s, int32_t* X, int32_t* Y, uint8_t* flags, int32_t* M, int32_t* slots);
#define G4R_SCHED_POSITIONS 2
int g4r_schedule_positions(const g4r_schedule* s, int64_t* pos);
int g4r_schedule_build_history(const int64_t* data_items, int64_t n_events, const int32_t* offset_sessions, int64_t n_sessions,
                               const int64_t* session_order, const int32_t* n_history, int32_t batch_size, int32_t mode, g4r_schedule** out);

int g4r_train_step(g4r_handle* h, const int32_t* X, const int32_t* Y, int32_t M, const int8_t* R, float* cost);
int g4r_train_steps(g4r_handle* h, const g4r_schedule* s, int64_t first, int64_t n, float* cost_out, int64_t* nan_step);
int g4r_upload_steps(g4r_handle* h, const g4r_schedule* s, int64_t first, int64_t n);
int g4r_run_uploaded(g4r_handle* h, float* cost_out , float* device_ms );
int g4r_profile_uploaded(g4r_handle* h, float* phase_ms, int32_t* phase_launches, int32_t n_phases);
const char* g4r_phase_name(int32_t i);
int64_t g4r_fast_windows(const g4r_handle* h, int64_t* fallback_windows);
int g4r_uses_tensor_cores(const g4r_handle* h);
int g4r_persistent_stamps(g4r_handle* h, int32_t enable, unsigned long long* out, int64_t n_steps);
int g4r_phase_count(void);
int64_t g4r_kernel_launches(const g4r_handle* h);

int g4r_mg_unique_id(char* out128);
int g4r_mg_init(g4r_handle* h, const char* id128);
int g4r_mg_sharded(const g4r_handle* h);
int g4r_mg_ipc_handle(g4r_handle* h, char* out64);
int g4r_mg_ipc_open(g4r_handle* h, const char* handles, int32_t world);
int g4r_mg_owner(int64_t item, int32_t world);
int64_t g4r_mg_local_row(int64_t item, int32_t world);
int64_t g4r_mg_shard_rows(int64_t n_items, int32_t world, int32_t rank);
int g4r_mg_segment_bytes(const g4r_config* cfg, size_t* total, size_t* inbox_bytes, size_t* inbox_in_bytes, size_t* dense_bytes);

int g4r_eval_schedule(g4r_handle* h, const g4r_schedule* s, const int32_t* cut_off, int32_t n_cut, int32_t mode,
                      double* recall_sum, double* mrr_sum, int64_t* n_events);
int g4r_eval_counts(g4r_handle* h, int32_t* out, int64_t n_lanes);
int g4r_set_eval_items(g4r_handle* h, const int64_t* items, int64_t n);
int g4r_set_eval_exclude_seen(g4r_handle* h, int32_t on);
int g4r_eval_events(g4r_handle* h, const g4r_schedule* s, const int32_t* cut_off, int32_t n_cut, int32_t mode, int32_t k,
                    double* recall_sum, double* mrr_sum, int64_t* n_events, int32_t* out_counts, int32_t* out_items, float* out_scores);

int g4r_predict(g4r_handle* h, const int32_t* X, int32_t batch, const uint8_t* reset_mask, float* out);
#define G4R_TOPK_MAX 1024
int g4r_predict_topk(g4r_handle* h, const int32_t* X, int32_t batch, const uint8_t* reset_mask, int32_t k,
                     int32_t* out_items, float* out_scores);
int g4r_predict_topk_filtered(g4r_handle* h, const int32_t* X, int32_t batch, const uint8_t* reset_mask, int32_t k,
                              const int32_t* cand, int64_t n_cand, const int64_t* excl_off, const int32_t* excl_items,
                              int32_t* out_items, float* out_scores);
int g4r_reset_eval_hidden(g4r_handle* h);

int g4r_sessions_open(g4r_handle* h, int64_t capacity);
int64_t g4r_sessions_count(const g4r_handle* h, int64_t* n_history_items);
int g4r_sessions_feed(g4r_handle* h, const int64_t* keys, const int32_t* X, int64_t n);
int g4r_sessions_topk(g4r_handle* h, const int64_t* keys, const int32_t* X, int64_t n, int32_t k,
                      const int32_t* cand, int64_t n_cand, const int64_t* excl_off, const int32_t* excl_items,
                      int32_t exclude_seen, int32_t* out_items, float* out_scores);
int g4r_sessions_end(g4r_handle* h, const int64_t* keys, int64_t n);
int g4r_sessions_export(g4r_handle* h, int64_t* keys, float* states, int64_t* hist_off, int32_t* hist_items);
int g4r_sessions_import(g4r_handle* h, const int64_t* keys, const float* states, const int64_t* hist_off,
                        const int32_t* hist_items, int64_t n);

#ifdef __cplusplus
}
#endif
#endif
```

Before: 32060.

## Replace counter barriers with sequence-tagged LL pair buffers in fast training kernel

Inter-CTA exchanges in the step_mode 2 persistent kernel (Hr, y, partial sums, backward deltas) now go through double-buffered value/sequence pair buffers written with volatile stores. Consumers poll the tags instead of waiting on group barriers and counter flags. This is meant to remove group-barrier round trips and fence latency per step. In exchange it doubles the bytes moved, adds a timeout/abort path with a host flag readback, and adds poison and sequence APIs for testing.

```diff
diff --git a/gru4rec_b200/_lib.py b/gru4rec_b200/_lib.py
--- a/gru4rec_b200/_lib.py
+++ b/gru4rec_b200/_lib.py
@@ -39,7 +39,7 @@
     'g4r_mrg_uniform', 'g4r_searchsorted', 'g4r_gather_rows',
     'g4r_schedule_build', 'g4r_schedule_build_history', 'g4r_schedule_free', 'g4r_schedule_steps', 'g4r_schedule_events', 'g4r_schedule_export', 'g4r_schedule_positions',
     'g4r_train_step', 'g4r_train_steps', 'g4r_upload_steps', 'g4r_run_uploaded', 'g4r_kernel_launches',
-    'g4r_profile_uploaded', 'g4r_phase_name', 'g4r_phase_count', 'g4r_persistent_stamps', 'g4r_fast_windows', 'g4r_uses_tensor_cores', 'g4r_mg_unique_id', 'g4r_mg_init',
+    'g4r_profile_uploaded', 'g4r_phase_name', 'g4r_phase_count', 'g4r_persistent_stamps', 'g4r_fast_windows', 'g4r_fast_poison', 'g4r_fast_sequence', 'g4r_uses_tensor_cores', 'g4r_mg_unique_id', 'g4r_mg_init',
     'g4r_mg_sharded', 'g4r_mg_ipc_handle', 'g4r_mg_ipc_open', 'g4r_mg_owner', 'g4r_mg_local_row', 'g4r_mg_shard_rows', 'g4r_mg_segment_bytes',
     'g4r_eval_schedule', 'g4r_eval_events', 'g4r_eval_counts', 'g4r_set_eval_items', 'g4r_set_eval_exclude_seen', 'g4r_predict', 'g4r_reset_eval_hidden',
     'g4r_predict_topk', 'g4r_predict_topk_filtered',
@@ -98,6 +98,8 @@
     lib.g4r_phase_count.restype = C.c_int
     lib.g4r_persistent_stamps.argtypes = [vp, i32, vp, i64]
     lib.g4r_fast_windows.argtypes = [vp, C.POINTER(i64)]; lib.g4r_fast_windows.restype = i64
+    lib.g4r_fast_poison.argtypes = [vp, C.c_uint32]
+    lib.g4r_fast_sequence.argtypes = [vp]; lib.g4r_fast_sequence.restype = i64
     lib.g4r_uses_tensor_cores.argtypes = [vp]
     lib.g4r_mg_unique_id.argtypes = [vp]
     lib.g4r_mg_init.argtypes = [vp, vp]
@@ -488,6 +490,12 @@
         n = self.lib.g4r_fast_windows(self.h, C.byref(fb))
         return n, fb.value
 
+    def fast_sequence(self):
+        return self.lib.g4r_fast_sequence(self.h)
+
+    def fast_poison(self, tag):
+        self._check(self.lib.g4r_fast_poison(self.h, tag))
+
     def kernel_launches(self):
         return self.lib.g4r_kernel_launches(self.h)
 
diff --git a/gru4rec_b200/csrc/g4r_fast.cuh b/gru4rec_b200/csrc/g4r_fast.cuh
--- a/gru4rec_b200/csrc/g4r_fast.cuh
+++ b/gru4rec_b200/csrc/g4r_fast.cuh
@@ -20,6 +20,93 @@
 }
 __device__ __forceinline__ void wait_ge(const unsigned int* p, unsigned int target) {
   while (ld_acquire_u32(p) < target) { }
+}
+
+constexpr unsigned long long LL_TIMEOUT_NS = 4000000000ull;
+__device__ __forceinline__ unsigned long long ll_timer() {
+  unsigned long long t;
+  asm volatile("mov.u64 %0, %%globaltimer;" : "=l"(t));
+  return t;
+}
+__device__ __forceinline__ void ll_store4(float* dst_pairs, float4 v, unsigned int seq) {
+  asm volatile("st.volatile.global.v4.u32 [%0], {%1, %2, %3, %4};" :: "l"(dst_pairs), "r"(__float_as_uint(v.x)), "r"(seq), "r"(__float_as_uint(v.y)), "r"(seq) : "memory");
+  asm volatile("st.volatile.global.v4.u32 [%0], {%1, %2, %3, %4};" :: "l"(dst_pairs + 4), "r"(__float_as_uint(v.z)), "r"(seq), "r"(__float_as_uint(v.w)), "r"(seq) : "memory");
+}
+__device__ __forceinline__ void ll_store1(float* dst_pair, float v, unsigned int seq) {
+  asm volatile("st.volatile.global.v2.u32 [%0], {%1, %2};" :: "l"(dst_pair), "r"(__float_as_uint(v)), "r"(seq) : "memory");
+}
+__device__ __forceinline__ bool ll_give_up(unsigned int& spins, unsigned long long& t0, int* abort) {
+  if ((++spins & 127u) != 0) return false;
+  if (*(volatile int*)abort) return true;
+  const unsigned long long t = ll_timer();
+  if (t0 == 0) t0 = t;
+  if (t - t0 > LL_TIMEOUT_NS) { atomicExch(abort, 1); return true; }
+  return false;
+}
+__device__ __forceinline__ void ll_ld4(uint4& a, uint4& b, const float* src_pairs) {
+  asm volatile("ld.volatile.global.v4.u32 {%0, %1, %2, %3}, [%4];" : "=r"(a.x), "=r"(a.y), "=r"(a.z), "=r"(a.w) : "l"(src_pairs) : "memory");
+  asm volatile("ld.volatile.global.v4.u32 {%0, %1, %2, %3}, [%4];" : "=r"(b.x), "=r"(b.y), "=r"(b.z), "=r"(b.w) : "l"(src_pairs + 4) : "memory");
+}
+__device__ __forceinline__ uint2 ll_ld1(const float* src_pair) {
+  uint2 a;
+  asm volatile("ld.volatile.global.v2.u32 {%0, %1}, [%2];" : "=r"(a.x), "=r"(a.y) : "l"(src_pair) : "memory");
+  return a;
+}
+__device__ __forceinline__ bool ll_tags4(const uint4& a, const uint4& b, unsigned int seq) { return a.y == seq && a.w == seq && b.y == seq && b.w == seq; }
+__device__ __forceinline__ float4 ll_val4(const uint4& a, const uint4& b) {
+  return make_float4(__uint_as_float(a.x), __uint_as_float(a.z), __uint_as_float(b.x), __uint_as_float(b.z));
+}
+__device__ __forceinline__ float4 ll_load4(const float* src_pairs, unsigned int seq, int* abort) {
+  uint4 a, b;
+  unsigned int spins = 0; unsigned long long t0 = 0;
+  while (true) {
+    ll_ld4(a, b, src_pairs);
+    if (ll_tags4(a, b, seq) || ll_give_up(spins, t0, abort)) break;
+  }
+  return ll_val4(a, b);
+}
+__device__ __forceinline__ float ll_load1(const float* src_pair, unsigned int seq, int* abort) {
+  uint2 a;
+  unsigned int spins = 0; unsigned long long t0 = 0;
+  while (true) {
+    a = ll_ld1(src_pair);
+    if (a.y == seq || ll_give_up(spins, t0, abort)) break;
+  }
+  return __uint_as_float(a.x);
+}
+template <int N>
+__device__ __forceinline__ void ll_load_n(float (&v)[N], const float* src, size_t stride, int n, unsigned int seq, int* abort) {
+  uint2 p[N];
+#pragma unroll
+  for (int i = 0; i < N; i++) { p[i] = make_uint2(0u, seq); if (i < n) p[i] = ll_ld1(src + i * stride); }
+#pragma unroll
+  for (int i = 0; i < N; i++) v[i] = p[i].y == seq ? __uint_as_float(p[i].x) : ll_load1(src + i * stride, seq, abort);
+}
+__device__ __forceinline__ void ll_stage_rows(float* dst, const float* src, int ldp, int M, int kw, unsigned int seq, int* abort) {
+  const int n = FK_B * kw;
+  for (int i0 = 0; i0 < n; i0 += 2 * FK_THREADS) {
+    uint4 a[2], b[2];
+    bool on[2];
+#pragma unroll
+    for (int u = 0; u < 2; u++) {
+      const int i = i0 + u * FK_THREADS + (int)threadIdx.x, rr = i / kw;
+      on[u] = i < n && rr < M;
+      a[u] = b[u] = make_uint4(0u, seq, 0u, seq);
+      if (on[u]) ll_ld4(a[u], b[u], src + ((size_t)rr * ldp + (i % kw) * 4) * 2);
+    }
+#pragma unroll
+    for (int u = 0; u < 2; u++) {
+      const int i = i0 + u * FK_THREADS + (int)threadIdx.x;
+      if (i >= n) continue;
+      float4 v = ll_val4(a[u], b[u]);
+      if (!ll_tags4(a[u], b[u], seq)) v = ll_load4(src + ((size_t)(i / kw) * ldp + (i % kw) * 4) * 2, seq, abort);
+      st4(dst + (i / kw) * FK_LDS + (i % kw) * 4, v);
+    }
+  }
+}
+__device__ __forceinline__ void wait_ge_abortable(const unsigned int* p, unsigned int target, int* abort) {
+  unsigned int spins = 0;
+  while (ld_acquire_u32(p) < target) { if ((++spins & 1023u) == 0 && *(volatile int*)abort) return; }
 }
 __device__ __forceinline__ uint32_t smem_u32(const void* p) { return (uint32_t)__cvta_generic_to_shared(p); }
 __device__ __forceinline__ void mbar_init(uint64_t* bar, unsigned int count) {
@@ -139,10 +226,10 @@
   }
 }
 
-__device__ __forceinline__ void fk_group_barrier(FastSync* fs, unsigned int& gepoch, unsigned int G = FK_G) {
+__device__ __forceinline__ void fk_group_barrier(FastSync* fs, unsigned int& gepoch) {
   __syncthreads();
   gepoch += 1;
-  if (threadIdx.x == 0) { red_release_add(&fs->grp, 1u); wait_ge(&fs->grp, gepoch * G); }
+  if (threadIdx.x == 0) { red_release_add(&fs->grp, 1u); wait_ge(&fs->grp, gepoch * FK_G); }
   __syncthreads();
 }
 
@@ -327,7 +414,7 @@
 }
 
 template <class SM>
-__device__ void fk_sparse_in_one(const ModelDev& md, SM& sm, int s, int b, const unsigned int* ctr, unsigned int target) {
+__device__ void fk_sparse_in_one(const ModelDev& md, SM& sm, int s, int b, const unsigned int* ctr, unsigned int target, int* abort = nullptr) {
   const LayerDev& ly = md.layer[0];
   const int M = md.wM[s], ld3 = ly.ld3, tid = threadIdx.x;
   const bool act = b < M && (md.wXflag[(size_t)s * md.B + b] & 1);
@@ -346,7 +433,7 @@
     if (ada) a0 = ld4(ly.Wx_acc + (size_t)item * ld3 + c4 * 4);
     if (mom) v0 = ld4(ly.Wx_vel + (size_t)item * ld3 + c4 * 4);
   }
-  if (tid == 0) wait_ge(ctr, target);
+  if (tid == 0) { if (abort) wait_ge_abortable(ctr, target, abort); else wait_ge(ctr, target); }
   __syncthreads();
   if (mine) {
     const int nmem = sm.gIdx[FK_B];
@@ -359,8 +446,8 @@
   }
 }
 
-template <bool CL, class SM>
-__device__ void fk_b1(const ModelDev& md, SM& sm, int s, int cta, int ncta) {
+template <bool CL, bool LL = false, class SM>
+__device__ void fk_b1(const ModelDev& md, SM& sm, int s, int cta, int ncta, const float* partp = nullptr, float* dap = nullptr, unsigned int T = 0, int* abort = nullptr) {
   const LayerDev& ly = md.layer[0];
   const int M = md.wM[s], L = ly.L, ldL = ly.ldL;
   const int tid = threadIdx.x, lane = tid & 31, warp = tid >> 5;
@@ -379,8 +466,11 @@
     float d = 0.f;
     if (e < E) {
       float v[10];
-#pragma unroll
-      for (int u = 0; u < 10; u++) { const int ch = warp + FK_NW * u; v[u] = ch < md.NCH ? md.part[(size_t)ch * cs + e] : 0.f; }
+      if (LL) ll_load_n<10>(v, partp + ((size_t)warp * cs + e) * 2, (size_t)FK_NW * cs * 2, (md.NCH - warp + FK_NW - 1) / FK_NW, T, abort);
+      else {
+#pragma unroll
+        for (int u = 0; u < 10; u++) { const int ch = warp + FK_NW * u; v[u] = ch < md.NCH ? md.part[(size_t)ch * cs + e] : 0.f; }
+      }
       d = (((v[0] + v[1]) + (v[2] + v[3])) + ((v[4] + v[5]) + (v[6] + v[7]))) + (v[8] + v[9]);
     }
     red[warp * per + eb + lane] = d;
@@ -390,6 +480,8 @@
     const int e = e0 + i;
     if (e >= E) continue;
     const int b = e / ldL, c = e % ldL;
+    float* da = dap + ((size_t)b * 2 * ldL + c) * 2;
+    if (LL && c >= L) { ll_store1(da, 0.f, T); ll_store1(da + 2 * ldL, 0.f, T); continue; }
     if (c >= L) continue;
     float dy = 0.f;
 #pragma unroll
@@ -401,6 +493,7 @@
     if (md.p_drop_h > 0.f) dh *= drop_scale(md.drop_seed, md.wG[s], 0u, (uint32_t)(b * L + c), 1.0f - md.p_drop_h);
     const float dz = dh * (ht - ho);
     const float dah = dh * z * act_der(md.hact, ah, ht);
+    if (LL) { ll_store1(da, dah, T); ll_store1(da + 2 * ldL, dz * z * (1.f - z), T); continue; }
     ly.dvec[(size_t)b * ly.ld3 + c] = dah;
     ly.dvec[(size_t)b * ly.ld3 + 2 * L + c] = dz * z * (1.f - z);
   }
@@ -487,7 +580,8 @@
   }
 }
 
-__device__ void fr_f1(const ModelDev& md, FastSmemR& sm, int s, int k0, const float* sH, const unsigned int* wait_ctr, unsigned int wait_target) {
+__device__ void fr_f1(const ModelDev& md, FastSmemR& sm, int s, int k0, const float* sH, const unsigned int* wait_ctr, unsigned int wait_target,
+                      float* hrp, unsigned int T, int* abort) {
   const LayerDev& ly = md.layer[0];
   const int M = md.wM[s], L = ly.L, ldL = ly.ldL, tid = threadIdx.x;
   if (tid == 0) sm.sFlag[3] = (!wait_ctr || ld_acquire_u32(wait_ctr) >= wait_target) ? 1 : 0;
@@ -504,7 +598,7 @@
   fk_slab_dot<2 * FR_U>(acc, sH, FK_LDS, sm.rC[0] + FR_U * FK_LDS, L);
   const float v = fk_slab_reduce<2 * FR_U>(acc, sm.sPart, jsel);
   if (!early) {
-    if (tid == 0) wait_ge(wait_ctr, wait_target);
+    if (tid == 0) wait_ge_abortable(wait_ctr, wait_target, abort);
     __syncthreads();
     if (on) pre = ly.Wx[(size_t)sm.gIdx[FK_B + b] * ly.ld3 + col] + bias;
   }
@@ -512,50 +606,57 @@
     const float g = on ? sigmoidf_(v + pre) : 0.f;
     if (isr) {
       sm.gR[b * FR_U + j] = g;
+      const float ho = sH[b * FK_LDS + c];
       if (on) {
-        const float ho = sH[b * FK_LDS + c];
         ly.r[(size_t)b * ldL + c] = g;
         ly.Hold[(size_t)b * ldL + c] = ho;
-        ly.Hr[(size_t)b * ldL + c] = ho * g;
-      }
+      }
+      if (b < M) ll_store1(hrp + ((size_t)b * ldL + c) * 2, on ? ho * g : 0.f, T);
     } else {
       sm.gZ[b * FR_U + j] = g;
       if (on) ly.z[(size_t)b * ldL + c] = g;
     }
   }
 }
-__device__ void fr_f2(const ModelDev& md, FastSmemR& sm, int s, int k0, const float* sHo) {
+__device__ void fr_f2(const ModelDev& md, FastSmemR& sm, int s, int k0, const float* sHo, const float* hrp, float* yp, unsigned int T, int* abort) {
   const LayerDev& ly = md.layer[0];
   const int M = md.wM[s], L = ly.L, ldL = ly.ldL, tid = threadIdx.x;
   const int b = tid & 31, jsel = tid >> 5, c = k0 + jsel;
   const bool on = jsel < FR_U && b < M && c < L;
   float pre = 0.f;
   if (on) pre = ly.Wx[(size_t)sm.gIdx[FK_B + b] * ly.ld3 + c] + sm.rB[0][jsel];
-  stage_rows4(sm.gHr, FK_LDS, FK_B, ldL / 4, [&](int rr) -> const float* { return rr < M ? ly.Hr + (size_t)rr * ldL : nullptr; });
+  ll_stage_rows(sm.gHr, hrp, ldL, M, ldL / 4, T, abort);
   __syncthreads();
   float acc[FR_U];
   fk_slab_dot<FR_U>(acc, sm.gHr, FK_LDS, sm.rC[0], L);
   const float v0 = fk_slab_reduce<FR_U>(acc, sm.sPart, jsel);
+  if (jsel < FR_U && b < M && !on) ll_store1(yp + ((size_t)b * ldL + c) * 2, 0.f, T);
   if (on) {
     const float v = v0 + pre;
     const float ht = act_fwd(md.hact, v);
     const float z = sm.gZ[b * FR_U + jsel], ho = sHo[b * FK_LDS + c];
     float h = (1.0f - z) * ho + z * ht;
     if (md.p_drop_h > 0.f) h *= drop_scale(md.drop_seed, md.wG[s], 0u, (uint32_t)(b * L + c), 1.0f - md.p_drop_h);
+    ll_store1(yp + ((size_t)b * ldL + c) * 2, h, T);
     ly.ah[(size_t)b * ldL + c] = v;
     ly.ht[(size_t)b * ldL + c] = ht;
     ly.y[(size_t)b * ldL + c] = h;
     ly.H[(size_t)sm.gIdx[b] * ldL + c] = (sm.gIdx[2 * FK_B + b] & 1) ? 0.f : h;
   }
 }
-__device__ void fr_b2(const ModelDev& md, FastSmemR& sm, int s, int k0, const float* sHo) {
-  const LayerDev& ly = md.layer[0];
-  const int M = md.wM[s], L = ly.L, ld3 = ly.ld3, tid = threadIdx.x;
-  float dz = 0.f;
-  if (tid < FK_B * FR_U && tid / FR_U < M && k0 + tid % FR_U < L) dz = ly.dvec[(size_t)(tid / FR_U) * ld3 + 2 * L + k0 + tid % FR_U];
-  stage_rows4(sm.sD, FK_LDS, FK_B, ly.ldL / 4, [&](int rr) -> const float* { return rr < M ? ly.dvec + (size_t)rr * ld3 : nullptr; });
+__device__ void fr_b2(const ModelDev& md, FastSmemR& sm, int s, int k0, const float* sHo, const float* dap, unsigned int T, int* abort) {
+  const LayerDev& ly = md.layer[0];
+  const int M = md.wM[s], L = ly.L, ldL = ly.ldL, ld3 = ly.ld3, tid = threadIdx.x;
+  const int bq = tid / FR_U, cq = k0 + tid % FR_U;
+  const bool own = tid < FK_B * FR_U && bq < M && cq < L;
+  const float* dzp = dap + ((size_t)bq * 2 * ldL + ldL + cq) * 2;
+  uint2 dzv = make_uint2(0u, T);
+  if (own) dzv = ll_ld1(dzp);
+  ll_stage_rows(sm.sD, dap, 2 * ldL, M, ldL / 4, T, abort);
+  const float dz = dzv.y == T ? __uint_as_float(dzv.x) : ll_load1(dzp, T, abort);
   if (tid < FK_B * FR_U) sm.gDz[tid] = dz;
   __syncthreads();
+  if (own) { ly.dvec[(size_t)bq * ld3 + cq] = sm.sD[bq * FK_LDS + cq]; ly.dvec[(size_t)bq * ld3 + 2 * L + cq] = dz; }
   const int b = tid & 31, jsel = tid >> 5, c = k0 + jsel;
   float acc[FR_U];
   fk_slab_dot<FR_U>(acc, sm.sD, FK_LDS, sm.rR[0], L);
@@ -615,8 +716,8 @@
     }
   }
 }
-template <class SM>
-__device__ __forceinline__ void fk_part(SM& sm, float* part, int M, int nj, int ldL) {
+template <bool LL = false, class SM>
+__device__ __forceinline__ void fk_part(SM& sm, float* part, int M, int nj, int ldL, unsigned int T = 0) {
   const int kw = ldL / 4;
   for (int t = threadIdx.x; t < M * kw; t += FK_THREADS) {
     const int bb = t / kw, q4 = t % kw;
@@ -626,7 +727,8 @@
       const float4 w = ld4(sm.sS + jj * FK_LDS + q4 * 4);
       a.x = fmaf(g, w.x, a.x); a.y = fmaf(g, w.y, a.y); a.z = fmaf(g, w.z, a.z); a.w = fmaf(g, w.w, a.w);
     }
-    st4(part + (size_t)bb * ldL + q4 * 4, a);
+    if (LL) ll_store4(part + ((size_t)bb * ldL + q4 * 4) * 2, a, T);
+    else st4(part + (size_t)bb * ldL + q4 * 4, a);
   }
 }
 template <class SM>
@@ -683,7 +785,7 @@
 #include "g4r_fastc.cuh"
 
 template <bool CL>
-__global__ void __launch_bounds__(FK_THREADS, 1) k_fast_t(int slot, int n_steps, FastSync* fs, unsigned long long* tstamp) {
+__global__ void __launch_bounds__(FK_THREADS, 1) k_fast_t(int slot, int n_steps, FastSync* fs, unsigned long long* tstamp, FastLL ll, unsigned int seq0) {
   using SM = typename std::conditional<CL, FastSmemC, FastSmemR>::type;
   extern __shared__ __align__(128) unsigned char fk_raw[];
   SM& sm = *reinterpret_cast<SM*>(fk_raw);
@@ -701,8 +803,12 @@
   const int ldL = md.ldL, B = md.B;
   const int kw = ldL / 4;
   uint64_t* bar = reinterpret_cast<uint64_t*>(&sm.mbar);
-  unsigned int bar_epoch = 0, gepoch = 0, stats_target = 0;
+  unsigned int bar_epoch = 0, stats_target = 0;
   const int in_ctas = min(B, ncta - G);
+  auto wait = [&](const unsigned int* p, unsigned int target) { if (CL) wait_ge(p, target); else wait_ge_abortable(p, target, ll.abort); };
+  auto llbuf = [](float* base, size_t n, unsigned int T) { return base + (size_t)(T & 1u) * n * 2; };
+  const size_t n_y = (size_t)B * ldL, n_stat = (size_t)md.NCH * B * G4R_NSTAT, n_rs = (size_t)B * G4R_NSTAT, n_part = (size_t)md.NCH * B * ldL,
+               n_da = (size_t)B * 2 * ldL;
 #ifdef G4R_CF_FINE
 #define FK_FTS(s_) ((tstamp && cta == 0 && (s_) < 500 && n_steps >= 1000) ? tstamp + (size_t)((s_) + 500) * 16 : nullptr)
 #define FK_STAMP_OK(s_) ((s_) < 500)
@@ -732,11 +838,12 @@
     if (gru) {
       fr_load_resident(md, sm, 4 * cta);
       if (n_steps > 0) {
+        const unsigned int T0 = seq0 + 1u;
         fk_stage_lanes(md, sm, 0, md.wM[0]);
         stage_rows4(sm.gH[0], FK_LDS, FK_B, kw, [&](int rr) -> const float* { const int sl = sm.gIdx[rr]; return sl >= 0 ? ly.H + (size_t)sl * ldL : nullptr; });
-        fr_f1(md, sm, 0, 4 * cta, sm.gH[0], nullptr, 0u);
-        fk_group_barrier(fs, gepoch, G);
-        fr_f2(md, sm, 0, 4 * cta, sm.gH[0]);
+        fr_f1(md, sm, 0, 4 * cta, sm.gH[0], nullptr, 0u, llbuf(ll.Hr, n_y, T0), T0, ll.abort);
+        __syncthreads();
+        fr_f2(md, sm, 0, 4 * cta, sm.gH[0], llbuf(ll.Hr, n_y, T0), llbuf(ll.y, n_y, T0), T0, ll.abort);
         __syncthreads();
         if (tid == 0) red_release_add(&fs->h_ready, 1u);
       }
@@ -747,6 +854,7 @@
     const int M = md.wM[s];
     const int sti = md.wSti[s];
     const int N = M + (sti >= 0 ? md.S : 0);
+    const unsigned int T = seq0 + (unsigned int)s + 1u;
     FK_STAMP(0);
     if (col) fk_load_idx(md, sm, s + 1, n_steps, chunk, buf ^ 1);
     const bool gru_next = !CL && gru && s + 1 < n_steps;
@@ -756,8 +864,10 @@
       sm.gIdx[FK_B + tid] = tid < M1 ? md.wX[(size_t)(s + 1) * B + tid] : 0;
       sm.gIdx[2 * FK_B + tid] = tid < M1 ? md.wF[(size_t)(s + 1) * B + tid] : 0;
     }
-    if (tid == 0) wait_ge(&fs->h_ready, (unsigned int)(s + 1) * (unsigned int)G);
-    __syncthreads();
+    if (CL || !col) {
+      if (tid == 0) wait(&fs->h_ready, (unsigned int)(s + 1) * (unsigned int)G);
+      __syncthreads();
+    }
     if constexpr (!CL) {
       if (!col) {
         const bool nxt = s + 1 < n_steps;
@@ -765,21 +875,40 @@
         const float* sHo = sm.gH[s & 1];
         float* hnext = sm.gH[(s + 1) & 1];
         if (nxt) stage_rows4(hnext, FK_LDS, FK_B, kw, [&](int rr) -> const float* { const int sl = sm.gIdx[rr]; return sl >= 0 ? ly.H + (size_t)sl * ldL : nullptr; });
-        __syncthreads();
-        if (tid == 0) wait_ge(&fs->b1_done, (unsigned int)(s + 1) * (unsigned int)ncol);
+        const float* dap = llbuf(ll.da, n_da, T);
+        if (warp == 0) {
+          const int E = M * ldL, per = ((E + ncol - 1) / ncol + 31) / 32 * 32;
+          const float* src[4];
+          unsigned int pend = 0, spins = 0;
+          unsigned long long t0 = 0;
+#pragma unroll
+          for (int u = 0; u < 4; u++) {
+            const int x = lane + 32 * u, e = min((x + 1) * per, E) - 1;
+            src[u] = dap + ((size_t)(e / ldL) * 2 * ldL + ldL + e % ldL) * 2;
+            if (x * per < E) pend |= 1u << u;
+          }
+          while (pend) {
+            uint2 p[4];
+#pragma unroll
+            for (int u = 0; u < 4; u++) if (pend & (1u << u)) p[u] = ll_ld1(src[u]);
+#pragma unroll
+            for (int u = 0; u < 4; u++) if ((pend & (1u << u)) && p[u].y == T) pend &= ~(1u << u);
+            if (pend && ll_give_up(spins, t0, ll.abort)) break;
+          }
+        }
         __syncthreads();
         FK_STAMP(4);
-        fr_b2(md, sm, s, k0, sHo);
+        fr_b2(md, sm, s, k0, sHo, dap, T, ll.abort);
         __syncthreads();
         if (tid == 0) red_release_add(&fs->dvec_done, 1u);
         FK_STAMP(5);
         fr_dense(md, sm, s, k0, sHo);
         FK_STAMP(6);
         if (nxt) {
-          fr_f1(md, sm, s + 1, k0, hnext, &fs->in_done, (unsigned int)(s + 1) * (unsigned int)in_ctas);
-          fk_group_barrier(fs, gepoch, G);
+          fr_f1(md, sm, s + 1, k0, hnext, &fs->in_done, (unsigned int)(s + 1) * (unsigned int)in_ctas, llbuf(ll.Hr, n_y, T + 1u), T + 1u, ll.abort);
+          __syncthreads();
           FK_STAMP(7);
-          fr_f2(md, sm, s + 1, k0, hnext);
+          fr_f2(md, sm, s + 1, k0, hnext, llbuf(ll.Hr, n_y, T + 1u), llbuf(ll.y, n_y, T + 1u), T + 1u, ll.abort);
           __syncthreads();
           if (tid == 0) red_release_add(&fs->h_ready, 1u);
         }
@@ -787,7 +916,13 @@
         continue;
       }
     }
-    stage_rows4(sm.sY, FK_LDS, FK_B, kw, [&](int rr) -> const float* { return rr < M ? ly.y + (size_t)rr * ldL : nullptr; });
+    if (CL) stage_rows4(sm.sY, FK_LDS, FK_B, kw, [&](int rr) -> const float* { return rr < M ? ly.y + (size_t)rr * ldL : nullptr; });
+    else {
+      const float* yp = llbuf(ll.y, n_y, T);
+      if (warp == 0 && lane < G && M > 0) ll_load1(yp + ((size_t)(M - 1) * ldL + 4 * lane + 3) * 2, T, ll.abort);
+      __syncthreads();
+      ll_stage_rows(sm.sY, yp, ldL, M, kw, T, ll.abort);
+    }
     mbar_wait(bar, (unsigned int)(s & 1));
     __syncthreads();
     FK_STAMP(1);
@@ -847,13 +982,13 @@
         }
 #pragma unroll
         for (int o = 1; o < 16; o <<= 1) mloc = fmaxf(mloc, __shfl_xor_sync(0xffffffffu, mloc, o));
-        float Z = 0.f, A = 0.f, Q = 0.f, D = 0.f, T = 0.f, has = 0.f;
+        float Z = 0.f, A = 0.f, Q = 0.f, D = 0.f, Tt = 0.f, has = 0.f;
 #pragma unroll
         for (int q = 0; q < 2; q++) {
           if (!use[q]) continue;
           const float y = yv[q];
           if (ist[q]) has = 1.f;
-          if (xe) { Z += expf(y - mloc); if (ist[q]) T = y; }
+          if (xe) { Z += expf(y - mloc); if (ist[q]) Tt = y; }
           else if (md.loss == G4R_LOSS_BPR_MAX) { if (!ist[q]) { const float e = expf(y - mloc), sg = sigmoidf_(t - y); Z += e; A += sg * e; Q += y * y * e; D += sg * (1.f - sg) * e; } }
           else if (md.loss == G4R_LOSS_TOP1_MAX) { if (!ist[q]) { const float e = expf(y - mloc), a1 = sigmoidf_(y - t), b1 = sigmoidf_(y * y); Z += e; A += (a1 + b1) * e; D += a1 * (1.f - a1) * e; } }
           else if (md.loss == G4R_LOSS_BPR) { const float sg = sigmoidf_(t - y); A += -logf(sg); if (!ist[q]) D += 1.f - sg; }
@@ -862,28 +997,43 @@
 #pragma unroll
         for (int o = 1; o < 16; o <<= 1) {
           Z += __shfl_xor_sync(0xffffffffu, Z, o); A += __shfl_xor_sync(0xffffffffu, A, o); Q += __shfl_xor_sync(0xffffffffu, Q, o);
-          D += __shfl_xor_sync(0xffffffffu, D, o); T += __shfl_xor_sync(0xffffffffu, T, o); has += __shfl_xor_sync(0xffffffffu, has, o);
+          D += __shfl_xor_sync(0xffffffffu, D, o); Tt += __shfl_xor_sync(0xffffffffu, Tt, o); has += __shfl_xor_sync(0xffffffffu, has, o);
         }
         if (has_chunk && okb && sub == 0) {
-          float* st = md.stat + ((size_t)chunk * md.B + b) * G4R_NSTAT;
-          st4(st, make_float4(mloc, Z, A, Q));
-          st4(st + 4, make_float4(D, T, has > 0.f ? 1.f : 0.f, pw ? t : 0.f));
+          const float4 s0 = make_float4(mloc, Z, A, Q), s1 = make_float4(D, Tt, has > 0.f ? 1.f : 0.f, pw ? t : 0.f);
+          if (CL) {
+            float* st = md.stat + ((size_t)chunk * md.B + b) * G4R_NSTAT;
+            st4(st, s0); st4(st + 4, s1);
+          } else {
+            float* st = llbuf(ll.stat, n_stat, T) + ((size_t)chunk * md.B + b) * G4R_NSTAT * 2;
+            ll_store4(st, s0, T); ll_store4(st + 8, s1, T);
+          }
         }
       }
     }
     __syncthreads();
     FK_STAMP(10);
-    bar_epoch += 1;
-    if (tid == 0) { red_release_add(&fs->bar, 1u); wait_ge(&fs->bar, bar_epoch * (unsigned int)ncol); }
-    __syncthreads();
+    if (CL) {
+      bar_epoch += 1;
+      if (tid == 0) { red_release_add(&fs->bar, 1u); wait_ge(&fs->bar, bar_epoch * (unsigned int)ncol); }
+      __syncthreads();
+    } else if (tid == 0) {
+      wait(&fs->h_ready, (unsigned int)(s + 1) * (unsigned int)G);
+    }
     if (chunk < M) {
       const int b = chunk;
       const bool maxed = !(md.loss == G4R_LOSS_BPR || md.loss == G4R_LOSS_TOP1);
-      float mc = -INFINITY, Z = 0.f, A = 0.f, Q = 0.f, D = 0.f, T = 0.f, has = 0.f, tt = 0.f;
+      float mc = -INFINITY, Z = 0.f, A = 0.f, Q = 0.f, D = 0.f, Tt = 0.f, has = 0.f, tt = 0.f;
       if (tid < md.NCH) {
-        const float* st = md.stat + ((size_t)tid * md.B + b) * G4R_NSTAT;
-        const float4 u = ld4(st), v = ld4(st + 4);
-        mc = u.x; Z = u.y; A = u.z; Q = u.w; D = v.x; T = v.y; has = v.z;
+        float4 u, v;
+        if (CL) {
+          const float* st = md.stat + ((size_t)tid * md.B + b) * G4R_NSTAT;
+          u = ld4(st); v = ld4(st + 4);
+        } else {
+          const float* st = llbuf(ll.stat, n_stat, T) + ((size_t)tid * md.B + b) * G4R_NSTAT * 2;
+          u = ll_load4(st, T, ll.abort); v = ll_load4(st + 8, T, ll.abort);
+        }
+        mc = u.x; Z = u.y; A = u.z; Q = u.w; D = v.x; Tt = v.y; has = v.z;
         if (tid == 0) tt = v.w;
       }
       float mg = mc;
@@ -901,34 +1051,45 @@
 #pragma unroll
       for (int o = 1; o < 32; o <<= 1) {
         Z += __shfl_xor_sync(0xffffffffu, Z, o); A += __shfl_xor_sync(0xffffffffu, A, o); Q += __shfl_xor_sync(0xffffffffu, Q, o);
-        D += __shfl_xor_sync(0xffffffffu, D, o); T += __shfl_xor_sync(0xffffffffu, T, o); has += __shfl_xor_sync(0xffffffffu, has, o);
-      }
-      __syncthreads();
-      if (lane == 0) { float* w = sm.sPart + 32 + warp * 8; w[0] = Z; w[1] = A; w[2] = Q; w[3] = D; w[4] = T; w[5] = has; w[6] = tt; }
+        D += __shfl_xor_sync(0xffffffffu, D, o); Tt += __shfl_xor_sync(0xffffffffu, Tt, o); has += __shfl_xor_sync(0xffffffffu, has, o);
+      }
+      __syncthreads();
+      if (lane == 0) { float* w = sm.sPart + 32 + warp * 8; w[0] = Z; w[1] = A; w[2] = Q; w[3] = D; w[4] = Tt; w[5] = has; w[6] = tt; }
       __syncthreads();
       if (tid == 0) {
         tt = sm.sPart[32 + 6];
-        for (int w = 1; w < FK_NW; w++) { const float* q = sm.sPart + 32 + w * 8; Z += q[0]; A += q[1]; Q += q[2]; D += q[3]; T += q[4]; }
+        for (int w = 1; w < FK_NW; w++) { const float* q = sm.sPart + 32 + w * 8; Z += q[0]; A += q[1]; Q += q[2]; D += q[3]; Tt += q[4]; }
         const float m = mg;
-        float* rs = md.RS + (size_t)b * G4R_NSTAT;
         float loss = 0.f, r0 = m, r1 = Z, r2 = 0.f, r3 = 0.f, r4 = 0.f, r5 = tt;
-        if (md.loss == G4R_LOSS_XE) { const float pt = __fdiv_rn(expf(T - m), Z); loss = -logf(pt + G4R_EPS_LOG); r2 = pt; r5 = T; }
-        else if (md.loss == G4R_LOSS_XE_LOGIT) { loss = logf(Z) - (T - m); r5 = T; }
+        if (md.loss == G4R_LOSS_XE) { const float pt = __fdiv_rn(expf(Tt - m), Z); loss = -logf(pt + G4R_EPS_LOG); r2 = pt; r5 = Tt; }
+        else if (md.loss == G4R_LOSS_XE_LOGIT) { loss = logf(Z) - (Tt - m); r5 = Tt; }
         else if (md.loss == G4R_LOSS_BPR_MAX) { r2 = __fdiv_rn(A, Z); r3 = __fdiv_rn(Q, Z); r4 = __fdiv_rn(D, Z); loss = -logf(r2 + G4R_EPS_LOG) + md.bpreg * r3; }
         else if (md.loss == G4R_LOSS_TOP1_MAX) { r2 = __fdiv_rn(A, Z); r4 = __fdiv_rn(D, Z); loss = r2; }
         else if (md.loss == G4R_LOSS_BPR) { loss = A; r4 = D; }
         else { const float c = sigmoidf_(tt * tt); loss = (float)M * (__fdiv_rn(A, (float)N) - __fdiv_rn(c, (float)(M + md.S_cfg))); r4 = D; }
-        st4(rs, make_float4(r0, r1, r2, r3));
-        st4(rs + 4, make_float4(r4, r5, loss, 0.f));
-        red_release_add(&fs->stats, 1u);
-      }
-    }
-    stats_target += (unsigned int)M;
-    if (tid == 0) wait_ge(&fs->stats, stats_target);
-    __syncthreads();
-    FK_STAMP(2);
-    if (tid < M * 2) st4(sm.sRS + tid * 4, ld4(md.RS + tid * 4));
-    __syncthreads();
+        const float4 q0 = make_float4(r0, r1, r2, r3), q1 = make_float4(r4, r5, loss, 0.f);
+        if (CL) {
+          float* rs = md.RS + (size_t)b * G4R_NSTAT;
+          st4(rs, q0); st4(rs + 4, q1);
+          red_release_add(&fs->stats, 1u);
+        } else {
+          float* rs = llbuf(ll.RS, n_rs, T) + (size_t)b * G4R_NSTAT * 2;
+          ll_store4(rs, q0, T); ll_store4(rs + 8, q1, T);
+        }
+      }
+    }
+    if (CL) {
+      stats_target += (unsigned int)M;
+      if (tid == 0) wait_ge(&fs->stats, stats_target);
+      __syncthreads();
+      FK_STAMP(2);
+      if (tid < M * 2) st4(sm.sRS + tid * 4, ld4(md.RS + tid * 4));
+      __syncthreads();
+    } else {
+      if (tid < M * 2) st4(sm.sRS + tid * 4, ll_load4(llbuf(ll.RS, n_rs, T) + tid * 8, T, ll.abort));
+      __syncthreads();
+      FK_STAMP(2);
+    }
     if (chunk == 0 && tid == 0) {
       float c = 0.f;
       for (int b = 0; b < M; b++) c += sm.sRS[b * 8 + 6];
@@ -944,8 +1105,8 @@
     __syncthreads();
     fk_dby(sm, M, nj);
     FK_STAMP(12);
-    float* part = md.part + (size_t)(has_chunk ? chunk : 0) * md.B * ldL;
     if constexpr (CL) {
+      float* part = md.part + (size_t)(has_chunk ? chunk : 0) * md.B * ldL;
       if (has_chunk) { fk_dsy(sm, M, nj, kw); fk_part(sm, part, M, nj, ldL); }
       __syncthreads();
       FK_STAMP(13);
@@ -990,25 +1151,20 @@
         if (tid == 0) red_release_add(&fs->in_done, 1u);
       }
     } else {
-      if (has_chunk) fk_part(sm, part, M, nj, ldL);
-      if (has_chunk && nj == 0) for (int i = tid; i < M * ldL; i += FK_THREADS) part[i] = 0.f;
-      __syncthreads();
+      const float* partp = llbuf(ll.part, n_part, T);
+      if (has_chunk) fk_part<true>(sm, const_cast<float*>(partp) + (size_t)chunk * md.B * ldL * 2, M, nj, ldL, T);
       FK_STAMP(13);
-      bar_epoch += 1;
-      if (tid == 0) { red_release_add(&fs->bar, 1u); wait_ge(&fs->bar, bar_epoch * (unsigned int)ncol); }
-      __syncthreads();
       FK_STAMP(3);
-      fk_b1<CL>(md, sm, s, chunk, ncol);
-      __syncthreads();
-      if (tid == 0) red_release_add(&fs->b1_done, 1u);
+      fk_b1<false, true>(md, sm, s, chunk, ncol, partp, llbuf(ll.da, n_da, T), T, ll.abort);
+      __syncthreads();
       FK_STAMP(15);
       fk_dsy(sm, M, nj, kw);
       __syncthreads();
       if (chunk < in_ctas) {
         const unsigned int tgt = (unsigned int)(s + 1) * (unsigned int)G;
-        if (in_ctas == B && ly.ld3 / 4 <= FK_THREADS) fk_sparse_in_one(md, sm, s, chunk, &fs->dvec_done, tgt);
+        if (in_ctas == B && ly.ld3 / 4 <= FK_THREADS) fk_sparse_in_one(md, sm, s, chunk, &fs->dvec_done, tgt, ll.abort);
         else {
-          if (tid == 0) wait_ge(&fs->dvec_done, tgt);
+          if (tid == 0) wait(&fs->dvec_done, tgt);
           __syncthreads();
           for (int b = chunk; b < B; b += in_ctas) { fk_sparse_in(md, sm, s, b); __syncthreads(); }
         }
@@ -1020,7 +1176,7 @@
       FK_STAMP(14);
       if (tid == 0) red_release_add(&fs->rows_done, 1u);
       if (s + 1 < n_steps) {
-        if (tid == 0) wait_ge(&fs->rows_done, (unsigned int)(s + 1) * (unsigned int)ncol);
+        if (tid == 0) wait(&fs->rows_done, (unsigned int)(s + 1) * (unsigned int)ncol);
         __syncthreads();
         fk_prefetch_rows(md, sm, s + 1, n_steps, buf ^ 1, pw);
       }
diff --git a/gru4rec_b200/csrc/g4r_kernels.cuh b/gru4rec_b200/csrc/g4r_kernels.cuh
--- a/gru4rec_b200/csrc/g4r_kernels.cuh
+++ b/gru4rec_b200/csrc/g4r_kernels.cuh
@@ -82,6 +82,16 @@
   unsigned int dvec_done; unsigned int p6[31];
   unsigned int rows_done; unsigned int p7[31];
 };
+struct FastLL {
+  float* y;
+  float* Hr;
+  float* stat;
+  float* RS;
+  float* part;
+  float* da;
+  size_t pairs;
+  int* abort;
+};
 struct GridBar { unsigned int count; unsigned int gen; unsigned int pad[30]; };
 
 struct LayerDev {
@@ -96,7 +106,6 @@
   float *Hold, *r, *z, *ah, *ht, *y;
   float *dvec;
   float *dy;
-  float *Hr;
   const float* in;
 };
 
diff --git a/gru4rec_b200/csrc/g4r_lib.cu b/gru4rec_b200/csrc/g4r_lib.cu
--- a/gru4rec_b200/csrc/g4r_lib.cu
+++ b/gru4rec_b200/csrc/g4r_lib.cu
@@ -76,6 +76,9 @@
   void* shard = nullptr;
   char* shard_ws = nullptr;
   size_t shard_ws_bytes = 0;
+  FastLL fast_ll = {};
+  uint32_t fast_seq = 0;
+  bool fast_ran = false;
   FastSync* dFastSync = nullptr; bool fast_ok = false; bool fastc_ok = false; int fastc_grid = 0; int* hFlags = nullptr; int64_t fast_windows = 0, slow_windows = 0;
   bool prof = false; bool stamp_on = false;
   bool two_pass = false;
@@ -202,7 +205,7 @@
     reg("He" + si, he, Be, L, ly.ldL);
     ly.Hold = cv.take<float>((size_t)Bmax * ly.ldL); ly.r = cv.take<float>((size_t)Bmax * ly.ldL); ly.z = cv.take<float>((size_t)Bmax * ly.ldL);
     ly.ah = cv.take<float>((size_t)Bmax * ly.ldL); ly.ht = cv.take<float>((size_t)Bmax * ly.ldL); ly.y = cv.take<float>((size_t)Bmax * ly.ldL);
-    ly.dvec = cv.take<float>((size_t)Bmax * ly.ld3); ly.dy = cv.take<float>((size_t)Bmax * ly.ldL); ly.Hr = cv.take<float>((size_t)Bmax * ly.ldL);
+    ly.dvec = cv.take<float>((size_t)Bmax * ly.ld3); ly.dy = cv.take<float>((size_t)Bmax * ly.ldL);
     reg("y" + si, ly.y, Bmax, L, ly.ldL); reg("dvec" + si, ly.dvec, Bmax, 3 * L, ly.ld3);
   }
   if (mode != 0) {
@@ -221,6 +224,16 @@
   md.gscale = gsc;
   md.cost = cv.take<float>((size_t)CAP);
   md.nanflag = cv.take<int>(4);
+  FastLL fll; memset(&fll, 0, sizeof(fll));
+  if (c.step_mode == 2 && mode == 0 && nl == 1 && ldL <= 128 && B <= 32 && !shard) {
+    const size_t ny = (size_t)B * ldL, nst = (size_t)NCH * B * G4R_NSTAT, nrs = (size_t)B * G4R_NSTAT, npart = (size_t)NCH * B * ldL, nda = (size_t)B * 2 * ldL;
+    fll.pairs = 2 * (2 * ny + nst + nrs + npart + nda);
+    float* p = cv.take<float>(fll.pairs * 2);
+    if (p) {
+      fll.y = p; fll.Hr = fll.y + 4 * ny; fll.stat = fll.Hr + 4 * ny; fll.RS = fll.stat + 4 * nst; fll.part = fll.RS + 4 * nrs; fll.da = fll.part + 4 * npart;
+      fll.abort = md.nanflag + 3;
+    }
+  }
   reg("O", md.O, NP, Bmax, md.Bld); reg("DSY", md.DSY, NP, Llast, ldL);
   int* dX = cv.take<int>((size_t)CAP * B); int* dY = cv.take<int>((size_t)CAP * B); int* dSlot = cv.take<int>((size_t)CAP * B);
   int* dXnext = cv.take<int>((size_t)CAP * B);
@@ -303,7 +316,7 @@
     md.ST = dST; md.logP0t = dL0t; md.logP0s = dL0s;
     h->md = md; h->Bmax = Bmax; h->CAP = CAP; h->mg_alloc = R > 1; h->mgdev = mgd; h->mg_tensors = mgt; h->gen_len = store ? gen_len : 0;
     h->dX = dX; h->dY = dY; h->dSlot = dSlot; h->dM = dM; h->dSti = dSti; h->dXnext = dXnext; h->dF = dF; h->dXflag = dXflag; h->dG = dG;
-    h->dGridBar = dGridBar; h->dStamp = dStamp; h->dFastSync = dFastSync;
+    h->dGridBar = dGridBar; h->dStamp = dStamp; h->dFastSync = dFastSync; h->fast_ll = fll;
     h->dStepBase = dStepBase; h->dP = dP; h->dLogP0t = dL0t; h->dLogP0s = dL0s; h->dST = dST; h->dU = dU; h->dMrgState = dMrg;
     h->dRankCnt = dRank; h->dTgt = dTgt;
     h->npow2 = next_pow2(B + S);
@@ -1183,6 +1196,7 @@
   return n;
 }
 
+#define FAST_TIMEOUT_MSG "step_mode 2: an exchange between the CTAs of the training kernel timed out; the window's results are not valid"
 static int run_window(g4r_handle* h, int64_t n) {
   bool fast = false, fastc = false;
   if ((h->cfg.step_mode == 3 && h->fastc_ok) || (h->cfg.step_mode == 2 && h->fast_ok)) {
@@ -1194,17 +1208,23 @@
       fast = fits && h->cfg.step_mode == 2;
     }
   }
+  h->fast_ran = fast;
   if (fastc) {
     int slot = h->slot, nst = (int)n; FastSync* fsp = h->dFastSync; unsigned long long* ts = h->stamp_on ? h->dStamp : nullptr;
-    void* args[] = {&slot, &nst, &fsp, &ts};
+    FastLL ll = {}; unsigned int seq0 = 0;
+    void* args[] = {&slot, &nst, &fsp, &ts, &ll, &seq0};
     CK(cudaMemsetAsync(h->dFastSync, 0, sizeof(FastSync), h->stream));
     CK(fastc_launch(h->fastc_grid, h->stream, args));
     h->launches += 1; h->fast_windows++;
   } else if (fast) {
     int slot = h->slot, nst = (int)n; FastSync* fsp = h->dFastSync; unsigned long long* ts = h->stamp_on ? h->dStamp : nullptr;
-    void* args[] = {&slot, &nst, &fsp, &ts};
+    FastLL ll = h->fast_ll; unsigned int seq0 = h->fast_seq;
+    void* args[] = {&slot, &nst, &fsp, &ts, &ll, &seq0};
     CK(cudaMemsetAsync(h->dFastSync, 0, sizeof(FastSync), h->stream));
+    CK(cudaMemsetAsync(h->md.nanflag + 3, 0, sizeof(int), h->stream));
     CK(cudaLaunchCooperativeKernel((void*)k_fast_t<false>, dim3(h->pk_blocks), dim3(FK_THREADS), args, sizeof(FastSmemR), h->stream));
+    CK(cudaMemcpyAsync(h->hFlags, h->md.nanflag, 4 * sizeof(int), cudaMemcpyDeviceToHost, h->stream));
+    h->fast_seq += (uint32_t)n;
     h->launches += 1; h->fast_windows++;
   } else if (h->cfg.step_mode >= 1 && !h->prof && h->pk_blocks > 0 && !h->phase_only && !h->tc_ok) {
     if (h->cfg.step_mode >= 2) h->slow_windows++;
@@ -1262,6 +1282,7 @@
   if (h->shard) CK(cudaMemcpyAsync(h->hFlags, h->md.nanflag, 4 * sizeof(int), cudaMemcpyDeviceToHost, h->stream));
   CK(cudaStreamSynchronize(h->stream));
   if (h->shard && h->hFlags[3]) FAIL(G4R_ERR_STATE, "multi-GPU: a cross-GPU wait timed out (a peer rank stopped or never started its window)");
+  if (h->fast_ran && h->hFlags[3]) FAIL(G4R_ERR_STATE, FAST_TIMEOUT_MSG);
   if (cost_out) memcpy(cost_out, h->hCost, (size_t)n * sizeof(float));
   if (device_ms) CK(cudaEventElapsedTime(device_ms, h->ev0, h->ev1));
   return G4R_OK;
@@ -1299,6 +1320,21 @@
   }
   return G4R_OK;
 }
+__global__ void k_ll_fill(float* p, size_t pairs, uint32_t tag) {
+  for (size_t i = (size_t)blockIdx.x * blockDim.x + threadIdx.x; i < pairs; i += (size_t)gridDim.x * blockDim.x) {
+    p[2 * i] = __uint_as_float(0x7fc00000u); p[2 * i + 1] = __uint_as_float(tag);
+  }
+}
+extern "C" int g4r_fast_poison(g4r_handle* h, uint32_t tag) {
+  if (!h) return G4R_ERR_INVALID;
+  if (!h->fast_ll.y) FAIL(G4R_ERR_STATE, "this handle has no step_mode 2 pair buffers");
+  cudaSetDevice(h->cfg.device);
+  k_ll_fill<<<264, 256, 0, h->stream>>>(h->fast_ll.y, h->fast_ll.pairs, tag);
+  CK(cudaGetLastError());
+  CK(cudaStreamSynchronize(h->stream));
+  return G4R_OK;
+}
+extern "C" int64_t g4r_fast_sequence(const g4r_handle* h) { return h ? (int64_t)h->fast_seq : 0; }
 extern "C" int g4r_uses_tensor_cores(const g4r_handle* h) { return (h && h->tc_ok) ? 1 : 0; }
 extern "C" int64_t g4r_fast_windows(const g4r_handle* h, int64_t* fallback_windows) {
   if (!h) return 0;
@@ -1335,6 +1371,7 @@
     if (h->shard) CK(cudaMemcpyAsync(h->hFlags, h->md.nanflag, 4 * sizeof(int), cudaMemcpyDeviceToHost, h->stream));
     CK(cudaStreamSynchronize(h->stream));
     if (h->shard && h->hFlags[3]) FAIL(G4R_ERR_STATE, "multi-GPU: a cross-GPU wait timed out (a peer rank stopped or never started its window)");
+    if (h->fast_ran && h->hFlags[3]) FAIL(G4R_ERR_STATE, FAST_TIMEOUT_MSG);
     for (int64_t i = 0; i < w; i++) {
       if (cost_out) cost_out[done + i] = h->hCost[i];
       if (h->hCost[i] != h->hCost[i]) {
@@ -1369,6 +1406,7 @@
   if (rc) return rc;
   CK(cudaMemcpyAsync(h->hCost, h->md.cost, sizeof(float), cudaMemcpyDeviceToHost, h->stream));
   CK(cudaStreamSynchronize(h->stream));
+  if (h->fast_ran && h->hFlags[3]) FAIL(G4R_ERR_STATE, FAST_TIMEOUT_MSG);
   if (cost) *cost = h->hCost[0];
   if (h->hCost[0] != h->hCost[0]) FAIL(G4R_ERR_NAN, "NaN error!");
   return G4R_OK;
diff --git a/gru4rec_b200/csrc/g4r_shard.cuh b/gru4rec_b200/csrc/g4r_shard.cuh
--- a/gru4rec_b200/csrc/g4r_shard.cuh
+++ b/gru4rec_b200/csrc/g4r_shard.cuh
@@ -1,6 +1,4 @@
 #pragma once
-
-constexpr unsigned long long MGS_TIMEOUT_NS = 4000000000ull;
 
 __device__ __forceinline__ unsigned int ld_acquire_sys_u32(const unsigned int* p) {
   unsigned int v;
@@ -15,19 +13,14 @@
   asm volatile("ld.volatile.global.v4.f32 {%0, %1, %2, %3}, [%4];" : "=f"(v.x), "=f"(v.y), "=f"(v.z), "=f"(v.w) : "l"(p) : "memory");
   return v;
 }
-__device__ __forceinline__ unsigned long long mgs_timer() {
-  unsigned long long t;
-  asm volatile("mov.u64 %0, %%globaltimer;" : "=l"(t));
-  return t;
-}
 __device__ __forceinline__ void wait_sys_ge(const unsigned int* p, unsigned int target, int* abort) {
   if ((int)(ld_acquire_sys_u32(p) - target) >= 0) return;
-  const unsigned long long t0 = mgs_timer();
+  const unsigned long long t0 = ll_timer();
   unsigned int spins = 0;
   while ((int)(ld_acquire_sys_u32(p) - target) < 0) {
     if ((++spins & 127u) == 0) {
       if (*(volatile int*)abort) return;
-      if (mgs_timer() - t0 > MGS_TIMEOUT_NS) { atomicExch(abort, 1); return; }
+      if (ll_timer() - t0 > LL_TIMEOUT_NS) { atomicExch(abort, 1); return; }
     }
   }
 }
@@ -37,45 +30,6 @@
     if (q < sh.R && q != skip) wait_sys_ge(sh.flags[sh.rank] + (size_t)(first + q) * MGS_FLAG_STRIDE, target, sh.abort);
     __syncwarp();
   }
-}
-__device__ __forceinline__ void ll_store4(float* dst_pairs, float4 v, unsigned int seq) {
-  asm volatile("st.volatile.global.v4.u32 [%0], {%1, %2, %3, %4};" :: "l"(dst_pairs), "r"(__float_as_uint(v.x)), "r"(seq), "r"(__float_as_uint(v.y)), "r"(seq) : "memory");
-  asm volatile("st.volatile.global.v4.u32 [%0], {%1, %2, %3, %4};" :: "l"(dst_pairs + 4), "r"(__float_as_uint(v.z)), "r"(seq), "r"(__float_as_uint(v.w)), "r"(seq) : "memory");
-}
-__device__ __forceinline__ float4 ll_load4(const float* src_pairs, unsigned int seq, int* abort) {
-  uint4 a, b;
-  unsigned int spins = 0; unsigned long long t0 = 0;
-  while (true) {
-    asm volatile("ld.volatile.global.v4.u32 {%0, %1, %2, %3}, [%4];" : "=r"(a.x), "=r"(a.y), "=r"(a.z), "=r"(a.w) : "l"(src_pairs) : "memory");
-    asm volatile("ld.volatile.global.v4.u32 {%0, %1, %2, %3}, [%4];" : "=r"(b.x), "=r"(b.y), "=r"(b.z), "=r"(b.w) : "l"(src_pairs + 4) : "memory");
-    if (a.y == seq && a.w == seq && b.y == seq && b.w == seq) break;
-    if ((++spins & 127u) == 0) {
-      if (*(volatile int*)abort) break;
-      const unsigned long long t = mgs_timer();
-      if (t0 == 0) t0 = t;
-      if (t - t0 > MGS_TIMEOUT_NS) { atomicExch(abort, 1); break; }
-    }
-  }
-  return make_float4(__uint_as_float(a.x), __uint_as_float(a.z), __uint_as_float(b.x), __uint_as_float(b.z));
-}
-__device__ __forceinline__ float ll_load1(const float* src_pair, unsigned int seq, int* abort) {
-  uint2 a;
-  unsigned int spins = 0; unsigned long long t0 = 0;
-  while (true) {
-    asm volatile("ld.volatile.global.v2.u32 {%0, %1}, [%2];" : "=r"(a.x), "=r"(a.y) : "l"(src_pair) : "memory");
-    if (a.y == seq) break;
-    if ((++spins & 127u) == 0) {
-      if (*(volatile int*)abort) break;
-      const unsigned long long t = mgs_timer();
-      if (t0 == 0) t0 = t;
-      if (t - t0 > MGS_TIMEOUT_NS) { atomicExch(abort, 1); break; }
-    }
-  }
-  return __uint_as_float(a.x);
-}
-__device__ __forceinline__ void wait_ge_abortable(const unsigned int* p, unsigned int target, int* abort) {
-  unsigned int spins = 0;
-  while (ld_acquire_u32(p) < target) { if ((++spins & 1023u) == 0 && *(volatile int*)abort) return; }
 }
 
 struct FastSmemMG : FastSmem {
diff --git a/include/g4r.h b/include/g4r.h
--- a/include/g4r.h
+++ b/include/g4r.h
@@ -104,6 +104,8 @@
 int g4r_profile_uploaded(g4r_handle* h, float* phase_ms, int32_t* phase_launches, int32_t n_phases);
 const char* g4r_phase_name(int32_t i);
 int64_t g4r_fast_windows(const g4r_handle* h, int64_t* fallback_windows);
+int64_t g4r_fast_sequence(const g4r_handle* h);
+int g4r_fast_poison(g4r_handle* h, uint32_t tag);
 int g4r_uses_tensor_cores(const g4r_handle* h);
 int g4r_persistent_stamps(g4r_handle* h, int32_t enable, unsigned long long* out, int64_t n_steps);
 int g4r_phase_count(void);
```

After: 32270, median of 6. Within noise of the previous version (+0.7%).
